# NCKempke/PIPS-IPMpp

Hardware: AMD Instinct MI355X
Metric: KKT factor+solve per IPM iter/sec, N-block arrowhead LP (higher is better)
Workload: dtype f64; 1 GPU; 64 blocks x 10000 vars (5000 eq rows, rho=0.001), Schur dim 2000, 64 blocks/GPU [BASELINE configs[1]]; deterministic=False, family=random, root=dense LDL^T, sparse_head=multifrontal (k_front), solves_per_unit=4, collective=none, nnzL_per_gpu=649118456

## Files before the change

### include/pips_hip.h

```cpp
#ifndef PIPS_HIP_H
#define PIPS_HIP_H
#include <stddef.h>
#include <stdint.h>

#ifdef __cplusplus
extern "C" {
#endif

const char* pips_hip_last_error(void);
long long pips_hip_host_wait_count(void);
int pips_hip_host_wait_sites(char* buf, int cap);
long long pips_hip_device_allocs_live(void);
long long pips_hip_device_bytes_live(void);
int pips_hip_device_count(void);

int pips_hip_ldl_create(void** handle, int n, const int* krow, const int* jcol, int device, int flags);
int pips_hip_ldl_set_inertia_hint(void* handle, int n_primal);
int pips_hip_ldl_set_pivot_rule(void* handle, double thr_rel, double repl_rel);
int pips_hip_ldl_set_refinement(void* handle, int max_steps, double tol);
int pips_hip_ldl_set_refinement_backward_error(void* handle, int max_steps, double tol);
int pips_hip_ldl_set_deterministic(void* handle, int on);
int pips_hip_ldl_analyze(void* handle);
int pips_hip_ldl_factor(void* handle, const double* vals_host);
int pips_hip_ldl_set_values(void* handle, const double* K_val_host);
// ... 147 lines not shown
} pips_csr_view;
typedef struct {
   int n, my, mz;
   pips_csr_view A, B, C, D, BL, DL;
   const double *c, *xlow, *xupp, *ixlow, *ixupp;
   const double* b;
   const double *clow, *cupp, *iclow, *icupp;
} pips_ipm_block;
int pips_ipm_create_general(void** handle, int n_blocks, const pips_ipm_block* blocks, int myl, int mzl, const double* bL,
                            const double* dlow, const double* dupp, const double* idlow, const double* idupp, double dual_reg,
                            int device, void* comm, int rank, int n_ranks);
int pips_ipm_create(void** handle, int N, int n0, int myl, const int* n_i, const int* my_i, const int* W_rowptr,
                    const int* W_colidx, const double* W_val, const int* T_rowptr, const int* T_colidx, const double* T_val,
                    const int* F_rowptr, const int* F_colidx, const double* F_val, const int* F0_rowptr, const int* F0_colidx,
                    const double* F0_val, const double* c, const double* b, double dual_reg, int device);
int pips_ipm_create_rank(void** handle, int N, int n0, int myl, const int* n_i, const int* my_i, const int* W_rowptr,
                         const int* W_colidx, const double* W_val, const int* T_rowptr, const int* T_colidx, const double* T_val,
                         const int* F_rowptr, const int* F_colidx, const double* F_val, const int* F0_rowptr, const int* F0_colidx,
                         const double* F0_val, const double* c, const double* b, double dual_reg, int device, void* comm, int rank,
                         int n_ranks);
int pips_ipm_solve(void* handle, int max_iter, double mutol, double artol, int verbose, double* result7);
int pips_ipm_set_gondzio(void* handle, int max_correctors);
int pips_ipm_set_option(void* handle, const char* name, double value);
int pips_ipm_set_free_variables(void* handle, const double* bounded_mask_host);
int pips_ipm_get_solution(void* handle, double* x_host, double* y_host);
int pips_ipm_get_dims(void* handle, long long* dims4);
int pips_ipm_get_iterate(void* handle, double* x, double* s, double* y, double* z, double* t, double* u, double* v, double* w,
                         double* lambda, double* pi, double* gamma, double* phi);
int pips_ipm_get_trace(void* handle, double* rows7, int max_rows, int* n_rows);
int pips_ipm_get_stats(void* handle, long long* stats4);
int pips_ipm_get_stats2(void* handle, long long* stats2);
int pips_ipm_get_schur_mode(void* handle, int* mode);
int pips_ipm_mult(void* handle, int transposed, const double* in_host, double* out_host);
enum {
   PIPS_SCALER_NONE = 0,
   PIPS_SCALER_EQUILIBRIUM = 1,
   PIPS_SCALER_GEOMETRIC_MEAN = 2,
   PIPS_SCALER_GEOMETRIC_MEAN_EQUILIBRIUM = 3,
   PIPS_SCALER_CURTIS_REID = 4
};
int pips_ipm_create_general_scaled(void** handle, int n_blocks, const pips_ipm_block* blocks, int myl, int mzl, const double* bL,
                                   const double* dlow, const double* dupp, const double* idlow, const double* idupp, double dual_reg,
                                   int device, void* comm, int rank, int n_ranks, int scaler);
int pips_ipm_get_scaling(void* handle, double* col, double* row_eq, double* row_ineq, double* info8);
int pips_ipm_outer_solve(void* handle, const double* G_host, const double* L_host, const double* rhs_host, double tol, double* sol_host,
                         double* info6);
int pips_ipm_create_qp(void** handle, int n_blocks, const pips_ipm_block* blocks, const pips_csr_view* Q, int myl, int mzl,
                       const double* bL, const double* dlow, const double* dupp, const double* idlow, const double* idupp,
                       double dual_reg, int device, void* comm, int rank, int n_ranks);
int pips_ipm_hessian_mult(void* handle, const double* in_host, double* out_host);
void pips_ipm_destroy(void* handle);

int pips_gen_row_nnz(int n_i, double rho);
int pips_gen_block(uint64_t seed, int block, int n_i, int my_i, int n0, int myl, double rho, int* W_rowptr,
                   int* W_colidx, double* W_val, int* T_rowptr, int* T_colidx, double* T_val, int* F_rowptr,
                   int* F_colidx, double* F_val, double* c, double* xstar);
int pips_gen_root(uint64_t seed, int n0, int myl, int* F0_rowptr, int* F0_colidx, double* F0_val, double* c0,
                  double* xstar0);
int pips_gen_diagonal(uint64_t seed, int block, int n, double lo, double hi, double* d);
int pips_kkt_leaf_assemble(int nx, int my, int mz, const int* Q_rowptr, const int* Q_colidx, const double* Q_val,
                           const int* B_rowptr, const int* B_colidx, const double* B_val, const int* D_rowptr,
                           const int* D_colidx, const double* D_val, int* K_rowptr, int* K_colidx, double* K_val,
                           int* diag_pos);
int pips_border_assemble(int nx, int my, int mz, int n0, int n_empty, int myl, int mzl, const int* R_rowptr,
                         const int* R_colidx, const double* R_val, const int* A_rowptr, const int* A_colidx,
                         const double* A_val, const int* C_rowptr, const int* C_colidx, const double* C_val,
                         const int* F_rowptr, const int* F_colidx, const double* F_val, const int* G_rowptr,
                         const int* G_colidx, const double* G_val, int* Bt_rowptr, int* Bt_colidx, double* Bt_val);
int pips_map_children_to_ranks(int n_children, int n_ranks, int* map);
int pips_symbolic_probe(int n, int n_primal, const int* krow, const int* jcol, int S, const int* Bt_rowptr,
                        const int* Bt_colidx, int force_n_head, int64_t* what, int n_what, int* perm, int* colcount);

int pips_symbolic_probe_hubs(int n, int n_primal, const int* krow, const int* jcol, int n_hubs, const int* hubs, int min_size,
                             int64_t* what, int n_what, int* perm, int* colcount);

int pips_layout_probe(int nblk, const int* n, const int* n_primal, const int* const* krow, const int* const* kcol,
                      int S, const int* const* bt_rowptr, const int* const* bt_colidx,
                      int deterministic, long long free_device_bytes, int64_t* what, int n_what);

int pips_tail_plan_probe(int nblk, const int* n, const int* n_primal, const int* const* krow, const int* const* kcol,
                         int S, const int* const* bt_rowptr, const int* const* bt_colidx, int force_n_head,
                         int* col_tasks, long long col_cap, int* grp_tasks, long long grp_cap, int64_t* counts);

int pips_det_plan_probe(int nblk, const int* n, const int* n_primal, const int* const* krow, const int* const* kcol,
                        int S, const int* const* bt_rowptr, const int* const* bt_colidx, int rank, int n_ranks, int n_panels,
                        long long* out, long long cap, int64_t* counts);

enum { PIPS_IPML_DIMS = 20, PIPS_IPML_SLOTS = 48 };
int pips_ipm_layout_probe(int n_blocks, const pips_ipm_block* blocks, const pips_csr_view* Q, int myl, int mzl, const double* bL,
                          const double* dlow, const double* dupp, const double* idlow, const double* idupp, int rank, int n_ranks,
                          int eliminate_z0, const double* col, const double* row, long long* dims, double* scalars, long long* sizes,
                          void* const* out);

int pips_schur_pack_probe(int nblk, int S, const int* const* bt_rowptr, int* nb, int* nb_max, int* const* local_of_row);

int pips_schur_target_probe(int nblk, int S, const int* const* bt_rowptr, const int* sc_rowptr, const int* sc_colidx, int lower, int* nb,
                            long long* n_touched, long long* pos, long long cap, int* const* tab);

int pips_gdx_read_block(void** block, const char* path, int num_blocks, int act_block, int offset);
int pips_gdx_block_counts(void* block, long long* counts14);
int pips_gdx_block_vector(void* block, int which, double* out, int capacity, int* length);
int pips_gdx_block_matrix(void* block, int which, int* present, int* rows, int* cols, int* rowptr, int* colidx, double* val);
void pips_gdx_block_destroy(void* block);

#ifdef __cplusplus
}
#endif
#endif
```

### pips-ipmpp_amd/csrc/engine.hip

```cpp
#include <hip/hip_runtime.h>

#include <algorithm>
#include <cstdlib>
#include <cstring>
#include <map>
#include <memory>
#include <mutex>
#include <thread>
#include <vector>

#include "common.h"
#include "devmem.h"
#include "layout.h"
#include "detplan.h"
#include "schurtarget.h"
#include "kernels.hip.h"
#include "rootkernel.hip.h"
#include "tailkernel.hip.h"
#include "pips_hip.h"

namespace pips {

static thread_local std::string g_last_error;
void set_last_error(const std::string& msg) { g_last_error = msg; }
// ... 655 lines not shown
         if (l.cnt > 0) launch_tile_gemm<2>(c, c.d_sc_tasks, l, c.stream, SC, ldSC);
         HIP_TRY(hipEventRecord((*c.ev_sc)[g], c.stream));
      }
   } else if (tile_gemm_bal_ready(c) && !c.d_sctab)
      launch_tile_gemm_bal<2>(c, p.d_tasks, p.schur, c.stream, SC, ldSC);
   else
      launch_tile_gemm<2>(c, p.d_tasks, p.schur, c.stream, SC, ldSC);
   return PIPS_OK;
}

static int tail_factor(const TailCtx& c, double* SC, int ldSC) {
   const bool trsm_tri = !c.bunch_kaufman && !c.is_root && env_int("PIPS_HIP_TRSM_DENSE", 0) == 0;
   if (!c.single && c.panels && c.side && trsm_tri && env_int("PIPS_HIP_TAIL_PANEL", 1) != 0) PIPS_TRY(tail_panels(c));
   else if (!c.single) PIPS_TRY(tail_columns(c, trsm_tri));
   else if (c.single->n_tasks > 0) PIPS_TRY(tail_single_launch(c));
   PIPS_TRY(tail_schur(c, SC, ldSC));
   HIP_TRY(hipGetLastError());
   return PIPS_OK;
}

static int tail_fwd(const TailCtx& c, double* xw, int nrhs = 1, long long xw_stride = 0) {
   const TailPlan& p = *c.plan;
   if (c.sweep && c.sweep->enabled && nrhs <= SWEEP_NRHS_MAX) {
      hipLaunchKernelGGL(k_tail_rows_fwd, dim3(c.sweep->n_tasks, nrhs), dim3(256), 0, c.stream, c.sweep->args(xw_stride, c.stream), c.d_blks, c.d_arena, c.d_dtail,
                         c.d_winv, xw);
      HIP_TRY(hipGetLastError());
      return PIPS_OK;
   }
   for (int j = 0; j < p.ntc_max; ++j)
      if (p.fwd[j].cnt > 0)
         hipLaunchKernelGGL(k_tail_fwd, dim3(p.fwd[j].cnt, nrhs), dim3(256), 0, c.stream, p.d_tasks + p.fwd[j].off, c.d_blks,
                            c.d_arena, c.d_dtail, c.d_winv, xw, j, xw_stride);
   HIP_TRY(hipGetLastError());
   return PIPS_OK;
}

static int tail_bwd(const TailCtx& c, double* xw, int nrhs = 1, long long xw_stride = 0, int border = 0) {
   const TailPlan& p = *c.plan;
   if (p.ntc_max == 0) return PIPS_OK;
   if (border && !(c.sweep && c.sweep->enabled)) PIPS_FAIL(PIPS_ERR_STATE, "border-backward sweep needs the single-launch tail sweeps");
   if (c.sweep && c.sweep->enabled && nrhs <= SWEEP_NRHS_MAX) {
      hipLaunchKernelGGL(k_tail_rows_bwd, dim3(c.sweep->n_tasks, nrhs), dim3(256), 0, c.stream, c.sweep->args(xw_stride, c.stream), c.d_blks, c.d_arena, c.d_dtail,
                         c.d_winv, xw, border);
      HIP_TRY(hipGetLastError());
      return PIPS_OK;
   }
   for (int i = p.ntc_max - 1; i >= 0; --i)
      if (p.bwd[i].cnt > 0)
         hipLaunchKernelGGL(k_tail_bwd, dim3(p.bwd[i].cnt, nrhs), dim3(256), 0, c.stream, p.d_tasks + p.bwd[i].off, c.d_blks,
                            c.d_arena, c.d_dtail, c.d_winv, xw, i, xw_stride);
   HIP_TRY(hipGetLastError());
   return PIPS_OK;
}


struct AnalyzeKnobs : LayoutKnobs {
   long long tail_poll_limit = 0;
   int tail_diag_blocked = 1;
};
struct Engine;
static void read_layout_knobs(const Engine* e, AnalyzeOptions& opt, AnalyzeKnobs& knobs);

struct EngineAnalysis {
   DevBuf<double> d_norms;
   PinnedBuf<double> h_norms;
   DevBuf<int> d_frowptr, d_fcol, d_fsrc;
   DevBuf<long long> d_flong;
   DevBuf<int> d_sctab;
   long long sc_len = 0;
   DevBuf<int> d_schur_cols, d_schur_slot;
   SchurPack pack;
   int packed_rhs = 0;
   DevBuf<int> d_pk_la;
   DevBuf<long long> d_pk_tabrow;
   PackRows h_pk_rows;
   std::vector<int> h_pk_tab;
   DevBuf<int> d_kb_rec;
   DevBuf<long long> d_kb_off;
   DevBuf<int> d_kb_list;
   DevBuf<int> d_kb_tail;
   DevBuf<double> d_mfU;
   DevBuf<double> d_mfLV;
   DevBuf<int> d_roots, d_root_off;
   DevBuf<BbBatch> d_bb_batches;
   DevBuf<BbMeta> d_bb_meta;
   DevBuf<int> d_bb_off, d_bb_pos;
   DevBuf<double> d_bb_out;
   DevBuf<int> d_bb_round_blk;
   DevBuf<int> d_round_blk;
   DevBuf<int> d_mfint;
   DevBuf<long long> d_mfdbg;
   DevBuf<int> d_spine, d_spine_off;
   TailPlan plan;
   PanelPlan panels;
   SweepRt sweep;
   TailSingle tsingle;
   DevBuf<double> d_uarena;
   DevBuf<double> d_arena, d_kval, d_bval, d_winv, d_dtail, d_xw, d_rhs, d_res, d_stage, d_pref;
   DevBuf<long long> d_kdst, d_bdst, d_kdiag, d_kptr, d_psign_off, d_perm_off, d_rowbase, d_bt_xoff;
   DevBuf<SnDesc> d_sns;
   DevBuf<BlkDesc> d_blks;
   DevBuf<int> d_lf_rows, d_lf_ptr, d_lf_src, d_lf_pos;
   DevBuf<double> d_lf_val;
   DevBuf<LeafDesc> d_leafdesc;
   DevBuf<int> d_lb_list;
   DevBuf<int> d_rowidx, d_upd, d_sncol, d_bmap, d_perm, d_inertia, d_nprimal;
   DevBuf<int> d_br_rowptr, d_br_sc, d_br_src;
   DevBuf<int> d_krowptr, d_kcolidx, d_bt_rowptr, d_bt_colidx, d_bt_rowsc;
   DevBuf<signed char> d_psign;
   struct GatherList {
      long long n_targets = 0, n_slots = 0;
      DevBuf<long long> d_tgt, d_off, d_slots;
      int upload(const HostGather& h) {
         *this = GatherList();
         n_targets = (long long)h.tgt.size(); n_slots = (long long)h.slots.size();
         if (h.tgt.empty()) return PIPS_OK;
         int rc;
         if ((rc = d_tgt.upload(h.tgt)) || (rc = d_off.upload(h.off)) || (rc = d_slots.upload(h.slots))) return rc;
         return PIPS_OK;
      }
   };
   DetGroupPlan det;
   ScKept sc_kept;
   DevBuf<double> d_slot_val, d_vslot_val;
   DevBuf<double> d_mvslot;
   std::vector<GatherList> g_levels, gv_levels;
   GatherList g_tail, g_sc, gv_tail;
   GatherList g_sc_grp;
   GatherList g_btm_grp;
   GatherList g_pk_grp;
   DevBuf<double> d_gvec, d_tvec;
   DevBuf<TileTask> d_det_tasks;
   DevBuf<double> d_gbuf;
   DevBuf<int> d_blk_group;
   GatherList g_btm, g_bm;
   DevBuf<BgEntry> d_bg_ent;
   DevBuf<long long> d_bg_ptr, d_bg_slot;
   DevBuf<int> d_bg_idx;
   DevBuf<double> d_bg_val;
   GatherList g_bslot_grp;
   DevBuf<double> d_bt_tmp;
   DevBuf<int> d_gemm_ctr;
   ScPanelPlan scp;
   std::vector<hipEvent_t> ev_sc;
   DevBuf<TileTask> d_sc_tasks;
   DevBuf<double> d_mx_xw, d_mx_rhs, d_mx_res;
   int mx_cap = 0;
   DevBuf<double> d_mmeasure;
   PinnedBuf<double> h_mmeasure;
   DevBuf<int> d_midx;
   DevBuf<double> d_hostx;
   DevBuf<double> d_hostpack;
   PinnedBuf<int> h_inertia_pin;
   hipEvent_t ev_inertia = nullptr;
   bool inertia_in_flight = false, inertia_on_host = false;
};

struct Engine : EngineAnalysis, BatchLayout {
   int device = 0;
   hipStream_t stream = nullptr;
   int nblk = 0, S = 0;
   bool analyzed = false, factored = false;
   long long analysis_gen = 0;
   int refine_steps = 1;
   double refine_tol = 0.0;
   int refine_mode = 0;
// ... 162 lines not shown
         PIPS_TRY(d_bb_meta.upload(h_bb_meta));
         PIPS_TRY(d_bb_pos.upload(h_bb_pos));
         PIPS_TRY(d_bb_off.upload(h_bb_off));
      }
      if (kb_any) {
         PIPS_TRY(d_kb_rec.upload(h_kb_rec));
         PIPS_TRY(d_kb_off.upload(h_kb_off));
         PIPS_TRY(d_kb_list.upload(h_kb_list));
         PIPS_TRY(d_kb_tail.upload(h_kb_tail));
      }
      if (mf) {
         PIPS_TRY(d_mfint.upload(h_mfint));
         PIPS_TRY(d_mfU.alloc((size_t)std::max<long long>(mfU_total, 1)));
         PIPS_TRY(d_mfLV.alloc((size_t)std::max<long long>(mfLV_total, 1)));
      }
      PIPS_TRY(d_frowptr.upload(h_frowptr));
      PIPS_TRY(d_fcol.upload(h_fcol));
      PIPS_TRY(d_fsrc.upload(h_fsrc));
      PIPS_TRY(d_flong.upload(h_flong));
      if (deterministic && bt_rows_total > 0) {
         const BorderGathers bg = border_product_gathers(*this);
         PIPS_TRY(g_btm.upload(bg.btm));
         PIPS_TRY(g_bm.upload(bg.bm));
         PIPS_TRY(d_bt_tmp.alloc((size_t)std::max<long long>(std::max(bt_rows_total, nnzB_total), 1)));
      }
      PIPS_TRY(d_schur_cols.upload(schur_cols));
      PIPS_TRY(d_schur_slot.upload(h_schur_slot));
      PIPS_TRY(d_arena.alloc(std::max<long long>(arena_total + bb_doubles + tail_scratch, 1)));
      if (tail_single) HIP_TRY(hipMemsetAsync(d_arena, 0, (size_t)arena_total * sizeof(double), stream));
      if (bb_doubles > 0) HIP_TRY(hipMemsetAsync(d_arena + arena_total, 0, (size_t)bb_doubles * sizeof(double), stream));
      PIPS_TRY(d_uarena.alloc(std::max<long long>(uarena_total, 1)));
      PIPS_TRY(d_kval.alloc(std::max<long long>(nnzK_total, 1)));
      HIP_TRY(hipMemset(d_kval, 0, std::max<long long>(nnzK_total, 1) * sizeof(double)));
      PIPS_TRY(d_winv.alloc(std::max<long long>(winv_total, 1)));
      PIPS_TRY(d_dtail.alloc(std::max<long long>(dtail_total, 1)));
      PIPS_TRY(d_xw.alloc(std::max<long long>(xw_total, 1)));
      PIPS_TRY(d_pref.alloc(std::max<long long>(xw_total, 1)));
      PIPS_TRY(d_rhs.alloc(std::max<long long>(n_total, 1)));
      PIPS_TRY(d_res.alloc(std::max<long long>(n_total, 1)));
      PIPS_TRY(d_stage.alloc(std::max<long long>(n_total, 1)));
      PIPS_TRY(d_norms.alloc((size_t)3 * nblk));
      PIPS_TRY(h_norms.alloc((size_t)3 * nblk));
      PIPS_TRY(d_inertia.alloc((size_t)3 * nblk));
      HIP_TRY(hipMemset(d_inertia, 0, (size_t)3 * nblk * sizeof(int)));
      PIPS_TRY(d_bval.upload(h_bval));
      PIPS_TRY(d_kdst.upload(h_kdst));
      PIPS_TRY(d_bdst.upload(h_bdst));
      PIPS_TRY(d_kdiag.upload(h_kdiag));
      PIPS_TRY(d_kptr.upload(kptr));
      PIPS_TRY(d_psign_off.upload(h_psign_off));
      PIPS_TRY(d_perm_off.upload(h_perm_off));
      PIPS_TRY(d_rowbase.upload(h_rowbase));
      PIPS_TRY(d_bt_xoff.upload(h_bt_xoff));
      PIPS_TRY(d_sns.upload(h_sns));
      PIPS_TRY(d_blks.upload(h_blks));
      PIPS_TRY(d_rowidx.upload(h_rowidx));
      if (n_lb > 0) PIPS_TRY(d_lb_list.upload(h_lb_list));
      if (!h_leafdesc.empty()) PIPS_TRY(d_leafdesc.upload(h_leafdesc));
      if (lf_entries > 0) {
         PIPS_TRY(d_lf_rows.upload(h_lf_rows));
         PIPS_TRY(d_lf_ptr.upload(h_lf_ptr));
         PIPS_TRY(d_lf_src.upload(h_lf_src));
         PIPS_TRY(d_lf_pos.upload(h_lf_pos));
         PIPS_TRY(d_lf_val.alloc((size_t)lf_entries));
      }
      PIPS_TRY(d_upd.upload(h_upd));
      PIPS_TRY(d_spine.upload(h_spine));
      PIPS_TRY(d_spine_off.upload(h_spine_off));
      PIPS_TRY(d_sncol.upload(h_sncol));
      PIPS_TRY(d_bmap.upload(h_bmap));
      PIPS_TRY(d_perm.upload(h_perm));
      PIPS_TRY(d_psign.upload(h_psign));
      PIPS_TRY(d_krowptr.upload(h_krowptr));
      PIPS_TRY(d_kcolidx.upload(h_kcolidx));
      PIPS_TRY(d_bt_rowptr.upload(h_bt_rowptr));
      PIPS_TRY(d_bt_colidx.upload(h_bt_colidx));
      PIPS_TRY(d_bt_rowsc.upload(h_bt_rowsc));
      if (!h_br_rowptr.empty()) {
         PIPS_TRY(d_br_rowptr.upload(h_br_rowptr));
         PIPS_TRY(d_br_sc.upload(h_br_sc));
         PIPS_TRY(d_br_src.upload(h_br_src));
      }
      PIPS_TRY(d_nprimal.upload(h_nprimal));
      return PIPS_OK;
   }

   ScatterCtx sx_atomic() const { return ScatterCtx{0, nullptr, nullptr, nullptr, nullptr}; }
   void launch_head_level(const LevelRange& L, double* SC, int ldSC, const ScatterCtx& sx) {
      if (L.simple_cnt > 0)
         hipLaunchKernelGGL(k_head_factor_simple, dim3((L.simple_cnt + 255) / 256), dim3(256), 0, stream, d_sns, L.simple_begin,
                            L.simple_cnt, d_blks, d_rowidx, d_upd, d_psign, d_psign_off, d_bmap, d_arena, SC, ldSC, d_inertia, d_pref, d_sctab, sx,
                            mf ? 1 : 0, d_mfLV, d_lf_pos, d_lf_val, d_arena);
      if (mf) return;
      if (L.small_cnt > 0)
         hipLaunchKernelGGL((k_head_factor<64, 8, 640>), dim3(L.small_cnt), dim3(64), (size_t)std::max(L.small_lds, 1) * sizeof(double), stream, d_sns,
                            L.small_begin, d_blks, d_rowidx, d_upd, d_psign, d_psign_off, d_bmap, d_arena, SC, ldSC, d_inertia, d_pref, d_sctab, sx,
                            L.small_lds);
      if (L.large_cnt > 0)
         hipLaunchKernelGGL((k_head_factor<256, 32, 6144>), dim3(L.large_cnt), dim3(256), (size_t)std::max(L.large_lds, 1) * sizeof(double), stream, d_sns,
                            L.large_begin, d_blks, d_rowidx, d_upd, d_psign, d_psign_off, d_bmap, d_arena, SC, ldSC,
                            d_inertia, d_pref, d_sctab, sx, L.large_lds);
   }
   template <int BLOCK, int WMAX, bool UG = false>
   int launch_front(const MfLaunch& m, double* SC, int ldSC) {
      const size_t lds = (size_t)m.lds_doubles * sizeof(double);
      if (lds > 64 * 1024) HIP_TRY(hipFuncSetAttribute((const void*)k_front<BLOCK, WMAX, UG>, hipFuncAttributeMaxDynamicSharedMemorySize, (int)lds));
      hipLaunchKernelGGL((k_front<BLOCK, WMAX, UG>), dim3(m.cnt), dim3(BLOCK), lds, stream, d_sns, m.begin, d_blks, d_rowidx, d_mfint, d_psign,
                         d_psign_off, d_bmap, d_arena, d_mfU, SC, ldSC, d_inertia, d_pref, d_sctab, d_mfdbg, d_mfLV, d_kval, d_bval, deterministic ? 1 : 0, d_arena);
      return PIPS_OK;
   }
   int launch_border_schur(double* SC, int ldSC) {
      constexpr int BLK = 512;
      const long long ncp = ((long long)bb_nbmax * (bb_nbmax + 1) / 2 + 1) & ~1LL;
      constexpr int parts = 1;
      const long long c_cap = ncp;
      BbPlanSize z; z.stage = bb_stage; z.poscap = bb_poscap; z.nbmax = bb_nbmax;
      const size_t lds = bb_lds_bytes(z);
      if (!bb_fits(z))
         PIPS_FAIL(PIPS_ERR_STATE, "k_border_schur: %zu bytes of LDS for nb = %d (batch of %d doubles, %d rows)", lds, bb_nbmax, bb_stage, bb_poscap);
      const int split = std::max(1, std::min(32, (bb_two_per_cu ? 512 : 256) / std::max(nblk, 1)));
      auto go = [&](auto kern, int cnt, const int* list, double* gb, long long gs, const int* grp, int sp, int ordered, double* out = nullptr,
                    long long out_stride = 0) -> int {
         if (lds > 64 * 1024) HIP_TRY(hipFuncSetAttribute((const void*)kern, hipFuncAttributeMaxDynamicSharedMemorySize, (int)lds));
         hipLaunchKernelGGL(kern, dim3(cnt, sp, parts), dim3(BLK), lds, stream, list, d_bb_off, d_bb_batches, d_bb_meta, d_bb_pos, d_blks, d_bmap, d_arena, SC, ldSC,
                            d_sctab, gb, gs, grp, bb_stage, bb_poscap, ordered, out, out_stride, (int)c_cap);
         return PIPS_OK;
      };
      const bool small = bb_stage <= 2 * 3 * BLK;
      int rc = PIPS_OK;
      if (deterministic && d_gbuf && d_bb_round_blk) {
         const long long tri = (long long)ncp;
         if (!d_bb_out) PIPS_TRY(d_bb_out.alloc((size_t)std::max(nblk, 1) * tri));
         rc = small ? go(k_border_schur<BLK, 3>, nblk, (const int*)nullptr, (double*)nullptr, 0LL, (const int*)nullptr, 1, 1, d_bb_out, tri)
                    : go(k_border_schur<BLK, 6>, nblk, (const int*)nullptr, (double*)nullptr, 0LL, (const int*)nullptr, 1, 1, d_bb_out, tri);
         for (size_t k = 0; k + 1 < det.bb_round_off.size() && !rc; ++k) {
            const int cnt = det.bb_round_off[k + 1] - det.bb_round_off[k];
            if (cnt > 0)
               hipLaunchKernelGGL(k_border_schur_add, dim3(cnt, 8), dim3(256), 0, stream, d_bb_round_blk + det.bb_round_off[k], d_blks, d_bmap, d_bb_out, tri, ldSC, d_sctab,
                                  d_gbuf, det_gstride(), d_blk_group);
         }
      } else
         rc = small ? go(k_border_schur<BLK, 3>, nblk, (const int*)nullptr, (double*)nullptr, 0LL, (const int*)nullptr, split, deterministic ? 1 : 0)
                    : go(k_border_schur<BLK, 6>, nblk, (const int*)nullptr, (double*)nullptr, 0LL, (const int*)nullptr, split, deterministic ? 1 : 0);
      return rc;
   }
   int dump_front_clocks() {
      std::vector<long long> h((size_t)nsn_total * 8);
      HIP_TRY(hipStreamSynchronize(stream));
      HIP_TRY(hipMemcpy(h.data(), d_mfdbg, h.size() * sizeof(long long), hipMemcpyDeviceToHost));
      static const char* names[7] = {"panel+zero", "stage ints", "leaf values + children", "leaf columns", "pivots", "update", "write-out"};
      for (const MfLaunch& m : mf_launches) {
         double ph[8] = {0}; long long nfs = 0, ws = 0;
         for (int i = m.begin; i < m.begin + m.cnt; ++i) {
            for (int q = 0; q < 7; ++q) ph[q] += (double)(h[(size_t)i * 8 + q + 1] - h[(size_t)i * 8 + q]);
            nfs += h_sns[i].w + h_sns[i].r; ws += h_sns[i].w;
         }
         fprintf(stderr, "[mf clocks] level %2d variant %d fronts %6d lds %6d  avg nf %5.1f w %4.1f | ", m.level, m.cls, m.cnt, m.lds_doubles * 8, (double)nfs / m.cnt, (double)ws / m.cnt);
         for (int q = 0; q < 7; ++q) fprintf(stderr, "%s %.1f%s", names[q], ph[q] / m.cnt * 0.01, q == 6 ? " us\n" : ", ");
      }
      return PIPS_OK;
   }
   void launch_border_rows(size_t l, hipStream_t st) {
      const int cnt = kb_level_off[l + 1] - kb_level_off[l];
      if (cnt == 0) return;
      const int* lst = d_kb_list + kb_level_off[l];
      if (kb_level_pairs[l] <= 3 || (cnt >= 16384 && kb_level_pairs[l] <= 8))
         hipLaunchKernelGGL((k_border_rows<64, 16>), dim3(cnt), dim3(64), kb_level_lds[l], st, lst, d_sns, d_blks, d_rowidx, d_kb_rec, d_kb_off, d_arena, d_arena, d_bval);
      else if (cnt <= 4096 && kb_level_pairs[l] > 8)
         hipLaunchKernelGGL((k_border_rows<512, 16>), dim3(cnt), dim3(512), kb_level_lds[l], st, lst, d_sns, d_blks, d_rowidx, d_kb_rec, d_kb_off, d_arena, d_arena, d_bval);
      else
         hipLaunchKernelGGL((k_border_rows<256, 16>), dim3(cnt), dim3(256), kb_level_lds[l], st, lst, d_sns, d_blks, d_rowidx, d_kb_rec, d_kb_off, d_arena, d_arena, d_bval);
   }
   int launch_fronts(int level, double* SC, int ldSC) {
      int rc = PIPS_OK;
      for (const MfLaunch& m : mf_launches) {
// ... 34 lines not shown
         HIP_TRY(hipGetLastError());
         HIP_TRY(hipStreamSynchronize(stream));
         HIP_TRY(hipMemcpy(rec.data(), d_rec, (size_t)slots_total * sizeof(long long), hipMemcpyDeviceToHost));
         d_rec.reset();
         PIPS_TRY(d_slot_val.alloc((size_t)slots_total));
      }
      {
         FactorSlotPlan fp;
         if ((rc = classify_factor_slots(rec, SCATTER_SC_FLAG, *this, sym, fp))) return rc;
         std::vector<long long>().swap(rec);
         for (int l = 0; l < nlev; ++l) PIPS_TRY(g_levels[l].upload(fp.levels[l]));
         PIPS_TRY(g_tail.upload(fp.tail));
         PIPS_TRY(g_sc.upload(fp.sc));
         sc_kept = std::move(fp.kept);
      }
      if (vslots_total > 0) {
         DevBuf<long long> d_rec;
         PIPS_TRY(d_rec.alloc((size_t)vslots_total));
         HIP_TRY(hipMemsetAsync(d_rec, 0xff, (size_t)vslots_total * sizeof(long long), stream));
         const ScatterCtx sxv{1, d_rec, nullptr, d_xw, nullptr};
         for (const LevelRange& L : levels) {
            if (L.simple_cnt > 0 && lf_rows == 0)
               hipLaunchKernelGGL(k_head_solve_simple, dim3((L.simple_cnt + 255) / 256, 1), dim3(256), 0, stream, d_sns, L.simple_begin,
                                  L.simple_cnt, d_blks, d_rowidx, d_arena, d_xw, 0LL, 0, sxv);
            const int begin = L.small_cnt > 0 ? L.small_begin : L.large_begin;
            const int cnt = L.small_cnt + L.large_cnt;
            if (cnt > 0) hipLaunchKernelGGL(k_head_fwd, dim3(cnt, 1), dim3(64), 0, stream, d_sns, begin, d_blks, d_rowidx, d_arena, d_xw, 0LL, sxv);
         }
         HIP_TRY(hipGetLastError());
         HIP_TRY(hipStreamSynchronize(stream));
         std::vector<long long> vrec((size_t)vslots_total);
         HIP_TRY(hipMemcpy(vrec.data(), d_rec, (size_t)vslots_total * sizeof(long long), hipMemcpyDeviceToHost));
         d_rec.reset();
         PIPS_TRY(d_vslot_val.alloc((size_t)vslots_total));
         SolveSlotPlan vp;
         classify_solve_slots(vrec, *this, sym, vp);
         for (int l = 0; l < nlev; ++l) PIPS_TRY(gv_levels[l].upload(vp.levels[l]));
         PIPS_TRY(gv_tail.upload(vp.tail));
      }
      (void)n_threads;
      return PIPS_OK;
   }

   const SchurPack& border_pack() {
      if (pack.off.empty()) build_schur_pack(in, S, pack);
      return pack;
   }
   int set_sc_tables(const std::vector<int>& tab, const std::vector<long long>& off, long long sc_nnz) {
      if (!analyzed) PIPS_FAIL(PIPS_ERR_STATE, "set_sc_tables: analyze first");
      HIP_TRY(hipSetDevice(device));
      int rc = d_sctab.upload(tab);
      if (rc) return rc;
      for (int b = 0; b < nblk; ++b) h_blks[b].sctab_off = off[b];
      HIP_TRY(hipMemcpy(d_blks, h_blks.data(), (size_t)nblk * sizeof(BlkDesc), hipMemcpyHostToDevice));
      sc_len = sc_nnz;
      packed_rhs = 0;
      if (schur_mode_eff == 2) {
         const SchurPack& pk = border_pack();
         if (pk.nb_max >= (1 << 24)) PIPS_FAIL(PIPS_ERR_STATE, "set_sc_tables: %d border columns in one block exceed the packed solves' 2^24", pk.nb_max);
         if ((rc = schur_pack_rows(in, S, off, (long long)tab.size(), h_pk_rows))) return rc;
         if ((long long)h_pk_rows.la.size() != bt_rows_total)
            PIPS_FAIL(PIPS_ERR_STATE, "set_sc_tables: %zu border rows, the analysis holds %lld", h_pk_rows.la.size(), bt_rows_total);
         PIPS_TRY(d_pk_la.upload(h_pk_rows.la));
         PIPS_TRY(d_pk_tabrow.upload(h_pk_rows.tabrow));
         if (deterministic) h_pk_tab = tab;
         else h_pk_rows = PackRows();
         packed_rhs = pk.nb_max;
      }
      if (head_slots) {
         g_levels.clear(); gv_levels.clear();
         g_tail = GatherList(); g_sc = GatherList(); gv_tail = GatherList();
         d_slot_val.reset(); d_vslot_val.reset(); d_mvslot.reset();
         if ((rc = build_deterministic(1))) return rc;
      }
      return PIPS_OK;
   }

   int factor_prologue() {
      PhaseTimer::Scope phase(&timer, stream, 0);
      hipLaunchKernelGGL(k_block_absmax_init, dim3((nblk + 255) / 256), dim3(256), 0, stream, d_blks, nblk);
      hipLaunchKernelGGL(k_block_absmax, dim3(std::max(1, std::min(64, (int)(nnzK_total / nblk / 4096))), nblk), dim3(256), 0, stream, d_kval,
                         d_kptr, d_blks);
      hipLaunchKernelGGL(k_block_absmax_finish, dim3((nblk + 255) / 256), dim3(256), 0, stream, d_blks, nblk, thr_rel, repl_rel);
      hipLaunchKernelGGL(k_arena_clear, dim3(256, nblk), dim3(256), 0, stream, d_blks, d_arena, mf ? 1 : 0);
      HIP_TRY(hipMemsetAsync(d_inertia, 0, (size_t)3 * nblk * sizeof(int), stream));
      if (!d_gemm_ctr) PIPS_TRY(d_gemm_ctr.alloc((size_t)GEMM_CTR_SLOTS * 8));
      HIP_TRY(hipMemsetAsync(d_gemm_ctr, 0, (size_t)GEMM_CTR_SLOTS * 8 * sizeof(int), stream));
      gemm_ctr_cursor = 0;
      if (nnzK_total > 0)
         hipLaunchKernelGGL(k_scatter, dim3(grid_for(nnzK_total, 256)), dim3(256), 0, stream, d_kdst, d_kval, d_arena, nnzK_total);
      if (nnzB_total > 0 && schur_mode_eff == 1)
         hipLaunchKernelGGL(k_scatter, dim3(grid_for(nnzB_total, 256)), dim3(256), 0, stream, d_bdst, d_bval, d_arena, nnzB_total);
      hipLaunchKernelGGL(k_tail_pad_diag, dim3(nblk), dim3(128), 0, stream, d_blks, d_arena, nblk);
      hipLaunchKernelGGL(k_pref_rows, dim3(32, nblk), dim3(256), 0, stream, d_blks, d_kval, d_kdiag, d_res, d_nprimal, d_krowptr, d_kcolidx);
      hipLaunchKernelGGL(k_pref_init, dim3(32, nblk), dim3(256), 0, stream, d_blks, d_perm, d_perm_off, (const double*)d_res, d_pref);
      return PIPS_OK;
   }
   void launch_root_assemble(double* SC, int ldSC) {
      const int asm_half = std::max(1, std::min(32, 1024 / std::max(nblk, 1)));
      if (deterministic && d_gbuf && SC && d_round_blk) {
         for (size_t k = 0; k + 1 < det.round_off.size(); ++k) {
            const int cnt = det.round_off[k + 1] - det.round_off[k];
            if (cnt > 0)
               hipLaunchKernelGGL(k_root_assemble, dim3(cnt, 2 * asm_half), dim3(256), 0, stream, d_round_blk + det.round_off[k], d_root_off, d_roots, d_sns, d_blks, d_rowidx,
                                  d_bmap, d_arena, d_mfU, SC, ldSC, d_sctab, d_gbuf, det_gstride(), d_blk_group, asm_half, asm_half);
         }
      } else
         hipLaunchKernelGGL(k_root_assemble, dim3(nblk, 2 * asm_half), dim3(256), 0, stream, (const int*)nullptr, d_root_off, d_roots, d_sns, d_blks, d_rowidx, d_bmap,
                            d_arena, d_mfU, SC, ldSC, d_sctab, (double*)nullptr, 0LL, (const int*)nullptr, asm_half, asm_half);
   }
   int factor_head(double* SC, int ldSC) {
      const ScatterCtx sx = head_slots ? ScatterCtx{2, nullptr, d_slot_val, d_arena, SC} : sx_atomic();
      for (size_t li = 0; li < levels.size(); ++li) {
         PhaseTimer::Scope phase(&timer, stream, 1);
         if (head_slots) gather(g_levels[li], d_slot_val, d_arena);
         launch_head_level(levels[li], SC, ldSC, sx);
         if (mf) PIPS_TRY(launch_fronts((int)li, SC, ldSC));
      }
      if (head_slots) {
         PhaseTimer::Scope phase(&timer, stream, 1);
         gather(g_tail, d_slot_val, d_arena);
         if (SC && deterministic && d_gbuf) {
            HIP_TRY(hipMemsetAsync(d_gbuf, 0, (size_t)det.n_groups * det_gstride() * sizeof(double), stream));
            gather(g_sc_grp, d_slot_val, d_gbuf);
         } else if (SC) gather(g_sc, d_slot_val, SC);
      }
      if (mf && n_roots > 0) { PhaseTimer::Scope phase(&timer, stream, 1); launch_root_assemble(SC, ldSC); }
      if (mf && d_kb_list) {
         PhaseTimer::Scope phase(&timer, stream, 1);
         for (size_t l = 0; l + 1 < kb_level_off.size(); ++l) launch_border_rows(l, stream);
         if (n_kb_tail > 0) hipLaunchKernelGGL(k_border_tail<16>, dim3(n_kb_tail), dim3(64), 0, stream, d_kb_tail, d_sns, d_blks, d_rowidx, d_arena);
      }
      if (mf && n_bb > 0 && SC) { PhaseTimer::Scope phase(&timer, stream, 1); PIPS_TRY(launch_border_schur(SC, ldSC)); }
      if (spine_total > 0) {
         PhaseTimer::Scope phase(&timer, stream, 1);
         hipLaunchKernelGGL((k_head_factor_spine<256, 32, 6144>), dim3(nblk), dim3(256), 0, stream, d_spine, d_spine_off, d_sns, d_blks,
                            d_rowidx, d_upd, d_psign, d_psign_off, d_bmap, d_arena, SC, ldSC, d_inertia, d_pref, d_sctab);
      }
      if (mf && getenv("PIPS_HIP_MF_CLOCKS")) {
         if (!d_mfdbg) PIPS_TRY(d_mfdbg.alloc((size_t)std::max(nsn_total, 1) * 8));
         else PIPS_TRY(dump_front_clocks());
      }
      hipLaunchKernelGGL(k_pref_tail, dim3(8, nblk), dim3(256), 0, stream, d_blks, d_arena, d_pref, 0);
      HIP_TRY(hipGetLastError());
      return PIPS_OK;
   }
   int factor_tail(double* SC, int ldSC) {
      TailCtx c = ctx();
      c.timer = &timer;
      c.det_reduce_later = schur_mode_eff == 2;
      PIPS_TRY(tail_factor(c, SC, ldSC));
      factored = true;
      perturbed_cache = -1;
      if (SC && schur_mode_eff == 2 && !schur_cols.empty()) {
         const int rec_schur = timer.begin_i(stream, 5);
         const int rc = schur_by_solves(SC, ldSC);
         timer.end_i(rec_schur, stream);
         if (rc) return rc;
      }
      if (SC && c.det_rounds && c.det_reduce_later) reduce_det_groups(c, SC, ldSC);
      return PIPS_OK;
   }
   int post_inertia() {
      h_amax.clear();
      if (!h_inertia_pin) {
         PIPS_TRY(h_inertia_pin.alloc((size_t)(3 * nblk + 1)));
         h_inertia_pin[3 * nblk] = 0;
         HIP_TRY(hipEventCreateWithFlags(&ev_inertia, hipEventDisableTiming));
      }
      HIP_TRY(hipMemcpyAsync(h_inertia_pin, d_inertia, (size_t)3 * nblk * sizeof(int), hipMemcpyDeviceToHost, stream));
      if (tail_single)
         HIP_TRY(hipMemcpyAsync(h_inertia_pin + 3 * nblk, tsingle.d_ctl + 9, sizeof(int), hipMemcpyDeviceToHost, stream));
      HIP_TRY(hipEventRecord(ev_inertia, stream));
      inertia_in_flight = true;
      inertia_on_host = false;
      return PIPS_OK;
   }
   int factor(double* SC, int ldSC) {
      if (!analyzed) PIPS_FAIL(PIPS_ERR_STATE, "factor called before analyze");
      HIP_TRY(hipSetDevice(device));
      if (deterministic && SC && S > 0 && !d_gbuf && d_blk_group)
         PIPS_TRY(d_gbuf.alloc((size_t)det.n_groups * det_gstride()));
      timer.reset();
      const int rec_total = timer.begin_i(stream, 6);
      PIPS_TRY(factor_prologue());
      PIPS_TRY(factor_head(SC, ldSC));
      PIPS_TRY(factor_tail(SC, ldSC));
      timer.end_i(rec_total, stream);
      return post_inertia();
   }

   int schur_by_solves(double* SC, int ldSC) {
      int rc = ensure_multi_buffers();
      if (rc) return rc;
      const bool det = deterministic && d_gbuf;
      const bool det_panel = det && det_panel_fits();
      if (det_panel && !d_mvslot) PIPS_TRY(d_mvslot.alloc((size_t)std::max<long long>(vslots_total, 1) * MQ));
      if (packed_rhs > 0) return schur_by_packed_solves(SC, det, det_panel);
      if (det && ldSC != S) PIPS_FAIL(PIPS_ERR_ARG, "deterministic mode, Schur mode 2: ldSC %d must equal S %d (the group buffers are S x S)", ldSC, S);
      const int bs = 32, ncols = (int)schur_cols.size();
      for (int c0 = 0; c0 < ncols; c0 += bs) {
         const int nr = std::min(bs, ncols - c0);
         HIP_TRY(hipMemsetAsync(d_mx_rhs, 0, (size_t)nr * n_total * sizeof(double), stream));
         hipLaunchKernelGGL(k_border_rows_to_dense, dim3(grid_for(bt_rows_total, 256)), dim3(256), 0, stream, d_bt_rowptr, d_bt_colidx,
                            d_bval, d_bt_rowsc, d_bt_xoff, d_schur_slot, c0, nr, d_mx_rhs, n_total, bt_rows_total);
         if ((rc = solve_chunk(d_mx_rhs, nr, det, det_panel))) return rc;
         if (det) {
            if (g_btm_grp.n_targets > 0)
               hipLaunchKernelGGL(k_border_tmult_chunk_det, dim3(grid_for(g_btm_grp.n_targets * 32, 256)), dim3(256), 0, stream, g_btm_grp.n_targets,
// ... 432 lines not shown
      {
         PhaseTimer::Scope phase(&timer, stream, 9);
         PIPS_TRY(tail_fwd(ctx(), d_xw));
         if (nb_pad_max > 0)
            hipLaunchKernelGGL(k_tail_border_fwd, dim3(nb_pad_max / TILE, nblk), dim3(256), 0, stream, d_blks, d_arena, d_dtail, d_xw);
         hipLaunchKernelGGL(k_border_collect, dim3(8, nblk), dim3(256), 0, stream, d_blks, d_bmap, d_xw, red);
      }
      ++aug_passes;
      HIP_TRY(hipGetLastError());
      return PIPS_OK;
   }
   int forward_augmented_det(const double* b_dev) {
      if (!factored) PIPS_FAIL(PIPS_ERR_STATE, "solve called before factor");
      if (!det.aug.ready || !head_slots) PIPS_FAIL(PIPS_ERR_STATE, "forward_augmented_det: not prepared");
      HIP_TRY(hipSetDevice(device));
      {
         PhaseTimer::Scope phase(&timer, stream, 7);
         hipLaunchKernelGGL(k_border_fill, dim3(8, nblk), dim3(256), 0, stream, d_blks, d_bmap, (const double*)nullptr, d_xw, 0.0);
         hipLaunchKernelGGL(k_permute_in, dim3(64, nblk, 1), dim3(256), 0, stream, d_blks, d_perm, d_perm_off, b_dev, 0LL, d_xw, 0LL);
      }
      {
         PhaseTimer::Scope phase(&timer, stream, 8);
         head_forward(d_xw, 1, 0, ScatterCtx{2, nullptr, d_vslot_val, d_xw, nullptr}, 0);
         hipLaunchKernelGGL(k_border_rowdot_det, dim3(grid_for(det.aug.n_ent, 256, 1 << 20)), dim3(256), 0, stream, det.aug.n_ent, d_bg_ent, d_arena, d_xw, d_bg_val);
         hipLaunchKernelGGL(k_border_gather_det, dim3((unsigned)((det.aug.n_targets + 3) / 4)), dim3(256), 0, stream, det.aug.n_targets, d_bg_ptr, d_bg_idx, d_bg_slot, d_bg_val, d_xw);
      }
      {
         PhaseTimer::Scope phase(&timer, stream, 9);
         PIPS_TRY(tail_fwd(ctx(), d_xw));
         if (nb_pad_max > 0)
            hipLaunchKernelGGL(k_tail_border_fwd, dim3(nb_pad_max / TILE, nblk), dim3(256), 0, stream, d_blks, d_arena, d_dtail, d_xw);
      }
      ++aug_passes;
      HIP_TRY(hipGetLastError());
      return PIPS_OK;
   }
   int backward_augmented(const double* x0_dev, double* out_dev) {
      if (!factored) PIPS_FAIL(PIPS_ERR_STATE, "solve called before factor");
      HIP_TRY(hipSetDevice(device));
      {
         PhaseTimer::Scope phase(&timer, stream, 10);
         hipLaunchKernelGGL(k_border_fill, dim3(8, nblk), dim3(256), 0, stream, d_blks, d_bmap, x0_dev, d_xw, 1.0);
         PIPS_TRY(tail_bwd(ctx(), d_xw, 1, 0, 1));
         head_backward(d_xw, 1, 0, 1, 1);
      }
      { PhaseTimer::Scope phase(&timer, stream, 7); hipLaunchKernelGGL(k_permute_out, dim3(64, nblk, 1), dim3(256), 0, stream, d_blks, d_perm, d_perm_off, out_dev, 0LL, d_xw, 0LL); }
      HIP_TRY(hipGetLastError());
      return PIPS_OK;
   }
   int solve_border_backward(const double* x0_dev, double* out_dev) {
      if (!factored) PIPS_FAIL(PIPS_ERR_STATE, "solve called before factor");
      HIP_TRY(hipSetDevice(device));
      HIP_TRY(hipMemsetAsync(d_xw, 0, (size_t)xw_total * sizeof(double), stream));
      hipLaunchKernelGGL(k_border_fill, dim3(8, nblk), dim3(256), 0, stream, d_blks, d_bmap, x0_dev, d_xw);
      TailCtx c = ctx();
      int rc = tail_bwd(c, d_xw, 1, 0, 1);
      if (rc) return rc;
      head_backward(d_xw, 1, 0, 1, 0, true);
      hipLaunchKernelGGL(k_permute_out, dim3(64, nblk, 1), dim3(256), 0, stream, d_blks, d_perm, d_perm_off, out_dev, 0LL, d_xw, 0LL);
      HIP_TRY(hipGetLastError());
      return PIPS_OK;
   }
};

static void read_layout_knobs(const Engine* e, AnalyzeOptions& opt, AnalyzeKnobs& knobs) {
   opt.tile = TILE;
   opt.max_sn_width = 16;
   if (const char* sw = getenv("PIPS_HIP_SN_WIDTH")) opt.max_sn_width = std::max(1, std::min(HEAD_WMAX, atoi(sw)));
   else if (e && e->sn_width > 0) opt.max_sn_width = std::min(HEAD_WMAX, e->sn_width);
   if (const char* rz = getenv("PIPS_HIP_RELAX_ZEROS")) opt.relax_zeros = atof(rz);
   if (const char* ndd = getenv("PIPS_HIP_ND_DEPTH")) opt.nd_depth = atoi(ndd);
   if (const char* ndm = getenv("PIPS_HIP_ND_MIN")) opt.nd_min_size = atoi(ndm);
   if (const char* ml = getenv("PIPS_HIP_MF_LDS")) opt.mf_lds_doubles = atoll(ml);
   if (const char* sp = getenv("PIPS_HIP_MF_SPLIT")) opt.mf_split_nb_max = atoi(sp) == 0 ? 0 : std::min(176, std::max(atoi(sp), 2));
   knobs.deterministic = e && e->deterministic;
   knobs.schur_mode = e ? e->schur_mode : 0;
   if (e && knobs.schur_mode == 0) knobs.schur_mode = std::max(0, std::min(2, env_int("PIPS_HIP_SCHUR_MODE", 0)));
   knobs.mf_lds_doubles = opt.mf_lds_doubles;
   knobs.mf_wanted = env_int("PIPS_HIP_MF", 1) != 0;
   if (!knobs.mf_wanted) opt.mf_split_nb_max = 0;
   opt.mf_konly = opt.mf_split_nb_max > 0 && !knobs.deterministic && opt.max_sn_width <= 16 && env_int("PIPS_HIP_MF_KONLY", 0) != 0;
   knobs.spine = env_flag("PIPS_HIP_SPINE");
   knobs.tail_single = env_flag("PIPS_HIP_TAIL_SINGLE");
   knobs.border_backward = env_flag("PIPS_HIP_BORDER_BACKWARD");
   knobs.aug_sweeps = env_flag("PIPS_HIP_AUG_SWEEPS");
   knobs.sweep_launches = getenv("PIPS_HIP_SWEEP_LAUNCHES") != nullptr;
   const int poll = env_int("PIPS_HIP_ROOT_POLL_LIMIT", 400000);
   knobs.tail_poll_limit = poll > 0 ? (long long)poll * 50 : 0;
   knobs.tail_diag_blocked = env_int("PIPS_HIP_ROOT_DIAG_BARRIERS", 0) ? 0 : 1;
}


extern "C" int pips_hip_allreduce_sum(void* comm, double* buf_dev, size_t n, void* stream);
extern "C" int pips_hip_all_gather(void* comm, double* buf_dev, size_t chunk, int n_parts, void* stream);
extern "C" int pips_hip_broadcast(void* comm, double* buf_dev, size_t n, int root, void* stream);
extern "C" int pips_hip_comm_has_broadcast(void* comm);

__global__ void k_inertia_to_double(const int* __restrict__ in, double* __restrict__ out, int back, int* __restrict__ in_out) {
   if (threadIdx.x < 3) { if (!back) out[threadIdx.x] = (double)in[threadIdx.x]; else in_out[threadIdx.x] = (int)(out[threadIdx.x] + 0.5); }
}

struct DenseLdl {
   int device = 0, n = 0, npad = 0, n_primal = -1;
   int pivoting = 0;
   hipStream_t stream = nullptr;
   double thr_rel = 1e-13, repl_rel = 1e-8;
   bool factored = false;
   std::vector<BlkDesc> h_blks;
   TailPlan plan;
   DevBuf<BlkDesc> d_blks;
   DevBuf<double> d_R, d_winv, d_dtail, d_xw, d_in, d_pref;
   DevBuf<double> d_U;
   DevBuf<signed char> d_psign;
   DevBuf<long long> d_psign_off, d_kptr;
   DevBuf<int> d_inertia;
   int h_inertia[3] = {0, 0, 0};
   hipStream_t side = nullptr;
   hipEvent_t ev_panel = nullptr, ev_rest = nullptr;
   int ensure_input_buffer() {
      if (!d_in) PIPS_TRY(d_in.alloc((size_t)std::max(n, 1) * std::max(n, 1)));
      return PIPS_OK;
   }

   ~DenseLdl() {
      if (side) (void)hipStreamDestroy(side);
      if (ev_panel) (void)hipEventDestroy(ev_panel);
      if (ev_rest) (void)hipEventDestroy(ev_rest);
   }
   SweepRt sweep;
   bool single_launch = !getenv("PIPS_HIP_ROOT_LAUNCHES");
   bool last_single = false;
   DevBuf<double> d_C;
   DevBuf<TileTask> d_rtasks;
   int n_rtasks = 0, n_rbulk = 0;
   DevBuf<int> d_rflags;
   double plan_makespan_us = 0.0;
   long long root_poll_limit = 400000;
   bool root_error_pending = false;
   int ensure_single_launch() {
      if (d_rtasks) return PIPS_OK;
      const int ntc = npad / TILE;
      RootPlanParams pp;
      if (const char* q = getenv("PIPS_HIP_ROOT_CHAIN_CU")) pp.chain_slots = atoi(q) != 0 ? 2 : 0;
      if (pp.chain_slots == 0) pp.workers = 512;
      std::vector<int> t, tc;
      int rc = build_root_plan(ntc, pp, t, tc, &plan_makespan_us);
      if (rc) return rc;
      n_rbulk = (int)(t.size() / 4);
      t.insert(t.end(), tc.begin(), tc.end());
      n_rtasks = (int)(t.size() / 4);
      PIPS_TRY(d_rtasks.alloc(std::max<size_t>(t.size() / 4, 1)));
      HIP_TRY(hipMemcpy(d_rtasks, t.data(), t.size() * sizeof(int), hipMemcpyHostToDevice));
      PIPS_TRY(d_rflags.alloc(((size_t)8 + (size_t)ntc * ntc + 2 * (size_t)ntc)));
      PIPS_TRY(d_C.alloc((size_t)npad * npad));
      if (const char* pl = getenv("PIPS_HIP_ROOT_POLL_LIMIT")) root_poll_limit = atoll(pl);
      return PIPS_OK;
   }
   int factor_single_launch() {
      const int ntc = npad / TILE;
      HIP_TRY(hipMemsetAsync(d_rflags, 0, ((size_t)8 + (size_t)ntc * ntc + 2 * (size_t)ntc) * sizeof(int), stream));
      RootArgs a{};
      a.tasks = d_rtasks; a.n_tasks = n_rtasks; a.n_bulk = n_rbulk; a.ntc = ntc; a.ld = npad;
      a.C = d_C; a.R = d_R; a.U = d_U; a.winv = d_winv; a.dtail = d_dtail; a.pref = d_pref; a.psign = d_psign; a.inertia = d_inertia;
      a.ctl = d_rflags; a.prog = d_rflags + 8; a.rowdone = a.prog + (size_t)ntc * ntc; a.dready = a.rowdone + ntc;
      a.blk = d_blks; a.poll_limit = root_poll_limit;
      a.diag_blocked = getenv("PIPS_HIP_ROOT_DIAG_BARRIERS") ? 0 : 1;
// ... 593 lines not shown
      hipLaunchKernelGGL(k_border_entry_products, dim3(grid_for(e->bt_rows_total, 256)), dim3(256), 0, e->stream, e->d_bt_rowptr, e->d_bval,
                         e->d_bt_rowsc, x0_dev, e->d_bt_tmp, e->bt_rows_total, alpha);
      e->gather(e->g_bm, e->d_bt_tmp, t_dev);
   } else if (e->bt_rows_total > 0 && e->d_br_rowptr)
      hipLaunchKernelGGL(k_border_mult_rows, dim3(grid_for(e->n_total, 256, 1 << 20)), dim3(256), 0, e->stream, e->d_br_rowptr, e->d_br_sc, e->d_br_src,
                         e->d_bval, x0_dev, t_dev, e->n_total, alpha);
   else if (e->bt_rows_total > 0)
      hipLaunchKernelGGL(k_border_mult, dim3(grid_for(e->bt_rows_total * BT_LANES, 256, 65536)), dim3(256), 0, e->stream, e->d_bt_rowptr,
                         e->d_bt_colidx, e->d_bval, e->d_bt_rowsc, e->d_bt_xoff, x0_dev, t_dev, e->bt_rows_total, alpha);
   HIP_TRY(hipGetLastError());
   return PIPS_OK;
}

int pips_hip_batch_inertia(void* handle, int b, int* pos, int* neg, int* zero) {
   Engine* e = (Engine*)handle;
   if (!e || !e->factored || b < 0 || b >= e->nblk) PIPS_FAIL(PIPS_ERR_STATE, "pips_hip_batch_inertia: factor first");
   int rc = e->fetch_inertia();
   if (rc) return rc;
   if (pos) *pos = e->h_inertia[3 * b];
   if (neg) *neg = e->h_inertia[3 * b + 1];
   if (zero) *zero = e->h_inertia[3 * b + 2];
   return PIPS_OK;
}

int pips_hip_batch_tail_to_host(void* handle, int b, int which, double* out, int64_t n_out, int* dims) {
   Engine* e = (Engine*)handle;
   if (!e || !e->factored || b < 0 || b >= e->nblk || which < 0 || which > 2) PIPS_FAIL(PIPS_ERR_STATE, "pips_hip_batch_tail_to_host: factor first");
   const BlkDesc& bd = e->h_blks[b];
   if (dims) { dims[0] = bd.m; dims[1] = bd.m_pad; dims[2] = bd.nb; dims[3] = bd.ldT; }
   if (!out) return PIPS_OK;
   const double* src = which == 0 ? e->d_arena + bd.T : which == 1 ? e->d_uarena + bd.U : e->d_dtail + bd.dt_off;
   const int64_t n = which == 0 ? (int64_t)bd.ldT * bd.m_pad : which == 1 ? (int64_t)bd.m_pad * bd.m_pad : bd.m_pad;
   if (n_out < n) PIPS_FAIL(PIPS_ERR_ARG, "pips_hip_batch_tail_to_host: %lld doubles needed, %lld given", (long long)n, (long long)n_out);
   HIP_TRY(hipSetDevice(e->device));
   HIP_TRY(hipStreamSynchronize(e->stream));
   if (n > 0) HIP_TRY(hipMemcpy(out, src, (size_t)n * sizeof(double), hipMemcpyDeviceToHost));
   return PIPS_OK;
}

static void sym_info(const std::vector<BlockSym>& sym, int64_t* what, int n_what) {
   int64_t v[13] = {0};
   for (const BlockSym& s : sym) {
      v[10] += (int64_t)s.upd.size() * 4;
      v[11] += s.nb;
      v[12] += (int64_t)s.a_dst.size();
      v[0] += s.nnzL; v[1] += s.n; v[2] += s.n_head; v[3] += s.m; v[4] += (int64_t)s.sn.size();
      v[5] = std::max<int64_t>(v[5], s.n_levels);
      v[6] += (int64_t)s.flops_factor; v[7] += (int64_t)s.flops_border; v[8] += s.arena * 8;
      v[9] = std::max<int64_t>(v[9], s.m_pad / TILE);
   }
   for (int i = 0; i < n_what && i < 13; ++i) what[i] = v[i];
}

int pips_hip_batch_info(void* handle, int64_t* what, int n_what) {
   Engine* e = (Engine*)handle;
   if (!e || e->sym.empty()) PIPS_FAIL(PIPS_ERR_STATE, "pips_hip_batch_info: analyze first");
   sym_info(e->sym, what, n_what);
   if (n_what > 13) what[13] = e->border_backward_ok ? 1 : 0;
   if (n_what > 14) what[14] = e->mf ? 1 : 0;
   if (n_what > 15) { what[15] = 0; for (const BlockSym& s : e->sym) what[15] = std::max<int64_t>(what[15], s.mf_max_front); }
   if (n_what > 16) what[16] = e->mfU_total * 8;
   if (n_what > 17) { what[17] = 0; for (const MfLaunch& m : e->mf_launches) if (m.cls >= 6) what[17] += m.cnt; }
   if (n_what > 19) {
      what[18] = what[19] = 0;
      for (const BlockSym& s : e->sym) {
         what[18] += s.nnzL - (int64_t)s.m * (s.m + 1) / 2;
         what[19] += (int64_t)s.rowidx.size();
      }
   }
   if (n_what > 21) {
      what[20] = 0;
      int64_t tail_border = 0;
      for (const BlockSym& s : e->sym) {
         for (const HeadSupernode& hs : s.sn) what[20] += (int64_t)hs.w * (hs.r - hs.rb);
         tail_border += (int64_t)s.nb * s.m;
      }
      what[21] = e->aug_sweeps_ok ? 1 : 0;
      if (n_what > 22) what[22] = e->aug_passes;
      if (n_what > 23) what[23] = tail_border;
   }
   if (n_what > 24) { what[24] = 0; for (const BlockSym& s : e->sym) what[24] += s.mf_split ? 1 : 0; }
   if (n_what > 25) { what[25] = 0; for (const BlockSym& s : e->sym) what[25] += (e->mf && s.mf_konly) ? 1 : 0; }
   if (n_what > 26) what[26] = e->packed_rhs;
   return PIPS_OK;
}

int pips_hip_batch_sync(void* handle) {
   Engine* e = (Engine*)handle;
   if (!e) PIPS_FAIL(PIPS_ERR_ARG, "null handle");
   HIP_TRY(hipSetDevice(e->device));
   HIP_TRY(hipStreamSynchronize(e->stream));
   return e->sweep.take_error("pips_hip_batch_sync");
}

int pips_hip_batch_set_timing(void* handle, int on) {
   Engine* e = (Engine*)handle;
   if (!e) PIPS_FAIL(PIPS_ERR_ARG, "null handle");
   e->timer.on = on != 0;
   return PIPS_OK;
}

int pips_hip_batch_get_timing(void* handle, double* ms, int64_t* cnt, int n) {
   Engine* e = (Engine*)handle;
   if (!e) PIPS_FAIL(PIPS_ERR_ARG, "null handle");
   HIP_TRY(hipSetDevice(e->device));
   HIP_TRY(hipStreamSynchronize(e->stream));
   e->timer.collect();
   for (int i = 0; i < n && i < PhaseTimer::NPHASE; ++i) {
      if (ms) ms[i] = e->timer.ms[i];
      if (cnt) cnt[i] = e->timer.cnt[i];
   }
   return PIPS_OK;
}

void pips_hip_batch_destroy(void* handle) { delete (Engine*)handle; }

struct LdlGroup;
struct SchurScratch {
   std::mutex mu;
   std::map<int, DevBuf<double>> per_device;
};
static SchurScratch& g_schur_scratch = *new SchurScratch;

__global__ void k_schur_take_block(double* __restrict__ SC, int ld, const int* __restrict__ bm, int nb, double* __restrict__ C) {
   const int j = blockIdx.y;
   for (int i = blockIdx.x * blockDim.x + threadIdx.x; i < nb; i += gridDim.x * blockDim.x) {
      double* p = SC + bm[i] + (long long)bm[j] * ld;
      C[i + (long long)j * nb] = *p;
      *p = 0.0;
   }
}

enum { SC_KIND_NONE = 0, SC_KIND_DENSE = 1, SC_KIND_SPARSE = 2 };
struct SparseSchurBind {
   bool bound = false;
   SchurPatternId id;
   std::vector<long long> pos;
   DevBuf<double> d_val;
   std::vector<double> h_val;
};

struct LdlHandle {
   Engine eng;
   bool have_perm = false;
   int sc_kind = SC_KIND_NONE;
   SparseSchurBind sparse_sc;
   DevBuf<double> d_sc;
   std::vector<double> h_sc;
   std::shared_ptr<LdlGroup> group;
   int group_index = -1;
   bool newest_in_group = false;
   ~LdlHandle();
};
struct LdlGroup {
   Engine eng;
   std::vector<LdlHandle*> members;
   DevBuf<double> d_sc, d_x;
   std::vector<double> h_sc;
   int sc_kind = SC_KIND_NONE;
   SparseSchurBind sparse_sc;
};
LdlHandle::~LdlHandle() {
   if (group && group_index >= 0 && group_index < (int)group->members.size() && group->members[group_index] == this) group->members[group_index] = nullptr;
}
static int ldl_group_is_current(const LdlGroup& g, const char* who) {
   if (!g.eng.factored) PIPS_FAIL(PIPS_ERR_STATE, "%s: pips_hip_ldl_factor_schur_batch first", who);
// ... 1017 lines not shown
   AnalyzeKnobs knobs;
   read_layout_knobs(nullptr, opt, knobs);
   if (deterministic) { knobs.deterministic = true; opt.mf_konly = false; }
   knobs.free_device_bytes = free_device_bytes;
   std::vector<BlockSym> sym;
   BatchLayout lay;
   const int n_threads = (int)std::max(1u, std::min(16u, std::thread::hardware_concurrency()));
   int rc = analyze_symbolic(in, S, n_threads, opt, knobs, sym);
   if (!rc) rc = build_batch_layout(in, sym, S, knobs, lay);
   if (!rc) rc = check_batch_layout(in, sym, S, knobs, lay);
   if (rc) return rc;
   int64_t v[21] = {lay.arena_total, lay.xw_total, lay.uarena_total, lay.nsn_total, (int64_t)lay.levels.size(), (int64_t)lay.levels_top.size(),
                    (int64_t)lay.mf_launches.size(), 0, lay.n_bb, lay.bb_stage, lay.tail_single, lay.border_backward_ok, lay.aug_sweeps_ok,
                    lay.slots_total, lay.vslots_total, lay.n_total, lay.mf, lay.schur_mode_eff, lay.bb_doubles, lay.mfU_total, lay.spine_total};
   for (const MfLaunch& m : lay.mf_launches) if (m.cls >= 6) v[7] += m.cnt;
   for (int i = 0; what && i < n_what && i < 21; ++i) what[i] = v[i];
   return PIPS_OK;
}

int pips_tail_plan_probe(int nblk, const int* n, const int* n_primal, const int* const* krow, const int* const* kcol, int S,
                         const int* const* bt_rowptr, const int* const* bt_colidx, int force_n_head, int* col_tasks, long long col_cap,
                         int* grp_tasks, long long grp_cap, int64_t* counts) {
   std::vector<BlockInput> in;
   PIPS_TRY(probe_inputs("pips_tail_plan_probe", nblk, n, n_primal, krow, kcol, S, bt_rowptr, bt_colidx, in));
   if (!counts || col_cap < 0 || grp_cap < 0 || (col_cap > 0 && !col_tasks) || (grp_cap > 0 && !grp_tasks))
      PIPS_FAIL(PIPS_ERR_ARG, "pips_tail_plan_probe: bad arguments");
   AnalyzeOptions opt;
   AnalyzeKnobs knobs;
   read_layout_knobs(nullptr, opt, knobs);
   opt.force_n_head = force_n_head;
   knobs.free_device_bytes = 0;
   std::vector<BlockSym> sym;
   BatchLayout lay;
   const int n_threads = (int)std::max(1u, std::min(16u, std::thread::hardware_concurrency()));
   PIPS_TRY(analyze_symbolic(in, S, n_threads, opt, knobs, sym));
   PIPS_TRY(build_batch_layout(in, sym, S, knobs, lay));
   TailPlan plan;
   plan.lists(lay.h_blks, 0, false, true, &lay.tile_first, true, 4);
   PanelPlan pp;
   pp.lists(plan, 4);
   long long nc = 0, ng = 0, launches_col = 0, launches_grp = 0;
   auto col = [&](const TaskList& l, int kind) {
      launches_col += l.cnt > 0;
      for (long long q = l.off; q < l.off + l.cnt; ++q, ++nc) {
         const TileTask& t = plan.h_tasks[q];
         if (nc < col_cap) { int* r = col_tasks + 6 * nc; r[0] = kind; r[1] = t.blk; r[2] = t.ti; r[3] = t.tj; r[4] = t.pad & 0xffff; r[5] = t.pad >> 16; }
      }
   };
   auto grp = [&](long long off, int cnt, int list, int group, int index) {
      for (int q = 0; q < cnt; ++q, ++ng) {
         const TileTask& t = pp.h_tasks[off + q];
         if (ng < grp_cap) {
            int* r = grp_tasks + 9 * ng;
            r[0] = list; r[1] = group; r[2] = index; r[3] = q; r[4] = t.blk; r[5] = t.ti; r[6] = t.tj; r[7] = t.pad & 0xffff; r[8] = t.pad >> 16;
         }
      }
   };
   auto grp_list = [&](const TaskList& l, int list, int group, int index) { launches_grp += l.cnt > 0; grp(l.off, l.cnt, list, group, index); };
   for (int j = 0; j < plan.ntc_max; ++j) {
      col(plan.upd_diag[j], 0);
      col(plan.upd[j], 0);
      launches_col += plan.diag[j].cnt > 0;
      col(plan.trsm[j], 1);
   }
   for (int i = 0; i < pp.n_groups; ++i) {
      grp_list(pp.deep[i], 0, i, 0);
      grp_list(pp.pre[i], 1, i, 0);
      grp_list(pp.block_deep[i], 2, i, 0);
      for (int j = i * pp.P; j < std::min((i + 1) * pp.P, plan.ntc_max); ++j) {
         grp_list(pp.upd_in[j], 3, i, j);
         launches_grp += plan.diag[j].cnt > 0;
         grp_list(pp.trsm_in[j], 4, i, j);
      }
      launches_grp += pp.strips[i].cnt > 0;
      for (int q = 0; q < pp.strips[i].cnt; ++q) {
         const TileStrip& st = pp.h_strips[pp.strips[i].off + q];
         grp(st.off, st.cnt, 5, i, q);
      }
   }
   counts[0] = nc; counts[1] = ng; counts[2] = plan.ntc_max; counts[3] = pp.n_groups; counts[4] = launches_col; counts[5] = launches_grp;
   return PIPS_OK;
}

int pips_det_plan_probe(int nblk, const int* n, const int* n_primal, const int* const* krow, const int* const* kcol, int S,
                        const int* const* bt_rowptr, const int* const* bt_colidx, int rank, int n_ranks, int n_panels, long long* out,
                        long long cap, int64_t* counts) {
   std::vector<BlockInput> in;
   PIPS_TRY(probe_inputs("pips_det_plan_probe", nblk, n, n_primal, krow, kcol, S, bt_rowptr, bt_colidx, in));
   if (!counts || cap < 0 || (cap > 0 && !out) || n_ranks < 1 || rank < 0 || rank >= n_ranks) PIPS_FAIL(PIPS_ERR_ARG, "pips_det_plan_probe: bad arguments");
   AnalyzeOptions opt;
   AnalyzeKnobs knobs;
   read_layout_knobs(nullptr, opt, knobs);
   knobs.deterministic = true; opt.mf_konly = false;
   knobs.free_device_bytes = 0;
   std::vector<BlockSym> sym;
   BatchLayout lay;
   const int n_threads = (int)std::max(1u, std::min(16u, std::thread::hardware_concurrency()));
   PIPS_TRY(analyze_symbolic(in, S, n_threads, opt, knobs, sym));
   PIPS_TRY(build_batch_layout(in, sym, S, knobs, lay));
   const BorderGathers bg = lay.bt_rows_total > 0 ? border_product_gathers(lay) : BorderGathers();
   const DetGroupPlan p = build_det_group_plan(lay, sym, S, rank, n_ranks, (long long)S * S, ScKept(), PackedTables());
   const ScPanelPlan sp = sc_panel_plan(lay, sym, S, n_panels);
   long long at = 0;
   int section = 0;
   auto put = [&](long long v) { if (at < cap) out[at] = v; ++at; };
   auto end = [&](long long& from) { counts[16 + section++] = at - from; from = at; };
   auto gather = [&](const HostGather& g) {
      put((long long)g.tgt.size());
      for (long long v : g.tgt) put(v);
      for (long long v : g.off) put(v);
      for (long long v : g.slots) put(v);
   };
   long long from = 0, aug_rows = 0;
   for (const SnDesc& sn : lay.h_sns) aug_rows += sn.r - sn.rb;
   for (int b = 0; b < nblk; ++b) put(p.grp[b]);
   end(from);
   for (int b = 0; b < nblk; ++b) {
      const BlkDesc& d = lay.h_blks[b];
      put(d.ntc); put(d.nb); put(d.nb_pad); put(lay.mf ? lay.h_root_off[b + 1] - lay.h_root_off[b] : 0);
      put(lay.n_bb > 0 ? lay.h_bb_off[b + 1] - lay.h_bb_off[b] : 0); put((long long)sym[b].bmap.size());
   }
   end(from);
   for (size_t k = 0; k < p.rounds.size(); ++k)
      for (long long q = p.rounds[k].off; q < p.rounds[k].off + p.rounds[k].cnt; ++q) { put((long long)k); put(p.tasks[q].blk); put(p.tasks[q].ti); put(p.tasks[q].tj); }
   end(from);
   for (size_t k = 0; k + 1 < p.round_off.size(); ++k)
      for (int q = p.round_off[k]; q < p.round_off[k + 1]; ++q) { put((long long)k); put(p.round_blk[q]); }
   end(from);
   for (size_t k = 0; k + 1 < p.bb_round_off.size(); ++k)
      for (int q = p.bb_round_off[k]; q < p.bb_round_off[k + 1]; ++q) { put((long long)k); put(p.bb_round_blk[q]); }
   end(from);
   gather(p.btm_grp); end(from);
   gather(bg.btm); end(from);
   gather(bg.bm); end(from);
   gather(p.aug.bslot_grp); end(from);
   for (const BgEntry& e : p.aug.ent) { put(e.off); put(e.y); put(e.stride); put(e.w); }
   end(from);
   for (long long v : p.aug.ptr) put(v);
   end(from);
   for (int v : p.aug.idx) put(v);
   end(from);
   for (long long v : p.aug.slot) put(v);
   end(from);
   for (int v : sp.row_begin) put(v);
   end(from);
   for (size_t g = 0; g < sp.groups.size(); ++g)
      for (long long q = sp.groups[g].off; q < sp.groups[g].off + sp.groups[g].cnt; ++q) { put((long long)g); put(sp.tasks[q].blk); put(sp.tasks[q].ti); put(sp.tasks[q].tj); }
   end(from);
   for (int b = 0; b < nblk; ++b)
      for (int v : sym[b].bmap) put(v);
   end(from);
   const int64_t head[16] = {p.n_groups, p.first_slot, p.slots, p.global, p.aug.ready, p.aug_sweeps_ok, lay.aug_sweeps_ok, lay.mf, lay.n_bb, lay.n_roots,
                             lay.schur_mode_eff, (int64_t)sp.groups.size(), p.aug.n_targets, p.aug.n_ent, aug_rows, at};
   std::copy(head, head + 16, counts);
   return PIPS_OK;
}

}
```

### pips-ipmpp_amd/csrc/kernels.hip.h

```cpp
#pragma once
#include <hip/hip_runtime.h>
#include <stdint.h>

#include "records.h"

namespace pips {

constexpr int KB = 16;
constexpr int LDS_PAD = 16;
constexpr int LDSW = TILE + LDS_PAD;

typedef double double4_t __attribute__((ext_vector_type(4)));

struct BelowRow { const double* p; long long stride; };
__device__ __forceinline__ BelowRow below_row(const double* __restrict__ arena, const SnDesc& sn, int a) {
   if (a < sn.ld - sn.w) return BelowRow{arena + sn.panel + sn.w + a, (long long)sn.ld};
   return BelowRow{arena + sn.bb + (a - sn.rb), (long long)((sn.r - sn.rb + 3) & ~3)};
}

__device__ __forceinline__ void atomic_add_f64(double* p, double v) {
   __hip_atomic_fetch_add(p, v, __ATOMIC_RELAXED, __HIP_MEMORY_SCOPE_AGENT);
}

struct ScatterCtx {
// ... 288 lines not shown
            if (aa >= bb) f(bs + aa, bs + bb);
         }
      }
   };

   int b0 = 0;
   const int* U = upd + sn.upd;
   for (int sg = 0; sg < sn.n_useg; ++sg) {
      const int sb0 = U[0], sb1 = U[1], tld = U[3];
      const long long tpanel = (long long)(((unsigned long long)(unsigned)U[5] << 32) | (unsigned long long)(unsigned)U[4]);
      const int* pp = U + USEG_HDR;
      double* TP = arena + bd.arena_off + tpanel;
      for_pairs(sb0, sb1, [&](int a, int b) {
         scatter_add(sx, TP + pp[a - sb0] + (long long)pp[b - sb0] * tld, false, pair_slot(sn.slot, a, b, r), -entry(a, b));
      });
      U += USEG_HDR + (r - sb0);
      b0 = sb1;
   }
   const int n = bd.n, n_head = bd.n_head;
   if (b0 < sn.rb) {
      double* T = arena + bd.T_in;
      for_pairs(b0, sn.rb, [&](int a, int b) {
         const int ra = rows[a], cb = rows[b];
         const int tr = ra < n ? ra - n_head : bd.m_pad + (ra - n);
         scatter_add(sx, T + tr + (long long)(cb - n_head) * bd.ldT, false, pair_slot(sn.slot, a, b, r), -entry(a, b));
      });
      b0 = sn.rb;
   }
   if (b0 < r && SC) {
      const int* bm = bmap + bd.bmap_off;
      for_pairs(b0, r, [&](int a, int b) {
         scatter_add(sx, sc_entry(SC, ldSC, bm, sctab, bd.sctab_off, bd.nb, rows[a] - n, rows[b] - n), true, pair_slot(sn.slot, a, b, r), -entry(a, b));
      });
   }
}

template <int BLOCK, int WMAX, int LCAP>
__global__ __launch_bounds__(BLOCK) void k_head_factor(const SnDesc* __restrict__ sns, int sn_begin,
                                                      const BlkDesc* __restrict__ blks,
                                                      const int* __restrict__ rowidx, const int* __restrict__ upd,
                                                      const signed char* __restrict__ psign,
                                                      const long long* __restrict__ psign_off,
                                                      const int* __restrict__ bmap, double* __restrict__ arena,
                                                      double* __restrict__ SC, int ldSC, int* __restrict__ inertia,
                                                      const double* __restrict__ pref, const int* __restrict__ sctab,
                                                      ScatterCtx sx = ScatterCtx{0, nullptr, nullptr, nullptr, nullptr}, int lcap = LCAP) {
   extern __shared__ double head_Ls[];
   const SnDesc sn = sns[sn_begin + blockIdx.x];
   const BlkDesc bd = blks[sn.blk];
   head_factor_body<BLOCK, WMAX, LCAP>(sn, bd, rowidx, upd, psign, psign_off, bmap, arena, SC, ldSC, inertia, pref, sctab, sx, head_Ls, lcap);
}

template <int BLOCK, int WMAX, int LCAP>
__global__ __launch_bounds__(BLOCK) void k_head_factor_spine(const int* __restrict__ spine, const int* __restrict__ spine_off,
                                                            const SnDesc* __restrict__ sns, const BlkDesc* __restrict__ blks,
                                                            const int* __restrict__ rowidx, const int* __restrict__ upd,
                                                            const signed char* __restrict__ psign,
                                                            const long long* __restrict__ psign_off,
                                                            const int* __restrict__ bmap, double* __restrict__ arena,
                                                            double* __restrict__ SC, int ldSC, int* __restrict__ inertia,
                                                            const double* __restrict__ pref, const int* __restrict__ sctab) {
   __shared__ double Ls[LCAP];
   const int p0 = spine_off[blockIdx.x], p1 = spine_off[blockIdx.x + 1];
   if (p0 == p1) return;
   const BlkDesc bd = blks[blockIdx.x];
   for (int p = p0; p < p1; ++p) {
      const SnDesc sn = sns[spine[p]];
      head_factor_body<BLOCK, WMAX, LCAP>(sn, bd, rowidx, upd, psign, psign_off, bmap, arena, SC, ldSC, inertia, pref, sctab,
                                          ScatterCtx{0, nullptr, nullptr, nullptr, nullptr}, Ls, LCAP);
      __threadfence();
      __syncthreads();
   }
}

__global__ __launch_bounds__(256) void k_head_factor_simple(const SnDesc* __restrict__ sns, int sn_begin, int cnt,
                                                           const BlkDesc* __restrict__ blks, const int* __restrict__ rowidx,
                                                           const int* __restrict__ upd, const signed char* __restrict__ psign,
                                                           const long long* __restrict__ psign_off, const int* __restrict__ bmap,
                                                           double* __restrict__ arena, double* __restrict__ SC, int ldSC,
                                                           int* __restrict__ inertia, const double* __restrict__ pref,
                                                           const int* __restrict__ sctab,
                                                           ScatterCtx sx = ScatterCtx{0, nullptr, nullptr, nullptr, nullptr}, int mf = 0,
                                                           double* __restrict__ lvals = nullptr, const int* __restrict__ lfpos = nullptr,
                                                           double* __restrict__ lfval = nullptr, double* __restrict__ bbarena = nullptr) {
   __shared__ int cnt_s[3];
   __shared__ int blk_s;
   const int t = blockIdx.x * blockDim.x + threadIdx.x;
   if (threadIdx.x == 0) blk_s = sns[sn_begin + min(blockIdx.x * blockDim.x, (unsigned)cnt - 1)].blk;
   if (threadIdx.x < 3) cnt_s[threadIdx.x] = 0;
   __syncthreads();
   if (t < cnt) {
      const SnDesc sn = sns[sn_begin + t];
      const BlkDesc bd = blks[sn.blk];
      const int r = sn.r;
      double* P = arena + sn.panel;
      const int* rows = rowidx + sn.rows;
      bool pert;
      const double d = fix_pivot(P[0], psign[psign_off[sn.blk] + sn.c0], pref[bd.xw_off + sn.c0], bd.thr_rel, bd.repl_rel, bd.repl_abs, pert);
      P[0] = d;
      const int which = pert ? 2 : (d > 0 ? 0 : 1);
      if (sn.blk == blk_s) atomicAdd(&cnt_s[which], 1); else atomicAdd(&inertia[3 * sn.blk + which], 1);
      double l[SIMPLE_RMAX];
      int ro[SIMPLE_RMAX];
#pragma unroll
      for (int a = 0; a < SIMPLE_RMAX; ++a)
         if (a < r) { ro[a] = rows[a]; l[a] = P[1 + a] / d; P[1 + a] = l[a]; }
      if (lfpos) {
         const int* lp = lfpos + sn.rows;
#pragma unroll
         for (int a = 0; a < SIMPLE_RMAX; ++a)
            if (a < r && ro[a] < bd.n) lfval[lp[a]] = l[a];
      }
      double* T = arena + bd.T_in;
      const int* bm = bmap + bd.bmap_off;
      const int n = bd.n, n_head = bd.n_head;
      const bool to_parent = mf && sn.n_useg > 0;
      if (to_parent) {
         double* lv = lvals + sn.U;
         lv[0] = d;
#pragma unroll
         for (int a = 0; a < SIMPLE_RMAX; ++a)
            if (a < r) lv[1 + a] = l[a];
         if (sn.bb >= 0) {
            double* Q = bbarena + sn.bb;
#pragma unroll
            for (int a = 0; a < SIMPLE_RMAX; ++a)
               if (a < r && a >= sn.rb) Q[a - sn.rb] = l[a];
            Q[(r - sn.rb + 3) & ~3] = d;
         }
      }
      int b_head = 0;
      if (to_parent) b_head = r;
      else {
         const int* U = upd + sn.upd;
         const int nseg = sn.n_useg < r ? sn.n_useg : r;
         for (int sg = 0; sg < nseg; ++sg) {
            const int sb0 = U[0], sb1 = U[1], tld = U[3];
            if (sb0 != b_head || sb1 <= sb0 || sb1 > r) break;
            const long long tpanel = (long long)(((unsigned long long)(unsigned)U[5] << 32) | (unsigned long long)(unsigned)U[4]);
            const int* pp = U + USEG_HDR;
            double* TP = arena + bd.arena_off + tpanel;
            for (int b = sb0; b < sb1; ++b) {
               const double lbd = P[1 + b] * d;
               const long long colo = (long long)pp[b - sb0] * tld;
               for (int a = b; a < r; ++a)
                  scatter_add(sx, TP + pp[a - sb0] + colo, false, pair_slot(sn.slot, a, b, r), -P[1 + a] * lbd);
            }
            U += USEG_HDR + (r - sb0);
            b_head = sb1;
         }
      }
#pragma unroll
      for (int b = 0; b < SIMPLE_RMAX; ++b) {
         if (b < r && b >= b_head) {
            const int cb = ro[b];
            const double lbd = l[b] * d;
#pragma unroll
            for (int a = b; a < SIMPLE_RMAX; ++a) {
               if (a < r) {
                  const int ra = ro[a];
                  const double u = l[a] * lbd;
                  if (cb < n) {
                     const int tr = ra < n ? ra - n_head : bd.m_pad + (ra - n);
                     scatter_add(sx, T + tr + (long long)(cb - n_head) * bd.ldT, false, pair_slot(sn.slot, a, b, r), -u);
                  } else if (SC) {
                     scatter_add(sx, sc_entry(SC, ldSC, bm, sctab, bd.sctab_off, bd.nb, ra - n, cb - n), true, pair_slot(sn.slot, a, b, r), -u);
                  }
               }
            }
         }
      }
   }
   __syncthreads();
   if (threadIdx.x < 3 && cnt_s[threadIdx.x]) atomicAdd(&inertia[3 * blk_s + threadIdx.x], cnt_s[threadIdx.x]);
}

__device__ __forceinline__ int packed_col(int p, int n) {
   const float t = 2.0f * n + 1.0f;
   int b = (int)((t - sqrtf(t * t - 8.0f * (float)p)) * 0.5f);
   b = b < 0 ? 0 : (b > n - 1 ? n - 1 : b);
   while (b > 0 && b * n - b * (b - 1) / 2 > p) --b;
   while (b + 1 < n && (b + 1) * n - (b + 1) * b / 2 <= p) ++b;
   return b;
}

__device__ __forceinline__ double readlane_f64(double v, int lane) {
   const int lo = __builtin_amdgcn_readlane(__double2loint(v), lane), hi = __builtin_amdgcn_readlane(__double2hiint(v), lane);
   return __hiloint2double(hi, lo);
}

__device__ __forceinline__ void lds_add(double* p, double v) {
   (void)__hip_atomic_fetch_add(p, v, __ATOMIC_RELAXED, __HIP_MEMORY_SCOPE_WORKGROUP);
}

template <int BLOCK, int WMAX, bool UG>
__global__ __launch_bounds__(BLOCK) void k_front(const SnDesc* __restrict__ sns, int sn_begin, const BlkDesc* __restrict__ blks,
                                                const int* __restrict__ rowidx, const int* __restrict__ mfint,
                                                const signed char* __restrict__ psign, const long long* __restrict__ psign_off,
                                                const int* __restrict__ bmap, double* __restrict__ arena,
                                                double* __restrict__ uarena, double* __restrict__ SC, int ldSC,
                                                int* __restrict__ inertia, const double* __restrict__ pref,
                                                const int* __restrict__ sctab, long long* __restrict__ dbg,
                                                const double* __restrict__ lvals, const double* __restrict__ kval,
                                                const double* __restrict__ bval, int ordered, double* __restrict__ bbarena) {
   extern __shared__ __attribute__((aligned(16))) double mf_F[];
   __shared__ double dk[WMAX];
#define MF_STAMP(q) do { if (dbg && threadIdx.x == 0) dbg[(long long)(sn_begin + blockIdx.x) * 8 + (q)] = (long long)wall_clock64(); } while (0)
   MF_STAMP(0);
   double* F = mf_F;
   const SnDesc sn = sns[sn_begin + blockIdx.x];
   const BlkDesc bd = blks[sn.blk];
   const int w = sn.w, r = bd.mf_split == 2 ? sn.rb : sn.r, nf = w + r, tid = threadIdx.x, lane = tid & 63, i = tid;
   const int* H = mfint + sn.mf;
   const int n_child = H[0], n_leaf = H[1], n_ent = H[2] >> 1, n_leafpart = H[3], n_items = H[4], n_vals = H[5], sum_rc = H[6];
   const int uc = bd.mf_split ? sn.rb : r;
   const int np = uc * r - uc * (uc - 1) / 2;
   auto co = [nf](int j) { return j * nf - j * (j - 1) / 2; };
   const int cw = co(w);
   const int rp = (r + 3) & ~3;
   const int pw = cw > w * rp ? cw : w * rp;
   double* FU = UG ? uarena + sn.U : F + pw;
   auto cu = [r](int b) { return b * r - b * (b - 1) / 2; };
   auto front_add = [&](int fi, int fj, double v) {
      if (fj < w) lds_add(F + co(fj) + (fi - fj), v);
      else if (UG) FU[cu(fj - w) + (fi - fj)] += v;
      else lds_add(FU + cu(fj - w) + (fi - fj), v);
   };
   double* P = arena + sn.panel;
   double* vals = F + pw + (UG ? 0 : np) + 8;
   int* relbuf = (int*)(vals + n_vals);
   int* leafpart = relbuf + sum_rc;

   const double prf = lane < w ? pref[bd.xw_off + sn.c0 + lane] : 1.0;
   const int sgn = lane < w ? (int)psign[psign_off[sn.blk] + sn.c0 + lane] : 0;

   {
      typedef double double2_t __attribute__((ext_vector_type(2)));
      const int nz = (pw + (UG ? 0 : np) + 8 + 1) >> 1;
      double2_t* F2 = (double2_t*)F;
      const double2_t z = {0.0, 0.0};
      for (int idx = tid; idx < nz; idx += BLOCK) F2[idx] = z;
      if (UG) for (int idx = tid; idx < np; idx += BLOCK) FU[idx] = 0.0;
   }
   __syncthreads();
   MF_STAMP(1);
   {
      const int* src = H + MF_HDR + 3 * n_child;
      for (int idx = tid; idx < sum_rc + n_leafpart; idx += BLOCK) relbuf[idx] = src[idx];
   }
   __syncthreads();
   MF_STAMP(2);
   if (n_leaf) {
      const double* lv = lvals + bd.lv_off + H[7];
      for (int idx = tid; idx < n_vals; idx += BLOCK) vals[idx] = lv[idx];
   }
   {
      const int* E = H + MF_HDR + 3 * n_child + sum_rc + n_leafpart + 1;
// ... 124 lines not shown
#pragma unroll
         for (int k = 0; k < WMAX; ++k)
            if (k < w) Q[k * rpb] = y[k];
      }
   }
   }
   __syncthreads();
   if (sn.bb >= 0 && tid < w) { const int rpb = (sn.r - sn.rb + 3) & ~3; bbarena[sn.bb + w * rpb + tid] = dk[tid]; }
   if (i >= w && i < nf) {
#pragma unroll
      for (int k = 0; k < WMAX; ++k)
         if (k < w) F[k * rp + (i - w)] = y[k];
   }
   for (int idx = tid; idx < w * (rp - r); idx += BLOCK) { const int k = idx / (rp - r); F[k * rp + r + (idx - k * (rp - r))] = 0.0; }
   __syncthreads();

   MF_STAMP(5);
   if (r > 0) {
      typedef double double2_t __attribute__((ext_vector_type(2)));
      const int nt = rp >> 2, ntb = (uc + 3) >> 2, ntiles = ntb * nt - ntb * (ntb - 1) / 2;
      for (int t = tid; t < ntiles; t += BLOCK) {
         const int tb = packed_col(t, nt), ta = tb + (t - (tb * nt - tb * (tb - 1) / 2));
         const int a0 = 4 * ta, b0 = 4 * tb;
         double acc[4][4];
#pragma unroll
         for (int x = 0; x < 4; ++x)
#pragma unroll
            for (int z = 0; z < 4; ++z) acc[x][z] = 0.0;
#pragma unroll 4
         for (int k = 0; k < w; ++k) {
            const double2_t* ca = (const double2_t*)(F + k * rp + a0);
            const double2_t* cb = (const double2_t*)(F + k * rp + b0);
            const double2_t a01 = ca[0], a23 = ca[1], b01 = cb[0], b23 = cb[1];
            const double d = dk[k];
            const double la[4] = {a01.x, a01.y, a23.x, a23.y};
            const double lb[4] = {b01.x * d, b01.y * d, b23.x * d, b23.y * d};
#pragma unroll
            for (int x = 0; x < 4; ++x)
#pragma unroll
               for (int z = 0; z < 4; ++z) acc[x][z] += la[x] * lb[z];
         }
#pragma unroll
         for (int z = 0; z < 4; ++z) {
            const int b = b0 + z;
            if (b < uc) {
               double* ub = FU + cu(b) - b;
#pragma unroll
               for (int x = 0; x < 4; ++x) {
                  const int a = a0 + x;
                  if (a < r && a >= b) { if (UG) ub[a] -= acc[x][z]; else lds_add(ub + a, -acc[x][z]); }
               }
            }
         }
      }
   }
   __syncthreads();

   MF_STAMP(6);
   if (np == 0) { MF_STAMP(7); return; }
   if (!UG) {
      double* Ug = uarena + sn.U;
      for (int idx = tid; idx < np; idx += BLOCK) Ug[idx] = FU[idx];
   }
   MF_STAMP(7);
}


__global__ __launch_bounds__(256) void k_root_assemble(const int* __restrict__ blk_list, const int* __restrict__ root_off,
                                                      const int* __restrict__ roots, const SnDesc* __restrict__ sns,
                                                      const BlkDesc* __restrict__ blks, const int* __restrict__ rowidx,
                                                      const int* __restrict__ bmap, double* __restrict__ arena,
                                                      const double* __restrict__ uarena, double* __restrict__ SC, int ldSC,
                                                      const int* __restrict__ sctab, double* __restrict__ gbuf, long long gstride,
                                                      const int* __restrict__ blk_group, int nt, int ns) {
   __shared__ int s_b0[256], s_b1[256], s_r[256], s_rb[256];
   __shared__ long long s_rows[256], s_U[256];
   const int blk = blk_list ? blk_list[blockIdx.x] : blockIdx.x;
   const BlkDesc bd = blks[blk];
   double* T = arena + bd.T_in;
   const int* bm = bmap + bd.bmap_off;
   const int n = bd.n, n_head = bd.n_head, c = blockIdx.y;
   double* S_ = gbuf ? gbuf + gstride * blk_group[blk] : SC;
   const bool tail_chunk = c < nt;
   if (!tail_chunk && (!S_ || bd.mf_split)) return;
   int lo, hi;
   if (tail_chunk) {
      const int cw = (bd.m_pad + nt - 1) / nt;
      lo = n_head + c * cw; hi = min(lo + cw, n);
   } else {
      const int cw = (bd.nb + ns - 1) / ns;
      lo = n + (c - nt) * cw; hi = min(lo + cw, n + bd.nb);
   }
   if (lo >= hi) return;
   const int q_begin = root_off[blk], q_end = root_off[blk + 1];
   for (int q0 = q_begin; q0 < q_end; q0 += 256) {
      const int nq = min(256, q_end - q0);
      __syncthreads();
      if ((int)threadIdx.x < nq) {
         const SnDesc sn = sns[roots[q0 + threadIdx.x]];
         const int* rows = rowidx + sn.rows;
         int a = 0, b = sn.r;
         while (a < b) { const int m = (a + b) >> 1; if (rows[m] < lo) a = m + 1; else b = m; }
         const int b0 = a;
         b = sn.r;
         while (a < b) { const int m = (a + b) >> 1; if (rows[m] < hi) a = m + 1; else b = m; }
         s_b0[threadIdx.x] = b0; s_b1[threadIdx.x] = a; s_r[threadIdx.x] = sn.r; s_rb[threadIdx.x] = sn.rb;
         s_rows[threadIdx.x] = sn.rows; s_U[threadIdx.x] = sn.U;
      }
      __syncthreads();
      for (int k = 0; k < nq; ++k) {
         const int b0 = s_b0[k], b1 = s_b1[k];
         if (b0 >= b1) continue;
         const int rb = s_rb[k], r = bd.mf_split == 2 ? rb : s_r[k];
         const int* rows = rowidx + s_rows[k];
         const double* U = uarena + s_U[k];
         const int per0 = r - b0, total = (b1 - b0) * per0;
         for (int idx = threadIdx.x; idx < total; idx += 256) {
            const int bi = idx / per0, a = b0 + (idx - bi * per0), b = b0 + bi;
            if (a < b) continue;
            const double u = U[b * r - b * (b - 1) / 2 + a - b];
            const int ra = rows[a], cb = rows[b];
            if (b < rb) {
               const int tr = ra < n ? ra - n_head : bd.m_pad + (ra - n);
               T[tr + (long long)(cb - n_head) * bd.ldT] += u;
            } else {
               double* tgt = sc_entry(S_, ldSC, bm, sctab, bd.sctab_off, bd.nb, ra - n, cb - n);
               if (gbuf) *tgt += u; else atomic_add_f64(tgt, u);
            }
         }
         __syncthreads();
      }
   }
}

constexpr int BR_IDMAX = 192;
constexpr int BR_PCHUNK = 64;
struct BrPair { long long panel, bb, rows; int wC, nbc, ldC, ns, b0, pad; };
template <int BLOCK, int WMAX>
__global__ __launch_bounds__(BLOCK) void k_border_rows(const int* __restrict__ list, const SnDesc* __restrict__ sns, const BlkDesc* __restrict__ blks,
                                                       const int* __restrict__ rowidx, const int* __restrict__ rec, const long long* __restrict__ rec_off,
                                                       double* __restrict__ arena, const double* __restrict__ fin, const double* __restrict__ bval) {
   extern __shared__ __attribute__((aligned(16))) double br_X[];
   constexpr int NW = BLOCK / 64;
   __shared__ short map[BR_IDMAX], kq[NW * WMAX];
   __shared__ double ljj[WMAX * WMAX], dj[WMAX], dl[NW * WMAX * WMAX];
   __shared__ BrPair pd[BR_PCHUNK];
   const int tid = threadIdx.x, lane = tid & 63, wave = tid >> 6;
   const int jid = list[blockIdx.x];
   const SnDesc J = sns[jid];
   const int* H = rec + rec_off[jid];
   const int bn = blks[J.blk].n;
   const long long b_off = blks[J.blk].b_off;
   const int w = J.w, nbj = J.r - J.rb, rp = (nbj + 3) & ~3;
   const int n_pairs = H[0], n_ent = H[1];
   double* X = br_X;
   for (int p = tid; p < n_pairs && p < BR_PCHUNK; p += BLOCK) {
      const int seg = H[3 + 2 * p], b0 = seg & 0xffff;
      const SnDesc C = sns[H[2 + 2 * p]];
      pd[p] = BrPair{C.panel + C.w + b0, C.bb, C.rows, C.w, C.r - C.rb, C.ld, (seg >> 16) - b0, b0, C.rb};
   }
   for (int idx = tid; idx < w * rp; idx += BLOCK) X[idx] = 0.0;
   for (int g = tid; g < BR_IDMAX; g += BLOCK) map[g] = -1;
   {
      const double* PJ = fin + J.panel;
      for (int idx = tid; idx < w * w; idx += BLOCK) {
         const int k = idx / w, j = idx - k * w;
         ljj[k * WMAX + j] = k > j ? PJ[k + (long long)j * J.ld] : 0.0;
      }
      if (tid < w) dj[tid] = PJ[tid + (long long)tid * J.ld];
   }
   __syncthreads();
   for (int a = tid; a < nbj; a += BLOCK) map[rowidx[J.rows + J.rb + a] - bn] = (short)a;
   {
      const int* E = H + 2 + 2 * n_pairs;
      const double* bv = bval + b_off;
      for (int e = tid; e < n_ent; e += BLOCK) {
         const int ak = E[2 * e];
         X[(ak >> 16) * rp + (ak & 0xffff)] = bv[E[2 * e + 1]];
      }
   }
   __syncthreads();
   double* dlw = dl + wave * (WMAX * WMAX);
   short* kqw = kq + wave * WMAX;
   for (int p0 = 0; p0 < n_pairs; p0 += BR_PCHUNK) {
      if (p0 > 0) {
         __syncthreads();
         for (int p = p0 + tid; p < n_pairs && p < p0 + BR_PCHUNK; p += BLOCK) {
            const int seg = H[3 + 2 * p], b0 = seg & 0xffff;
            const SnDesc C = sns[H[2 + 2 * p]];
            pd[p - p0] = BrPair{C.panel + C.w + b0, C.bb, C.rows, C.w, C.r - C.rb, C.ld, (seg >> 16) - b0, b0, C.rb};
         }
         __syncthreads();
      }
      const int pn = n_pairs - p0 < BR_PCHUNK ? n_pairs - p0 : BR_PCHUNK;
      for (int p = wave; p < pn; p += NW) {
         const BrPair P = pd[p];
         const int wC = P.wC, nbc = P.nbc, rpC = (nbc + 3) & ~3, ns = P.ns, w4 = (wC + 3) & ~3;
         const double* PC = fin + P.panel;
         const double* LbC = fin + P.bb;
         for (int idx = lane; idx < ns * w4; idx += 64) {
            const int c = idx / ns, qi = idx - c * ns;
            dlw[qi * WMAX + c] = c < wC ? PC[qi + (long long)c * P.ldC] : 0.0;
         }
         if (lane < ns) kqw[lane] = (short)(rowidx[P.rows + P.b0 + lane] - J.c0);
         __builtin_amdgcn_fence(__ATOMIC_ACQ_REL, "wavefront");
         __builtin_amdgcn_wave_barrier();
         for (int t = lane; t < nbc; t += 64) {
            const int aj = map[rowidx[P.rows + P.pad + t] - bn];
            double lbd[WMAX];
#pragma unroll
            for (int c = 0; c < WMAX; ++c) {
               const int cc = c < wC ? c : wC - 1;
               const double v = LbC[cc * rpC + t] * LbC[wC * rpC + cc];
               lbd[c] = c < wC ? v : 0.0;
            }
// ... 2378 lines not shown
```

### pips-ipmpp_amd/csrc/layout.cpp

```cpp
#include "layout.h"

#include <algorithm>
#include <climits>
#include <cmath>
#include <thread>
#include <type_traits>
#include <utility>

namespace pips {

static inline long long mf_unp(const BlockSym& bs, const HeadSupernode& s) {
   const long long uc = bs.mf_split ? s.rb : s.r, r = mf_rows(bs, s);
   return uc * r - uc * (uc - 1) / 2;
}

FrontLds front_lds(const BlockSym& bs, int l) {
   const HeadSupernode& s = bs.sn[l];
   const long long w = s.w, r = mf_rows(bs, s), nf = w + r;
   FrontLds f;
   f.panel = std::max<long long>(w * nf - w * (w - 1) / 2, w * ((r + 3) / 4 * 4));
   f.upd = mf_unp(bs, s);
   f.extra = 0;
   if (l < (int)bs.mf_meta.size() && bs.mf_meta[l] >= 0) {
      const int* H = bs.mf_int.data() + bs.mf_meta[l];
// ... 415 lines not shown
      if (h_list.empty()) h_list.push_back(0);
      if (h_tail.empty()) h_tail.push_back(0);
   }
   return PIPS_OK;
}

void layout_spine_lists(const std::vector<BlockSym>& sym, const std::vector<std::vector<int>>& sorted_id, int lstar, BatchLayout& o) {
   const int nblk = (int)sym.size();
   o.h_spine_off.assign(nblk + 1, 0);
   for (int b = 0; b < nblk; ++b) {
      for (int l = 0; l < (int)sym[b].sn.size(); ++l)
         if (sym[b].sn[l].level >= lstar) o.h_spine.push_back(sorted_id[b][l]);
      o.h_spine_off[b + 1] = (int)o.h_spine.size();
   }
   o.spine_total = (int)o.h_spine.size();
}

void layout_tail_single(const std::vector<BlockSym>& sym, const LayoutKnobs& knobs, BatchLayout& o) {
   const int nblk = (int)sym.size();
   long long scratch = 0;
   for (int b = 0; b < nblk; ++b) scratch += sym[b].arena - sym[b].T_off;
   const double need = 8.0 * (double)(o.arena_total + o.bb_doubles + scratch + o.uarena_total) + 4e9;
   const int want_single = knobs.tail_single >= 0 ? knobs.tail_single : (nblk <= 16 ? 1 : 0);
   o.tail_single = o.mf && !knobs.deterministic && scratch > 0 && want_single != 0 && need < (double)(size_t)knobs.free_device_bytes;
   o.tail_scratch = o.tail_single ? scratch : 0;
   long long at = o.arena_total + o.bb_doubles;
   for (int b = 0; b < nblk; ++b) {
      o.h_blks[b].T_in = o.tail_single ? at : o.h_blks[b].T;
      at += sym[b].arena - sym[b].T_off;
   }
}

int layout_index_arrays(const std::vector<BlockInput>& in, const std::vector<BlockSym>& sym, const std::vector<std::vector<int>>& sorted_id,
                        const Bases& B, BatchLayout& o) {
   const int nblk = (int)in.size();
   const bool mf = o.mf;
   const std::vector<long long>&kptr = o.kptr, &x_off = o.x_off;
   o.h_upd.reserve(B.upd_base[nblk]);
   o.h_psign_off.assign(nblk, 0); o.h_perm_off.assign(nblk, 0);
   o.h_kdst.assign(o.nnzK_total, 0); o.h_bdst.assign(o.nnzB_total, 0); o.h_kdiag.assign(o.n_total, 0); o.h_rowbase.assign(o.n_total, 0);
   o.h_krowptr.assign(o.n_total + 1, 0); o.h_kcolidx.assign(o.nnzK_total, 0);
   o.h_rowidx.reserve(B.rows_base[nblk]);
   o.h_sncol.reserve(B.sncol);
   for (int b = 0; b < nblk; ++b) {
      const BlockSym& s = sym[b];
      o.h_rowidx.insert(o.h_rowidx.end(), s.rowidx.begin(), s.rowidx.end());
      o.h_upd.insert(o.h_upd.end(), s.upd.begin(), s.upd.end());
      for (int c = 0; c < s.n_head; ++c) o.h_sncol.push_back(sorted_id[b][s.sn_of_col[c]]);
      o.h_bmap.insert(o.h_bmap.end(), s.bmap.begin(), s.bmap.end());
      o.h_psign_off[b] = (long long)o.h_psign.size();
      o.h_psign.insert(o.h_psign.end(), s.psign.begin(), s.psign.end());
      o.h_perm_off[b] = (long long)o.h_perm.size();
      o.h_perm.insert(o.h_perm.end(), s.perm.begin(), s.perm.end());
      auto dst = [&](long long rel) { return rel >= s.T_off ? o.h_blks[b].T_in + (rel - s.T_off) : o.h_blks[b].arena_off + rel; };
      for (size_t p = 0; p < s.a_dst.size(); ++p) o.h_kdst[kptr[b] + p] = (mf && s.a_front[p]) ? -1 : dst(s.a_dst[p]);
      for (size_t p = 0; p < s.b_dst.size(); ++p) o.h_bdst[B.bptr[b] + p] = (mf && s.b_front[p]) ? -1 : dst(s.b_dst[p]);
      for (int i = 0; i < s.n; ++i) {
         long long dp = -1;
         for (int p = in[b].krow[i]; p < in[b].krow[i + 1]; ++p)
            if (in[b].kcol[p] == i) dp = kptr[b] + p;
         if (dp < 0) PIPS_FAIL(PIPS_ERR_ARG, "block %d row %d has no explicit diagonal entry (create_kkt always stores one)", b, i);
         o.h_kdiag[x_off[b] + i] = dp;
         o.h_rowbase[x_off[b] + i] = x_off[b];
         o.h_krowptr[x_off[b] + i] = (int)(kptr[b] + in[b].krow[i]);
      }
      std::copy(in[b].kcol.begin(), in[b].kcol.end(), o.h_kcolidx.begin() + kptr[b]);
   }
   o.h_krowptr[o.n_total] = (int)o.nnzK_total;
   if (mf) {
      o.h_mfint.assign((size_t)B.mfint_base[nblk], 0);
      for (int b = 0; b < nblk; ++b) {
         const BlockSym& s = sym[b];
         std::copy(s.mf_int.begin(), s.mf_int.end(), o.h_mfint.begin() + B.mfint_base[b]);
         for (int64_t pos : s.mf_fix) o.h_mfint[(size_t)(B.mfint_base[b] + pos)] = sorted_id[b][s.mf_int[(size_t)pos]];
      }
   }
   o.h_nprimal.resize(nblk);
   for (int b = 0; b < nblk; ++b) o.h_nprimal[b] = in[b].n_primal;
   o.tile_first.resize(nblk);
   for (int b = 0; b < nblk; ++b) o.tile_first[b] = &sym[b].tile_first;
   return PIPS_OK;
}

void layout_full_rows(const std::vector<BlockInput>& in, const std::vector<BlockSym>& sym, BatchLayout& o) {
   const int nblk = (int)in.size();
   const std::vector<long long>&kptr = o.kptr, &x_off = o.x_off;
   std::vector<int>& frp = o.h_frowptr;
   frp.assign(o.n_total + 1, 0);
   for (int b = 0; b < nblk; ++b)
      for (int i = 0; i < sym[b].n; ++i)
         for (int p = in[b].krow[i]; p < in[b].krow[i + 1]; ++p) {
            const int j = in[b].kcol[p];
            ++frp[x_off[b] + i + 1];
            if (j != i) ++frp[x_off[b] + j + 1];
         }
   for (long long r = 0; r < o.n_total; ++r) frp[r + 1] += frp[r];
   std::vector<int>&fcol = o.h_fcol, &fsrc = o.h_fsrc;
   fcol.assign(frp[o.n_total], 0); fsrc.assign(frp[o.n_total], 0);
   std::vector<int> fill(frp.begin(), frp.end() - 1);
   for (int b = 0; b < nblk; ++b)
      for (int i = 0; i < sym[b].n; ++i)
         for (int p = in[b].krow[i]; p < in[b].krow[i + 1]; ++p) {
            const int j = in[b].kcol[p], src = (int)(kptr[b] + p);
            int q = fill[x_off[b] + i]++;
            fcol[q] = j; fsrc[q] = src;
            if (j != i) { q = fill[x_off[b] + j]++; fcol[q] = i; fsrc[q] = src; }
         }
   for (long long r = 0; r < o.n_total; ++r)
      if (frp[r + 1] - frp[r] > FULL_LONG_ROW) o.h_flong.push_back(r);
   o.n_flong = (int)o.h_flong.size();
}

void layout_border_csr(const std::vector<BlockInput>& in, int S, const Bases& B, BatchLayout& o) {
   const int nblk = (int)in.size();
   std::vector<int>&h_bt_rowptr = o.h_bt_rowptr, &h_bt_colidx = o.h_bt_colidx, &h_bt_rowsc = o.h_bt_rowsc;
   std::vector<long long>& h_bt_xoff = o.h_bt_xoff;
   h_bt_colidx.assign(o.nnzB_total, 0);
   o.h_bval.assign(o.nnzB_total, 0.0);
   h_bt_rowptr.push_back(0);
   for (int b = 0; b < nblk; ++b) {
      if (in[b].btrow.empty()) continue;
      for (int s2 = 0; s2 < S; ++s2) {
         h_bt_rowptr.push_back((int)(B.bptr[b] + in[b].btrow[s2 + 1]));
         h_bt_rowsc.push_back(s2);
         h_bt_xoff.push_back(o.x_off[b]);
      }
      std::copy(in[b].btcol.begin(), in[b].btcol.end(), h_bt_colidx.begin() + B.bptr[b]);
      std::copy(in[b].btval.begin(), in[b].btval.end(), o.h_bval.begin() + B.bptr[b]);
   }
   o.bt_rows_total = (long long)h_bt_rowsc.size();
   o.h_bt_rownnz.assign((size_t)o.bt_rows_total, 0);
   for (long long i = 0; i < o.bt_rows_total; ++i) o.h_bt_rownnz[(size_t)i] = h_bt_rowptr[i + 1] - h_bt_rowptr[i];
   for (int b = 0; b < nblk; ++b)
      if (!in[b].btrow.empty()) o.h_bt_rowblk.insert(o.h_bt_rowblk.end(), (size_t)S, b);
   {
      std::vector<char> used(std::max(S, 1), 0);
      for (int b = 0; b < nblk; ++b)
         if (!in[b].btrow.empty())
            for (int s2 = 0; s2 < S; ++s2)
               if (in[b].btrow[s2 + 1] > in[b].btrow[s2]) used[s2] = 1;
      o.h_schur_slot.assign(std::max(S, 1), -1);
      for (int s2 = 0; s2 < S; ++s2)
         if (used[s2]) { o.h_schur_slot[s2] = (int)o.schur_cols.size(); o.schur_cols.push_back(s2); }
   }
   if (o.bt_rows_total > 0 && o.nnzB_total > 0 && o.nnzB_total < (1LL << 31)) {
      std::vector<int>&rp = o.h_br_rowptr, &sc = o.h_br_sc, &src = o.h_br_src;
      rp.assign((size_t)o.n_total + 1, 0);
      for (long long r = 0; r < o.bt_rows_total; ++r)
         for (int p = h_bt_rowptr[r]; p < h_bt_rowptr[r + 1]; ++p) ++rp[h_bt_xoff[r] + h_bt_colidx[p] + 1];
      for (long long i = 0; i < o.n_total; ++i) rp[i + 1] += rp[i];
      sc.assign((size_t)o.nnzB_total, 0); src.assign((size_t)o.nnzB_total, 0);
      std::vector<int> fill(rp.begin(), rp.end() - 1);
      for (long long r = 0; r < o.bt_rows_total; ++r)
         for (int p = h_bt_rowptr[r]; p < h_bt_rowptr[r + 1]; ++p) {
            const int q = fill[h_bt_xoff[r] + h_bt_colidx[p]]++;
            sc[q] = h_bt_rowsc[r]; src[q] = p;
         }
   }
}

void layout_leaf_gather(BatchLayout& o) {
   const std::vector<SnDesc>& h_sns = o.h_sns;
   const std::vector<BlkDesc>& h_blks = o.h_blks;
   const std::vector<int>& h_rowidx = o.h_rowidx;
   const long long xw_total = o.xw_total;
   if (!o.levels.empty())
// ... 12 lines not shown
         int r_in = 0;
         while (r_in < sn.r && h_rowidx[sn.rows + r_in] < bd.n) ++r_in;
         h_leaf[i] = LeafDesc{sn.panel, (int)sn.rows, (int)bd.xw_off, sn.c0, r_in};
      }
      std::vector<int> cnt((size_t)xw_total + 1, 0);
      long long nent = 0;
      for (int i = L0->simple_begin; i < L0->simple_begin + L0->simple_cnt; ++i) {
         const SnDesc& sn = h_sns[i];
         const BlkDesc& bd = h_blks[sn.blk];
         for (int a = 0; a < sn.r; ++a) {
            const int ra = h_rowidx[sn.rows + a];
            if (ra >= bd.n) break;
            ++cnt[bd.xw_off + ra];
            ++nent;
         }
      }
      if (nent > 0 && nent < (1LL << 31)) {
         std::vector<int>&h_rows = o.h_lf_rows, &h_ptr = o.h_lf_ptr, &h_src = o.h_lf_src, &h_pos = o.h_lf_pos;
         h_ptr.assign(1, 0); h_src.assign((size_t)nent, 0); h_pos.assign(h_rowidx.size(), -1);
         std::vector<int> slot((size_t)xw_total, -1);
         for (long long t = 0; t < xw_total; ++t)
            if (cnt[t] > 0) { slot[t] = (int)h_rows.size(); h_rows.push_back((int)t); h_ptr.push_back(h_ptr.back() + cnt[t]); }
         std::vector<int> fill(h_ptr.begin(), h_ptr.end() - 1);
         for (int i = L0->simple_begin; i < L0->simple_begin + L0->simple_cnt; ++i) {
            const SnDesc& sn = h_sns[i];
            const BlkDesc& bd = h_blks[sn.blk];
            for (int a = 0; a < sn.r; ++a) {
               const int ra = h_rowidx[sn.rows + a];
               if (ra >= bd.n) break;
               const int q = fill[slot[bd.xw_off + ra]]++;
               h_src[q] = (int)(bd.xw_off + sn.c0);
               h_pos[sn.rows + a] = q;
            }
         }
         o.lf_rows = (long long)h_rows.size(); o.lf_entries = nent;
      }
   }
}

void layout_sweep_decisions(const std::vector<BlockSym>& sym, const LayoutKnobs& knobs, BatchLayout& o) {
   double fwd_entries = 0.0, border_entries = 0.0;
   int ntc_max = 0;
   for (const BlkDesc& bd : o.h_blks) ntc_max = std::max(ntc_max, bd.ntc);
   for (const BlockSym& sb : sym) {
      fwd_entries += 0.5 * (double)sb.m_pad * sb.m_pad;
      border_entries += (double)sb.nb_pad * sb.m_pad;
      for (const HeadSupernode& sn : sb.sn) {
         const int nbord = sn.r - sn.rb;
         fwd_entries += (double)sn.w * (sn.r - nbord) + 0.5 * sn.w * sn.w;
         border_entries += (double)sn.w * nbord;
      }
   }
   o.fwd_entries = fwd_entries; o.border_entries = border_entries;
   const bool sweep_enabled = ntc_max > 0 && !knobs.sweep_launches;
   const bool deterministic = knobs.deterministic;
   o.border_backward_ok = o.schur_mode_eff == 1 && o.nnzB_total > 0 && (sweep_enabled || ntc_max == 0) && !deterministic && border_entries <= 3.0 * fwd_entries;
   if (knobs.border_backward >= 0)
      o.border_backward_ok = knobs.border_backward != 0 && o.schur_mode_eff == 1 && o.nnzB_total > 0 && sweep_enabled && !deterministic;
   const bool aug_paths = o.schur_mode_eff == 1 && o.nnzB_total > 0 && (sweep_enabled || ntc_max == 0) && o.spine_total == 0;
   o.aug_sweeps_ok = aug_paths && border_entries <= 3.0 * fwd_entries;
   if (knobs.aug_sweeps >= 0) o.aug_sweeps_ok = knobs.aug_sweeps != 0 && aug_paths;
}

}

int build_batch_layout(const std::vector<BlockInput>& in, const std::vector<BlockSym>& sym, int S, const LayoutKnobs& knobs,
                       BatchLayout& out) {
   out = BatchLayout();
   out.mf = knobs.mf;
   out.schur_mode_eff = knobs.schur_mode_eff;
   Bases B;
   int rc, nlev = 0;
   if ((rc = layout_offsets(in, sym, out.mf, out, B))) return rc;
   const std::vector<Key> keys = layout_sort_keys(sym, out.mf, knobs.mf_lds_doubles, out.nsn_total, nlev);
   out.n_levels_all = nlev;
   const int lstar = layout_spine_cut(sym, nlev, knobs);
   std::vector<std::vector<int>> sorted_id, roots_of;
   layout_supernodes(sym, keys, nlev, lstar, B, out, sorted_id, roots_of);
   if (out.mf) layout_roots_and_batches(sym, sorted_id, roots_of, out);
   if ((rc = layout_konly(sym, sorted_id, out))) return rc;
   layout_spine_lists(sym, sorted_id, lstar, out);
   layout_tail_single(sym, knobs, out);
   if ((rc = layout_index_arrays(in, sym, sorted_id, B, out))) return rc;
   layout_full_rows(in, sym, out);
   layout_border_csr(in, S, B, out);
   layout_leaf_gather(out);
   layout_sweep_decisions(sym, knobs, out);
   return PIPS_OK;
}

#define LAYOUT_REQUIRE(cond, ...) \
   do { if (!(cond)) PIPS_FAIL(PIPS_ERR_STATE, "layout invariant " __VA_ARGS__); } while (0)

int check_batch_layout(const std::vector<BlockInput>& in, const std::vector<BlockSym>& sym, int S, const LayoutKnobs& knobs,
                       const BatchLayout& o) {
   const int nblk = (int)in.size();
   (void)S;
   auto scratch_of = [&](int b) { return sym[b].arena - sym[b].T_off; };
   for (int b = 0; b < nblk; ++b) {
      const BlkDesc& d = o.h_blks[b];
      const bool last = b + 1 == nblk;
      const BlockSym& s = sym[b];
      LAYOUT_REQUIRE(d.arena_off >= 0 && d.arena_off + s.arena <= (last ? o.arena_total : o.h_blks[b + 1].arena_off), "1: arena region of block %d", b);
      LAYOUT_REQUIRE(d.U + (long long)s.m_pad * s.m_pad <= (last ? o.uarena_total : o.h_blks[b + 1].U), "1: U-arena region of block %d", b);
      LAYOUT_REQUIRE(d.xw_off + s.n_head + s.m_pad + s.nb_pad <= (last ? o.xw_total : o.h_blks[b + 1].xw_off), "1: work-vector region of block %d", b);
      LAYOUT_REQUIRE(d.winv_off + (long long)d.ntc * TILE * TILE <= (last ? o.winv_total : o.h_blks[b + 1].winv_off), "1: winv region of block %d", b);
      LAYOUT_REQUIRE(d.dt_off + s.m_pad <= (last ? o.dtail_total : o.h_blks[b + 1].dt_off), "1: dtail region of block %d", b);
      if (!o.tail_single) LAYOUT_REQUIRE(d.T_in == d.T, "1: T_in of block %d differs from T without the single-launch tails", b);
      else {
         const long long end = last ? o.arena_total + o.bb_doubles + o.tail_scratch : o.h_blks[b + 1].T_in;
         LAYOUT_REQUIRE(d.T_in >= o.arena_total + o.bb_doubles && d.T_in + scratch_of(b) <= end, "1: scratch region of block %d", b);
      }
   }
   std::vector<long long> sn_base(nblk + 1, 0);
   for (int b = 0; b < nblk; ++b) sn_base[b + 1] = sn_base[b] + (long long)sym[b].sn.size();
   LAYOUT_REQUIRE((long long)o.h_sns.size() == sn_base[nblk] && o.nsn_total == (int)sn_base[nblk], "2: %zu supernode records", o.h_sns.size());
   std::vector<int> loc_of(o.h_sns.size()), level_of(o.h_sns.size()), sorted_of((size_t)sn_base[nblk], -1);
   for (size_t i = 0; i < o.h_sns.size(); ++i) {
      const SnDesc& sn = o.h_sns[i];
      LAYOUT_REQUIRE(sn.blk >= 0 && sn.blk < nblk && sn.c0 >= 0 && sn.c0 < sym[sn.blk].n_head, "2: supernode %zu names no head column", i);
      const int loc = sym[sn.blk].sn_of_col[sn.c0];
      LAYOUT_REQUIRE(sorted_of[(size_t)(sn_base[sn.blk] + loc)] < 0, "2: supernode %d of block %d appears twice in the sorted order", loc, sn.blk);
      sorted_of[(size_t)(sn_base[sn.blk] + loc)] = (int)i;
      loc_of[i] = loc; level_of[i] = sym[sn.blk].sn[loc].level;
      LAYOUT_REQUIRE(i == 0 || level_of[i - 1] <= level_of[i], "2: supernode %zu breaks the order by level", i);
      const int par = sym[sn.blk].sn_parent.empty() ? -1 : sym[sn.blk].sn_parent[loc];
      LAYOUT_REQUIRE(par < 0 || sym[sn.blk].sn[par].level > level_of[i], "2: head parent of supernode %zu is not on a higher level", i);
   }
   {
      int pos = 0;
      const int nl = (int)(o.levels.size() + o.levels_top.size());
      LAYOUT_REQUIRE(nl == o.n_levels_all, "2: %d level ranges for %d levels", nl, o.n_levels_all);
      for (int l = 0; l < nl; ++l) {
         const LevelRange& L = l < (int)o.levels.size() ? o.levels[l] : o.levels_top[l - (int)o.levels.size()];
         std::pair<int, int> rg[3] = {{L.simple_begin, L.simple_cnt}, {L.small_begin, L.small_cnt}, {L.large_begin, L.large_cnt}};
         std::sort(rg, rg + 3, [](auto& a, auto& b) { return (a.second > 0 ? a.first : INT_MAX) < (b.second > 0 ? b.first : INT_MAX); });
         for (auto& r : rg) {
            if (r.second <= 0) continue;
            LAYOUT_REQUIRE(r.first == pos, "2: ranges of level %d overlap or leave a gap at supernode %d", l, pos);
            pos += r.second;
         }
         LAYOUT_REQUIRE(pos <= o.nsn_total && (pos == 0 || level_of[pos - 1] <= l) && (pos == o.nsn_total || level_of[pos] > l), "2: ranges of level %d do not hold the level", l);
      }
      LAYOUT_REQUIRE(pos == o.nsn_total, "2: level ranges cover %d of %d supernodes", pos, o.nsn_total);
   }
   if (o.mf) {
      std::vector<char> covered(o.h_sns.size(), 0);
      for (const MfLaunch& m : o.mf_launches) {
         LAYOUT_REQUIRE(m.begin >= 0 && m.cnt > 0 && m.begin + m.cnt <= o.nsn_total && m.lds_doubles <= MF_LDS_MAX, "3: front launch at %d (%d fronts, %d doubles of LDS)", m.begin, m.cnt, m.lds_doubles);
         for (int i = m.begin; i < m.begin + m.cnt; ++i) {
            const BlockSym& bs = sym[o.h_sns[i].blk];
            const HeadSupernode& s = bs.sn[loc_of[i]];
            LAYOUT_REQUIRE(!covered[i] && !is_simple(s) && level_of[i] == m.level, "3: supernode %d in a second launch, simple, or on another level", i);
            covered[i] = 1;
            const FrontLds f = front_lds(bs, loc_of[i]);
            const long long nf = s.w + mf_rows(bs, s);
            LAYOUT_REQUIRE(m.lds_doubles >= f.doubles(knobs.mf_lds_doubles), "3: launch of front %d has %d doubles of LDS, the front needs %lld", i, m.lds_doubles, f.doubles(knobs.mf_lds_doubles));
            const bool admits = m.cls >= 6 ? (!f.resident(knobs.mf_lds_doubles) && (m.cls == 7 || nf <= 256))
                                           : (f.resident(knobs.mf_lds_doubles) && (m.cls % 3 != 0 || nf <= 64) && (m.cls / 3 != 0 || s.w <= 16));
            LAYOUT_REQUIRE(admits && nf <= MF_MAX_FRONT, "3: class %d does not admit front %d (w %d, %lld rows)", m.cls, i, s.w, nf);
         }
      }
      for (size_t i = 0; i < o.h_sns.size(); ++i)
         LAYOUT_REQUIRE((covered[i] != 0) == !is_simple(sym[o.h_sns[i].blk].sn[loc_of[i]]), "3: front %zu is in no launch", i);
   } else
      LAYOUT_REQUIRE(o.mf_launches.empty() && o.n_bb == 0, "3: front launches without the multifrontal head");
// ... 5 lines not shown
            const BbBatch& c = o.h_bb_batches[q];
            LAYOUT_REQUIRE(c.cnt >= 1 && c.cnt <= BB_GMAX && c.ndoubles <= o.bb_stage && c.npos <= o.bb_poscap, "4: batch %d holds %d supernodes, %d doubles, %d rows", q, c.cnt, c.ndoubles, c.npos);
            LAYOUT_REQUIRE(c.src == at && sym[b].mf_split, "4: batch %d of block %d is not contiguous with the one before", q, b);
            at += c.ndoubles;
            for (int p = 0; p < c.npos; ++p) {
               const int pos = o.h_bb_pos[(size_t)(c.pos + p)];
               LAYOUT_REQUIRE(pos >= 0 && pos < sym[b].nb, "4: batch %d stages border row %d of %d", q, pos, sym[b].nb);
            }
         }
      LAYOUT_REQUIRE(at == o.arena_total + o.bb_doubles, "4: batches hold %lld of %lld doubles", at - o.arena_total, o.bb_doubles);
      std::vector<std::pair<long long, long long>> reg;
      for (const SnDesc& sn : o.h_sns)
         if (sn.bb >= 0) reg.push_back({sn.bb, (long long)sn.w * ((sn.r - sn.rb + 3) & ~3) + ((sn.w + 1) & ~1)});
      std::sort(reg.begin(), reg.end());
      for (size_t i = 0; i < reg.size(); ++i)
         LAYOUT_REQUIRE(reg[i].first >= o.arena_total && reg[i].first + reg[i].second <= (i + 1 < reg.size() ? reg[i + 1].first : o.arena_total + o.bb_doubles), "4: border-row regions overlap or leave the arena");
      BbPlanSize z; z.stage = o.bb_stage; z.poscap = o.bb_poscap; z.nbmax = o.bb_nbmax;
      LAYOUT_REQUIRE(bb_fits(z), "4: %zu bytes of LDS for k_border_schur", bb_lds_bytes(z));
   }
   std::vector<long long> bptr(nblk + 1, 0);
   for (int b = 0; b < nblk; ++b) bptr[b + 1] = bptr[b] + (long long)in[b].btcol.size();
   for (int b = 0; b < nblk; ++b) {
      const BlkDesc& d = o.h_blks[b];
      auto inside = [&](long long t) {
         return t == -1 || (t >= d.arena_off && t < d.arena_off + sym[b].arena) || (o.tail_single && t >= d.T_in && t < d.T_in + scratch_of(b));
      };
      for (long long p = o.kptr[b]; p < o.kptr[b + 1]; ++p) LAYOUT_REQUIRE(inside(o.h_kdst[(size_t)p]), "5: entry %lld of K leaves block %d", p, b);
      for (long long p = bptr[b]; p < bptr[b + 1]; ++p) LAYOUT_REQUIRE(inside(o.h_bdst[(size_t)p]), "5: border entry %lld leaves block %d", p, b);
      for (int i = 0; i < sym[b].n; ++i) {
         const long long dp = o.h_kdiag[(size_t)(o.x_off[b] + i)];
         LAYOUT_REQUIRE(dp >= o.kptr[b] + in[b].krow[i] && dp < o.kptr[b] + in[b].krow[i + 1] && o.h_kcolidx[(size_t)dp] == i, "5: diagonal position of row %d of block %d", i, b);
      }
   }
   LAYOUT_REQUIRE((long long)o.h_fcol.size() == 2 * o.nnzK_total - o.n_total && o.h_fsrc.size() == o.h_fcol.size(), "5: two-triangle structure holds %zu entries", o.h_fcol.size());
   {
      std::vector<int> row_of((size_t)o.nnzK_total);
      for (long long r = 0; r < o.n_total; ++r)
         for (int p = o.h_krowptr[(size_t)r]; p < o.h_krowptr[(size_t)r + 1]; ++p) row_of[(size_t)p] = (int)(r - o.h_rowbase[(size_t)r]);
      for (long long r = 0; r < o.n_total; ++r)
         for (int q = o.h_frowptr[(size_t)r]; q < o.h_frowptr[(size_t)r + 1]; ++q) {
            const int src = o.h_fsrc[(size_t)q], i = row_of[(size_t)src], j = o.h_kcolidx[(size_t)src], me = (int)(r - o.h_rowbase[(size_t)r]), c = o.h_fcol[(size_t)q];
            LAYOUT_REQUIRE((me == i && c == j) || (me == j && c == i), "5: entry %d of the two-triangle row %lld maps to (%d, %d)", q, r, i, j);
         }
   }
   if (!o.h_br_rowptr.empty()) {
      std::vector<int> btrow_of((size_t)o.nnzB_total);
      for (long long r = 0; r < o.bt_rows_total; ++r)
         for (int p = o.h_bt_rowptr[(size_t)r]; p < o.h_bt_rowptr[(size_t)r + 1]; ++p) btrow_of[(size_t)p] = (int)r;
      std::vector<char> seen((size_t)o.nnzB_total, 0);
      LAYOUT_REQUIRE(o.h_br_rowptr[(size_t)o.n_total] == o.nnzB_total, "6: the border by leaf row holds %d of %lld entries", o.h_br_rowptr[(size_t)o.n_total], o.nnzB_total);
      for (long long i = 0; i < o.n_total; ++i)
         for (int q = o.h_br_rowptr[(size_t)i]; q < o.h_br_rowptr[(size_t)i + 1]; ++q) {
            const int p = o.h_br_src[(size_t)q];
            LAYOUT_REQUIRE(p >= 0 && p < o.nnzB_total && !seen[(size_t)p], "6: border entry %d taken twice", p);
            seen[(size_t)p] = 1;
            const int r = btrow_of[(size_t)p];
            LAYOUT_REQUIRE(o.h_bt_xoff[(size_t)r] + o.h_bt_colidx[(size_t)p] == i && o.h_bt_rowsc[(size_t)r] == o.h_br_sc[(size_t)q], "6: border entry %d sits in another leaf row or Schur column", p);
         }
   }
   if (o.lf_entries > 0) {
      std::vector<char> seen((size_t)o.lf_entries, 0);
      const LevelRange& L0 = o.levels[0];
      long long n_seen = 0;
      for (int i = L0.simple_begin; i < L0.simple_begin + L0.simple_cnt; ++i) {
         const SnDesc& sn = o.h_sns[i];
         bool in_block = true;
         for (int a = 0; a < sn.r; ++a) {
            in_block = in_block && o.h_rowidx[(size_t)(sn.rows + a)] < o.h_blks[sn.blk].n;
            const int q = o.h_lf_pos[(size_t)(sn.rows + a)];
            LAYOUT_REQUIRE(in_block ? (q >= 0 && q < o.lf_entries && !seen[(size_t)q]) : q == -1, "6: gather position of row %d of leaf %d", a, i);
            if (in_block) { seen[(size_t)q] = 1; ++n_seen; }
         }
      }
      LAYOUT_REQUIRE(n_seen == o.lf_entries, "6: %lld of %lld gather positions are taken", n_seen, o.lf_entries);
   }
   return PIPS_OK;
}

void BatchLayout::drop_uploaded() {
   auto drop = [](auto&... v) { (std::decay_t<decltype(v)>().swap(v), ...); };
   drop(h_rowidx, h_sncol, h_bmap, h_perm, h_upd, h_mfint, h_nprimal, h_psign, h_psign_off, h_perm_off, h_kdst, h_bdst, h_kdiag, h_rowbase,
        h_krowptr, h_kcolidx, h_frowptr, h_fcol, h_fsrc, h_flong, h_bt_rowptr, h_bt_colidx, h_bt_xoff, h_bval, h_br_rowptr, h_br_sc, h_br_src,
        h_schur_slot, h_leafdesc, h_lf_rows, h_lf_ptr, h_lf_src, h_lf_pos, h_lb_list, tile_first, h_roots, h_bb_batches, h_bb_meta, h_bb_pos,
        h_kb_rec, h_kb_list, h_kb_tail, h_kb_off, h_spine, h_spine_off);
}

}

extern "C" int pips_schur_pack_probe(int nblk, int S, const int* const* bt_rowptr, int* nb, int* nb_max, int* const* local_of_row) {
   if (nblk <= 0 || S < 0 || !bt_rowptr || !nb || !nb_max || !local_of_row) PIPS_FAIL(pips::PIPS_ERR_ARG, "pips_schur_pack_probe: bad arguments");
   *nb_max = 0;
   for (int b = 0; b < nblk; ++b) {
      if (!local_of_row[b]) PIPS_FAIL(pips::PIPS_ERR_ARG, "pips_schur_pack_probe: local_of_row[%d] is NULL", b);
      nb[b] = pips::schur_pack_block(S, bt_rowptr[b], local_of_row[b]);
      *nb_max = std::max(*nb_max, nb[b]);
   }
   return pips::PIPS_OK;
}
```

### pips-ipmpp_amd/csrc/layout.h

```cpp
#pragma once
#include <cstdint>
#include <string>
#include <vector>

#include "common.h"
#include "records.h"

namespace pips {

struct BlockInput {
   int n = 0, n_primal = -1;
   std::vector<int> krow, kcol;
   std::vector<int> btrow, btcol;
   std::vector<double> btval;
};

struct LevelRange {
   int simple_begin, simple_cnt, small_begin, small_cnt, large_begin, large_cnt;
   int small_lds = 0, large_lds = 0;
};

struct MfLaunch { int level, cls, begin, cnt, lds_doubles; };
constexpr long long MF_LDS_MAX = 20352;

inline bool is_simple(const HeadSupernode& s) { return s.w == 1 && s.r <= SIMPLE_RMAX && s.level == 0; }
inline int mf_rows(const BlockSym& bs, const HeadSupernode& s) { return bs.mf_konly ? s.rb : s.r; }

struct FrontLds {
   long long panel, upd, extra;
   bool resident(long long lds_budget) const { return panel + upd + 8 <= lds_budget; }
   long long doubles(long long lds_budget) const { return panel + (resident(lds_budget) ? upd : 0) + 8 + extra; }
};
FrontLds front_lds(const BlockSym& bs, int l);
int mf_class(const BlockSym& bs, int l, long long lds_budget);

struct BbPlanSize { int stage = 3072, poscap = 0, nbmax = 0; bool two_per_cu = false; };
BbPlanSize bb_plan_size(const std::vector<BlockSym>& sym);
size_t bb_lds_bytes(const BbPlanSize& z);
inline bool bb_fits(const BbPlanSize& z) { return bb_lds_bytes(z) <= 160 * 1024 && z.poscap <= 4 * 512 && z.stage <= 2 * 6 * 512; }

struct LayoutKnobs {
   bool deterministic = false;
   int schur_mode = 0;
   bool mf_wanted = true;
   long long mf_lds_doubles = 19200;
   int spine = -1;
   int tail_single = -1;
   int border_backward = -1, aug_sweeps = -1;
   bool sweep_launches = false;
   long long free_device_bytes = 0;
   bool mf = false;
   int schur_mode_eff = 1;
};

struct SchurPack {
   std::vector<int> nb;
   std::vector<long long> off;
   std::vector<int> cols;
   int nb_max = 0;
   const int* block_cols(int b) const { return cols.data() + off[b]; }
};
int schur_pack_block(int S, const int* bt_rowptr, int* local_of_row);
void build_schur_pack(const std::vector<BlockInput>& in, int S, SchurPack& out);
struct PackRows {
   std::vector<int> la;
   std::vector<long long> tabrow;
};
int schur_pack_rows(const std::vector<BlockInput>& in, int S, const std::vector<long long>& off, long long tab_size, PackRows& out);

struct BatchLayout {
   bool mf = false;
   int schur_mode_eff = 1;
   std::vector<BlkDesc> h_blks;
   std::vector<long long> kptr;
   std::vector<long long> x_off;
   long long n_total = 0, nnzK_total = 0, nnzB_total = 0, arena_total = 0, xw_total = 0, bt_rows_total = 0, uarena_total = 0;
   long long winv_total = 0, dtail_total = 0;
   long long mfU_total = 0, mfLV_total = 0;
   int nsn_total = 0;
   std::vector<SnDesc> h_sns;
   std::vector<LevelRange> levels;
   std::vector<LevelRange> levels_top;
   std::vector<MfLaunch> mf_launches;
   int spine_total = 0, n_levels_all = 0;
   int head_wcap = HEAD_WMAX;
   long long slots_total = 0, vslots_total = 0;
   std::vector<int> h_roots, h_root_off;
   int n_roots = 0;
   std::vector<BbBatch> h_bb_batches;
   std::vector<BbMeta> h_bb_meta;
   std::vector<int> h_bb_pos, h_bb_off;
   int n_bb = 0;
   long long bb_doubles = 0;
   int bb_stage = 3072, bb_nbmax = 0, bb_poscap = 0;
   bool bb_two_per_cu = false;
   bool kb_any = false;
   std::vector<int> h_kb_rec, h_kb_list, h_kb_tail;
   std::vector<long long> h_kb_off;
   std::vector<int> kb_level_off;
   std::vector<int> kb_level_pairs, kb_level_lds;
   int n_kb_tail = 0;
   std::vector<int> h_spine, h_spine_off;
   bool tail_single = false;
   long long tail_scratch = 0;
   std::vector<int> schur_cols;
   std::vector<int> h_bt_rowsc, h_bt_rownnz, h_bt_rowblk;
   int n_flong = 0;
   long long lf_rows = 0, lf_entries = 0;
   int n_lb = 0, nb_pad_max = 0;
   bool border_backward_ok = false, aug_sweeps_ok = false;
   double fwd_entries = 0.0, border_entries = 0.0;
   std::vector<int> h_rowidx, h_sncol, h_bmap, h_perm, h_upd, h_mfint, h_nprimal;
   std::vector<signed char> h_psign;
   std::vector<long long> h_psign_off, h_perm_off, h_kdst, h_bdst, h_kdiag, h_rowbase;
   std::vector<int> h_krowptr, h_kcolidx;
   std::vector<int> h_frowptr, h_fcol, h_fsrc;
   std::vector<long long> h_flong;
   std::vector<int> h_bt_rowptr, h_bt_colidx;
   std::vector<long long> h_bt_xoff;
   std::vector<double> h_bval;
   std::vector<int> h_br_rowptr, h_br_sc, h_br_src;
   std::vector<int> h_schur_slot;
   std::vector<LeafDesc> h_leafdesc;
   std::vector<int> h_lf_rows, h_lf_ptr, h_lf_src, h_lf_pos;
   std::vector<int> h_lb_list;
   std::vector<const std::vector<int>*> tile_first;
   void drop_uploaded();
};

int analyze_blocks(const std::vector<BlockInput>& in, int S, const AnalyzeOptions& opt, int n_threads, bool with_border, std::vector<BlockSym>& sym);
bool blocked_solves_cheaper(const std::vector<BlockSym>& sym, int S, const AnalyzeOptions& opt);
bool fronts_fit(const std::vector<BlockSym>& sym, const AnalyzeOptions& opt);
bool border_split_must_go(const std::vector<BlockSym>& sym, bool mf);
int analyze_symbolic(const std::vector<BlockInput>& in, int S, int n_threads, AnalyzeOptions& opt, LayoutKnobs& knobs, std::vector<BlockSym>& sym);

int build_batch_layout(const std::vector<BlockInput>& in, const std::vector<BlockSym>& sym, int S, const LayoutKnobs& knobs,
                       BatchLayout& out);
int check_batch_layout(const std::vector<BlockInput>& in, const std::vector<BlockSym>& sym, int S, const LayoutKnobs& knobs,
                       const BatchLayout& lay);

}
```

### pips-ipmpp_amd/csrc/records.h

```cpp
#pragma once
#include <stdint.h>

#ifdef __HIPCC__
#define PIPS_HD __host__ __device__
#else
#define PIPS_HD
#endif

namespace pips {

constexpr int TILE = 128;

struct SnDesc {
   long long panel;
   long long rows;
   long long upd;
   int w, r, c0, blk;
   int n_useg, rb;
   int ld, pad_;
   long long slot;
   long long vslot;
   long long U;
   long long mf;
   long long bb;
};

struct BlkDesc {
   long long arena_off;
   long long T;
   long long sncol_off;
   long long xw_off;
   long long x_off;
   long long bmap_off;
   long long winv_off;
   long long dt_off;
   long long sctab_off;
   int n, n_head, m, m_pad, nb, nb_pad, ldT, ntc, ntr;
   int mf_split;
   long long U;
   double thr_rel, repl_rel;
   double repl_abs;
   long long lv_off;
   long long k_off, b_off;
   long long T_in;
};

struct TileTask { int blk, ti, tj, pad; };
struct TileStrip { int off, cnt; };

constexpr int HEAD_WMAX = 32;
constexpr int SIMPLE_RMAX = 16;

constexpr int BB_GMAX = 8;
constexpr int BB_TR = 4;
PIPS_HD inline int bb_tile_count(int rp) {
   const int nt4 = rp >> 2;
   if (BB_TR == 4) return nt4 * (nt4 + 1) / 2;
   const int nt8 = (rp + 7) >> 3;
   int cnt = 0;
   for (int tb = 0; tb < nt4; ++tb) cnt += nt8 - (tb >> 1);
   return cnt;
}
struct BbMeta { int lt_off, pos_off, w, nbj, tile0, pad0, pad1, pad2; };
struct BbBatch {
   long long src;
   long long pos;
   int first, cnt;
   int ndoubles, ntiles, npos, pad;
};

struct LeafDesc {
   long long panel;
   int rows;
   int xoff;
   int c0;
   int r_in;
};

struct BgEntry { long long off; unsigned y; unsigned short stride, w; };

constexpr int FULL_LONG_ROW = 512;

static_assert(sizeof(SnDesc) == 96 && sizeof(BlkDesc) == 176 && sizeof(TileTask) == 16, "record layout read by the kernels");
static_assert(sizeof(BbMeta) == 32 && sizeof(BbBatch) == 40 && sizeof(LeafDesc) == 24 && sizeof(BgEntry) == 16, "record layout read by the kernels");

}
```

### pips-ipmpp_amd/python/capi.py

```python
import ctypes as C
import sys
import os

import numpy as np

try:
    import torch
except Exception:
    torch = None

_HERE = os.path.dirname(os.path.abspath(__file__))
LIB_PATH = os.environ.get("PIPS_HIP_LIBRARY") or os.path.join(os.path.dirname(_HERE), "libpipship.so")


class PipsHipError(RuntimeError):
    pass


def _load():
    if not os.path.exists(LIB_PATH):
        raise PipsHipError(
            f"{LIB_PATH} is missing: build it with `python -c 'import __graft_entry__ as g; g.build()'` "
            "(hipcc --offload-arch=gfx950). The MI355X backend has no CPU fallback.")
    return C.CDLL(LIB_PATH, mode=C.RTLD_GLOBAL)


lib = _load()

_i32p = np.ctypeslib.ndpointer(dtype=np.int32, flags="C_CONTIGUOUS")
_f64p = np.ctypeslib.ndpointer(dtype=np.float64, flags="C_CONTIGUOUS")
_i64p = np.ctypeslib.ndpointer(dtype=np.int64, flags="C_CONTIGUOUS")
_vp = C.c_void_p

lib.pips_hip_last_error.restype = C.c_char_p
lib.pips_hip_device_count.restype = C.c_int
lib.pips_hip_host_wait_count.restype = C.c_longlong
lib.pips_hip_device_allocs_live.restype = C.c_longlong
lib.pips_hip_device_bytes_live.restype = C.c_longlong

SYMBOLS = [
    "pips_hip_last_error", "pips_hip_device_count",
    "pips_hip_ldl_create", "pips_hip_ldl_set_inertia_hint", "pips_hip_ldl_set_pivot_rule", "pips_hip_ldl_set_refinement", "pips_hip_ldl_set_refinement_backward_error", "pips_hip_ldl_set_deterministic",
    "pips_hip_ldl_analyze", "pips_hip_ldl_factor", "pips_hip_ldl_set_values", "pips_hip_ldl_solve", "pips_hip_ldl_inertia", "pips_hip_ldl_info",
    "pips_hip_ldl_get_perm", "pips_hip_ldl_set_border", "pips_hip_ldl_factor_schur", "pips_hip_ldl_destroy",
    "pips_hip_ldl_solve_dev", "pips_hip_ldl_solve_sparse", "pips_hip_ldl_factor_schur_batch", "pips_hip_ldl_solve_batch", "pips_hip_ldl_solve_batch_dev",
    "pips_hip_ldl_inertia_batch", "pips_hip_ldl_factor_schur_sparse", "pips_hip_ldl_factor_schur_sparse_batch",
    "pips_hip_dense_ldl_create", "pips_hip_dense_ldl_factor", "pips_hip_dense_ldl_factor_dev", "pips_hip_dense_ldl_solve",
    "pips_hip_dense_ldl_solve_dev", "pips_hip_dense_ldl_inertia", "pips_hip_dense_ldl_info", "pips_hip_dense_ldl_set_pivoting", "pips_hip_dense_ldl_set_distributed", "pips_hip_dense_ldl_destroy", "pips_root_plan_build", "pips_layout_probe", "pips_tail_plan_probe", "pips_ipm_layout_probe", "pips_hip_host_wait_count", "pips_hip_host_wait_sites", "pips_hip_device_allocs_live", "pips_hip_device_bytes_live",
    "pips_hip_batch_create", "pips_hip_batch_set_block", "pips_hip_batch_set_options", "pips_hip_batch_set_schur_mode", "pips_hip_batch_set_deterministic", "pips_hip_batch_get_schur_mode", "pips_hip_batch_add_regularization", "pips_hip_batch_set_refinement",
    "pips_hip_batch_last_refinement_steps", "pips_hip_batch_set_refinement_backward_error",
    "pips_hip_batch_last_refinement_measure", "pips_hip_batch_analyze",
    "pips_hip_batch_set_values", "pips_hip_batch_set_diagonals_dev", "pips_hip_batch_set_diagonals", "pips_hip_batch_factor",
    "pips_hip_batch_solve_dev", "pips_hip_batch_solve", "pips_hip_batch_border_tmult_dev", "pips_hip_batch_border_mult_dev",
    "pips_hip_batch_inertia", "pips_hip_batch_tail_to_host", "pips_hip_batch_info", "pips_hip_batch_sync", "pips_hip_batch_set_timing",
    "pips_hip_batch_get_timing", "pips_hip_batch_destroy",
    "pips_hip_kkt_create", "pips_hip_kkt_create_sparse", "pips_hip_kkt_get_schur_sparse", "pips_hip_kkt_sparse_root_info", "pips_hip_kkt_factorize", "pips_hip_kkt_set_root_regularization", "pips_hip_kkt_solve_compressed", "pips_hip_kkt_get_schur",
    "pips_hip_kkt_set_root_inequalities", "pips_hip_kkt_set_zdiag0_dev", "pips_hip_kkt_set_root_hessian",
    "pips_hip_kkt_root_inertia", "pips_hip_kkt_get_timing", "pips_hip_kkt_last_ltsolve_from_factor", "pips_hip_kkt_last_solve_path", "pips_hip_kkt_set_solve_check", "pips_hip_kkt_solve_check_counts", "pips_hip_kkt_set_solve_graph", "pips_hip_kkt_set_root_stream", "pips_hip_kkt_solve_graph_stats", "pips_hip_kkt_set_root_pivoting", "pips_hip_kkt_destroy",
    "pips_hip_malloc", "pips_hip_free", "pips_hip_memcpy_h2d", "pips_hip_memcpy_d2h", "pips_hip_memset",
    "pips_hip_comm_unique_id", "pips_hip_comm_create", "pips_hip_comm_create_external", "pips_hip_comm_set_external_rsag", "pips_hip_comm_set_external_broadcast", "pips_hip_broadcast", "pips_hip_comm_has_broadcast", "pips_hip_allreduce_sum_rsag", "pips_hip_all_gather", "pips_hip_comm_size", "pips_hip_allreduce_sum", "pips_hip_comm_destroy",
    "pips_hip_vec_axpy", "pips_hip_vec_axpby", "pips_hip_vec_scale", "pips_hip_vec_copy", "pips_hip_vec_set",
    "pips_hip_vec_add_const", "pips_hip_vec_mul", "pips_hip_vec_div", "pips_hip_vec_add_product", "pips_hip_vec_add_quotient",
    "pips_hip_vec_divide_some", "pips_hip_vec_select_nonzeros", "pips_hip_vec_safe_invert", "pips_hip_vec_gondzio_projection", "pips_hip_vec_dot",
    "pips_hip_vec_one_norm", "pips_hip_vec_inf_norm", "pips_hip_vec_min", "pips_hip_vec_sumsq_scaled", "pips_hip_vec_stepbound",
    "pips_hip_vec_find_blocking", "pips_hip_vec_weighted_stepbounds", "pips_hip_vec_dot_shifted", "pips_ipm_create", "pips_ipm_create_rank", "pips_ipm_create_general", "pips_ipm_create_general_scaled", "pips_ipm_create_qp", "pips_ipm_hessian_mult", "pips_ipm_get_scaling", "pips_ipm_get_dims", "pips_ipm_get_iterate", "pips_ipm_get_stats2", "pips_ipm_get_schur_mode", "pips_ipm_mult", "pips_ipm_outer_solve", "pips_ipm_solve", "pips_ipm_set_gondzio", "pips_ipm_set_option", "pips_ipm_set_free_variables", "pips_ipm_get_solution", "pips_ipm_get_trace", "pips_ipm_get_stats", "pips_ipm_destroy",
    "pips_gdx_read_block", "pips_gdx_block_counts", "pips_gdx_block_vector", "pips_gdx_block_matrix", "pips_gdx_block_destroy",
    "pips_gen_row_nnz", "pips_gen_block", "pips_gen_root", "pips_gen_diagonal", "pips_kkt_leaf_assemble",
    "pips_border_assemble", "pips_symbolic_probe", "pips_symbolic_probe_hubs", "pips_map_children_to_ranks", "pips_schur_pack_probe", "pips_det_plan_probe", "pips_schur_target_probe",
]

PIPS_SCALER_NONE = 0
PIPS_SCALER_EQUILIBRIUM = 1
PIPS_SCALER_GEOMETRIC_MEAN = 2
PIPS_SCALER_GEOMETRIC_MEAN_EQUILIBRIUM = 3
PIPS_SCALER_CURTIS_REID = 4
SCALERS = {None: PIPS_SCALER_NONE, "none": PIPS_SCALER_NONE, "equilibrium": PIPS_SCALER_EQUILIBRIUM, "geometric": PIPS_SCALER_GEOMETRIC_MEAN,
           "geometric_equilibrium": PIPS_SCALER_GEOMETRIC_MEAN_EQUILIBRIUM, "curtis_reid": PIPS_SCALER_CURTIS_REID}


def _check(rc, what):
    if rc != 0:
        msg = lib.pips_hip_last_error()
        raise PipsHipError(f"{what} failed (code {rc}): {msg.decode() if msg else '?'}")


def device_count():
    return int(lib.pips_hip_device_count())


def host_wait_count():
    return int(lib.pips_hip_host_wait_count())


def device_allocs_live():
    return int(lib.pips_hip_device_allocs_live())


def device_bytes_live():
    return int(lib.pips_hip_device_bytes_live())


def host_wait_sites():
    buf = C.create_string_buffer(16384)
    lib.pips_hip_host_wait_sites(buf, 16384)
    out = {}
    for ln in buf.value.decode().splitlines():
        k, v = ln.rsplit(" ", 1)
        out[k] = int(v)
    return out


def _ptr(a):
    if a is None:
        return None
    if isinstance(a, (int, np.integer)):
        return C.c_void_p(int(a))
    if torch is not None and isinstance(a, torch.Tensor):
        return C.c_void_p(a.data_ptr())
    return a.ctypes.data_as(C.c_void_p)


def _i32(a):
    return np.ascontiguousarray(a, dtype=np.int32)


def _f64(a):
    return np.ascontiguousarray(a, dtype=np.float64)


class Csr:

# ... 406 lines not shown
        self.n[b] = K.nrows
        _check(lib.pips_hip_batch_set_block(self._h, C.c_int(b), C.c_int(K.nrows), C.c_int(n_primal), _ptr(K.rowptr),
                                            _ptr(K.colidx), _ptr(Bt.rowptr) if Bt is not None else None,
                                            _ptr(Bt.colidx) if Bt is not None else None,
                                            _ptr(Bt.val) if Bt is not None else None), "pips_hip_batch_set_block")

    def set_options(self, force_n_head=-1, refine_steps=-1, thr_rel=-1.0, repl_rel=-1.0):
        _check(lib.pips_hip_batch_set_options(self._h, C.c_int(force_n_head), C.c_int(refine_steps), C.c_double(thr_rel),
                                              C.c_double(repl_rel)), "pips_hip_batch_set_options")

    def add_regularization(self, primal, dual):
        _check(lib.pips_hip_batch_add_regularization(self._h, C.c_double(primal), C.c_double(dual)), "add_regularization")

    def set_refinement(self, max_steps, tol):
        _check(lib.pips_hip_batch_set_refinement(self._h, C.c_int(max_steps), C.c_double(tol)), "pips_hip_batch_set_refinement")

    def set_refinement_backward_error(self, max_steps, tol):
        _check(lib.pips_hip_batch_set_refinement_backward_error(self._h, C.c_int(max_steps), C.c_double(tol)),
               "pips_hip_batch_set_refinement_backward_error")

    def last_refinement_measure(self):
        lib.pips_hip_batch_last_refinement_measure.restype = C.c_double
        return float(lib.pips_hip_batch_last_refinement_measure(self._h))

    def last_refinement_steps(self):
        return int(lib.pips_hip_batch_last_refinement_steps(self._h))

    def analyze(self, n_threads=8):
        _check(lib.pips_hip_batch_analyze(self._h, C.c_int(n_threads)), "pips_hip_batch_analyze")

    def set_values(self, b, vals):
        _check(lib.pips_hip_batch_set_values(self._h, C.c_int(b), _ptr(_f64(vals))), "pips_hip_batch_set_values")

    def set_schur_mode(self, mode):
        _check(lib.pips_hip_batch_set_schur_mode(self._h, C.c_int(mode)), "pips_hip_batch_set_schur_mode")

    def set_deterministic(self, on=True):
        _check(lib.pips_hip_batch_set_deterministic(self._h, C.c_int(1 if on else 0)), "pips_hip_batch_set_deterministic")

    def schur_mode(self):
        m = C.c_int()
        _check(lib.pips_hip_batch_get_schur_mode(self._h, C.byref(m)), "pips_hip_batch_get_schur_mode")
        return m.value

    def set_diagonals(self, diag):
        if torch is not None and isinstance(diag, torch.Tensor):
            _check(lib.pips_hip_batch_set_diagonals_dev(self._h, _ptr(diag)), "pips_hip_batch_set_diagonals_dev")
        else:
            _check(lib.pips_hip_batch_set_diagonals(self._h, _ptr(_f64(diag))), "pips_hip_batch_set_diagonals")

    def factor(self, SC_dev=None, ldSC=0):
        _check(lib.pips_hip_batch_factor(self._h, _ptr(SC_dev), C.c_int(ldSC)), "pips_hip_batch_factor")

    def solve(self, x):
        if torch is not None and isinstance(x, torch.Tensor):
            _check(lib.pips_hip_batch_solve_dev(self._h, _ptr(x)), "pips_hip_batch_solve_dev")
        else:
            assert x.dtype == np.float64 and x.flags.c_contiguous
            _check(lib.pips_hip_batch_solve(self._h, _ptr(x)), "pips_hip_batch_solve")
        return x

    def border_tmult(self, z_dev, b0_dev, alpha):
        _check(lib.pips_hip_batch_border_tmult_dev(self._h, _ptr(z_dev), _ptr(b0_dev), C.c_double(alpha)), "border_tmult")

    def border_mult(self, x0_dev, t_dev, alpha):
        _check(lib.pips_hip_batch_border_mult_dev(self._h, _ptr(x0_dev), _ptr(t_dev), C.c_double(alpha)), "border_mult")

    def inertia(self, b):
        p, n, z = C.c_int(), C.c_int(), C.c_int()
        _check(lib.pips_hip_batch_inertia(self._h, C.c_int(b), C.byref(p), C.byref(n), C.byref(z)), "batch inertia")
        return p.value, n.value, z.value

    def tail_to_host(self, b, which):
        w = {"panel": 0, "U": 1, "d": 2}[which]
        dims = (C.c_int * 4)()
        _check(lib.pips_hip_batch_tail_to_host(self._h, C.c_int(b), C.c_int(w), None, C.c_int64(0), dims), "pips_hip_batch_tail_to_host")
        m, m_pad, nb, ldT = (int(v) for v in dims)
        shape = {0: (m_pad, ldT), 1: (m_pad, m_pad), 2: (m_pad,)}[w]
        out = np.zeros(shape, np.float64)
        _check(lib.pips_hip_batch_tail_to_host(self._h, C.c_int(b), C.c_int(w), _ptr(out), C.c_int64(out.size), dims), "pips_hip_batch_tail_to_host")
        return (out.T if w < 2 else out), (m, m_pad, nb, ldT)

    def info(self):
        what = np.zeros(27, np.int64)
        _check(lib.pips_hip_batch_info(self._h, _ptr(what), C.c_int(27)), "pips_hip_batch_info")
        keys = ["nnzL", "n", "n_head", "m", "n_sn", "n_levels", "flops_factor", "flops_border", "arena_bytes", "ntc", "upd_table_bytes", "nb", "nnzK",
                "ltsolve_from_augmented_factor", "multifrontal_head", "max_front", "update_matrix_bytes", "fronts_in_device_memory", "nnzL_head", "head_row_indices",
                "nnzL_border", "augmented_sweeps", "augmented_passes", "tail_border_entries", "blocks_with_border_split", "blocks_with_k_only_fronts",
                "packed_schur_rhs"]
        return {k: int(v) for k, v in zip(keys, what)}

    def sync(self):
        _check(lib.pips_hip_batch_sync(self._h), "pips_hip_batch_sync")

    def set_timing(self, on=True):
        _check(lib.pips_hip_batch_set_timing(self._h, C.c_int(1 if on else 0)), "set_timing")

    def get_timing(self):
        ms = np.zeros(16)
        cnt = np.zeros(16, np.int64)
        _check(lib.pips_hip_batch_get_timing(self._h, _ptr(ms), _ptr(cnt), C.c_int(16)), "get_timing")
        names = ["scatter", "head", "tail_update", "tail_diag", "tail_trsm", "schur", "total", "solve_permute", "solve_head_fwd", "solve_tail",
                 "solve_head_bwd", "solve_refine"]
        return {k: (float(ms[i]), int(cnt[i])) for i, k in enumerate(names)}

    def close(self):
        if self._h:
            lib.pips_hip_batch_destroy(self._h)
            self._h = C.c_void_p()

    def __del__(self):
        try:
            self.close()
        except Exception:
            pass


class Comm:

    def __init__(self, id_bytes, n_ranks, rank, device):
        self._h = C.c_void_p()
        buf = (C.c_char * 128).from_buffer_copy(id_bytes)
        _check(lib.pips_hip_comm_create(C.byref(self._h), buf, C.c_int(n_ranks), C.c_int(rank), C.c_int(device)),
               "pips_hip_comm_create")

    @staticmethod
    def unique_id():
        buf = (C.c_char * 128)()
        _check(lib.pips_hip_comm_unique_id(buf), "pips_hip_comm_unique_id")
        return bytes(buf)

    def allreduce_sum(self, t, n=None, stream=None):
        n = t.numel() if n is None else n
        _check(lib.pips_hip_allreduce_sum(self._h, _ptr(t), C.c_size_t(n), _ptr(stream)), "pips_hip_allreduce_sum")

    def broadcast(self, t, root, n=None, stream=None):
        n = t.numel() if n is None else n
        _check(lib.pips_hip_broadcast(self._h, _ptr(t), C.c_size_t(n), C.c_int(root), _ptr(stream)), "pips_hip_broadcast")

    def has_broadcast(self):
        return bool(lib.pips_hip_comm_has_broadcast(self._h))

    def close(self):
        if self._h:
            lib.pips_hip_comm_destroy(self._h)
            self._h = C.c_void_p()


_ALLREDUCE_CB = C.CFUNCTYPE(C.c_int, C.c_void_p, C.c_void_p, C.c_size_t)


class _DeviceDoubles:

    def __init__(self, ptr, n):
        self.__cuda_array_interface__ = {"shape": (int(n),), "typestr": "<f8", "data": (int(ptr), False), "version": 2}


class ExternalComm(Comm):

    def __init__(self, allreduce, reduce_scatter=None, all_gather=None, n_ranks=1, rank=0):
        def _cb(_user, ptr, n):
            try:
                allreduce(int(ptr), int(n))
                return 0
            except Exception as e:
                sys.stderr.write(f"external all-reduce failed: {e}\n")
                return 1

        self._cb = _ALLREDUCE_CB(_cb)
        self._h = C.c_void_p()
        _check(lib.pips_hip_comm_create_external(C.byref(self._h), self._cb, None), "pips_hip_comm_create_external")
        if reduce_scatter is not None and all_gather is not None:
# ... 530 lines not shown
```

Before: 8.470 64-block work units/s (1 factorize + 4 solveCompressed).

## Add first-touch tail column assembly kernel behind an environment flag

```diff
diff --git a/include/pips_hip.h b/include/pips_hip.h
--- a/include/pips_hip.h
+++ b/include/pips_hip.h
@@ -253,6 +253,10 @@
                          int S, const int* const* bt_rowptr, const int* const* bt_colidx, int force_n_head,
                          int* col_tasks, long long col_cap, int* grp_tasks, long long grp_cap, int64_t* counts);
 
+int pips_first_touch_probe(int nblk, const int* n, const int* n_primal, const int* const* krow, const int* const* kcol,
+                           int S, const int* const* bt_rowptr, const int* const* bt_colidx, int force_n_head, int deterministic,
+                           long long lds_bytes, long long free_device_bytes, long long* out, long long cap, int64_t* counts);
+
 int pips_det_plan_probe(int nblk, const int* n, const int* n_primal, const int* const* krow, const int* const* kcol,
                         int S, const int* const* bt_rowptr, const int* const* bt_colidx, int rank, int n_ranks, int n_panels,
                         long long* out, long long cap, int64_t* counts);
diff --git a/pips-ipmpp_amd/csrc/engine.hip b/pips-ipmpp_amd/csrc/engine.hip
--- a/pips-ipmpp_amd/csrc/engine.hip
+++ b/pips-ipmpp_amd/csrc/engine.hip
@@ -761,6 +761,10 @@
    DevBuf<double> d_mfU;
    DevBuf<double> d_mfLV;
    DevBuf<int> d_roots, d_root_off;
+   DevBuf<long long> d_ft_colbase;
+   DevBuf<int> d_ft_init_off, d_ft_piece_off, d_ft_leaves;
+   DevBuf<FtInit> d_ft_init;
+   DevBuf<FtPiece> d_ft_piece;
    DevBuf<BbBatch> d_bb_batches;
    DevBuf<BbMeta> d_bb_meta;
    DevBuf<int> d_bb_off, d_bb_pos;
@@ -1089,6 +1093,16 @@
          PIPS_TRY(d_br_src.upload(h_br_src));
       }
       PIPS_TRY(d_nprimal.upload(h_nprimal));
+      if (tail_first_touch) {
+         if ((size_t)ft_ld_max * sizeof(double) > 64 * 1024)
+            HIP_TRY(hipFuncSetAttribute((const void*)k_tail_first_touch, hipFuncAttributeMaxDynamicSharedMemorySize, (int)(ft_ld_max * sizeof(double))));
+         PIPS_TRY(d_ft_colbase.upload(h_ft_colbase));
+         PIPS_TRY(d_ft_init_off.upload(h_ft_init_off));
+         PIPS_TRY(d_ft_init.upload(h_ft_init));
+         PIPS_TRY(d_ft_piece_off.upload(h_ft_piece_off));
+         PIPS_TRY(d_ft_piece.upload(h_ft_piece));
+         PIPS_TRY(d_ft_leaves.upload(h_ft_leaves));
+      }
       return PIPS_OK;
    }
 
@@ -1097,7 +1111,7 @@
       if (L.simple_cnt > 0)
          hipLaunchKernelGGL(k_head_factor_simple, dim3((L.simple_cnt + 255) / 256), dim3(256), 0, stream, d_sns, L.simple_begin,
                             L.simple_cnt, d_blks, d_rowidx, d_upd, d_psign, d_psign_off, d_bmap, d_arena, SC, ldSC, d_inertia, d_pref, d_sctab, sx,
-                            mf ? 1 : 0, d_mfLV, d_lf_pos, d_lf_val, d_arena);
+                            mf ? 1 : 0, d_mfLV, d_lf_pos, d_lf_val, d_arena, tail_first_touch ? 1 : 0);
       if (mf) return;
       if (L.small_cnt > 0)
          hipLaunchKernelGGL((k_head_factor<64, 8, 640>), dim3(L.small_cnt), dim3(64), (size_t)std::max(L.small_lds, 1) * sizeof(double), stream, d_sns,
@@ -1298,7 +1312,7 @@
       hipLaunchKernelGGL(k_block_absmax, dim3(std::max(1, std::min(64, (int)(nnzK_total / nblk / 4096))), nblk), dim3(256), 0, stream, d_kval,
                          d_kptr, d_blks);
       hipLaunchKernelGGL(k_block_absmax_finish, dim3((nblk + 255) / 256), dim3(256), 0, stream, d_blks, nblk, thr_rel, repl_rel);
-      hipLaunchKernelGGL(k_arena_clear, dim3(256, nblk), dim3(256), 0, stream, d_blks, d_arena, mf ? 1 : 0);
+      if (!tail_first_touch) hipLaunchKernelGGL(k_arena_clear, dim3(256, nblk), dim3(256), 0, stream, d_blks, d_arena, mf ? 1 : 0);
       HIP_TRY(hipMemsetAsync(d_inertia, 0, (size_t)3 * nblk * sizeof(int), stream));
       if (!d_gemm_ctr) PIPS_TRY(d_gemm_ctr.alloc((size_t)GEMM_CTR_SLOTS * 8));
       HIP_TRY(hipMemsetAsync(d_gemm_ctr, 0, (size_t)GEMM_CTR_SLOTS * 8 * sizeof(int), stream));
@@ -1307,13 +1321,19 @@
          hipLaunchKernelGGL(k_scatter, dim3(grid_for(nnzK_total, 256)), dim3(256), 0, stream, d_kdst, d_kval, d_arena, nnzK_total);
       if (nnzB_total > 0 && schur_mode_eff == 1)
          hipLaunchKernelGGL(k_scatter, dim3(grid_for(nnzB_total, 256)), dim3(256), 0, stream, d_bdst, d_bval, d_arena, nnzB_total);
-      hipLaunchKernelGGL(k_tail_pad_diag, dim3(nblk), dim3(128), 0, stream, d_blks, d_arena, nblk);
+      if (!tail_first_touch) hipLaunchKernelGGL(k_tail_pad_diag, dim3(nblk), dim3(128), 0, stream, d_blks, d_arena, nblk);
       hipLaunchKernelGGL(k_pref_rows, dim3(32, nblk), dim3(256), 0, stream, d_blks, d_kval, d_kdiag, d_res, d_nprimal, d_krowptr, d_kcolidx);
       hipLaunchKernelGGL(k_pref_init, dim3(32, nblk), dim3(256), 0, stream, d_blks, d_perm, d_perm_off, (const double*)d_res, d_pref);
       return PIPS_OK;
    }
    void launch_root_assemble(double* SC, int ldSC) {
       const int asm_half = std::max(1, std::min(32, 1024 / std::max(nblk, 1)));
+      if (tail_first_touch) {
+         if (SC && n_roots > 0)
+            hipLaunchKernelGGL(k_root_assemble, dim3(nblk, asm_half), dim3(256), 0, stream, (const int*)nullptr, d_root_off, d_roots, d_sns, d_blks, d_rowidx, d_bmap,
+                               d_arena, d_mfU, SC, ldSC, d_sctab, (double*)nullptr, 0LL, (const int*)nullptr, 0, asm_half);
+         return;
+      }
       if (deterministic && d_gbuf && SC && d_round_blk) {
          for (size_t k = 0; k + 1 < det.round_off.size(); ++k) {
             const int cnt = det.round_off[k + 1] - det.round_off[k];
@@ -1325,6 +1345,15 @@
          hipLaunchKernelGGL(k_root_assemble, dim3(nblk, 2 * asm_half), dim3(256), 0, stream, (const int*)nullptr, d_root_off, d_roots, d_sns, d_blks, d_rowidx, d_bmap,
                             d_arena, d_mfU, SC, ldSC, d_sctab, (double*)nullptr, 0LL, (const int*)nullptr, asm_half, asm_half);
    }
+   int launch_tail_first_touch(double* SC, int ldSC) {
+      const size_t lds = (size_t)ft_ld_max * sizeof(double);
+      hipLaunchKernelGGL(k_tail_first_touch, dim3(ft_cols_max, nblk), dim3(64), lds, stream, d_blks, d_ft_colbase, d_ft_init_off, d_ft_init, d_ft_piece_off,
+                         d_ft_piece, d_rowidx, d_kval, d_bval, d_mfU, d_arena);
+      if (n_ft_leaves > 0)
+         hipLaunchKernelGGL(k_leaf_products, dim3((n_ft_leaves + 255) / 256), dim3(256), 0, stream, d_ft_leaves, n_ft_leaves, d_sns, d_blks, d_rowidx, d_bmap,
+                            d_arena, SC, ldSC, d_sctab);
+      return PIPS_OK;
+   }
    int factor_head(double* SC, int ldSC) {
       const ScatterCtx sx = head_slots ? ScatterCtx{2, nullptr, d_slot_val, d_arena, SC} : sx_atomic();
       for (size_t li = 0; li < levels.size(); ++li) {
@@ -1341,6 +1370,7 @@
             gather(g_sc_grp, d_slot_val, d_gbuf);
          } else if (SC) gather(g_sc, d_slot_val, SC);
       }
+      if (tail_first_touch) { PhaseTimer::Scope phase(&timer, stream, 1); PIPS_TRY(launch_tail_first_touch(SC, ldSC)); }
       if (mf && n_roots > 0) { PhaseTimer::Scope phase(&timer, stream, 1); launch_root_assemble(SC, ldSC); }
       if (mf && d_kb_list) {
          PhaseTimer::Scope phase(&timer, stream, 1);
@@ -1939,6 +1969,8 @@
    opt.mf_konly = opt.mf_split_nb_max > 0 && !knobs.deterministic && opt.max_sn_width <= 16 && env_int("PIPS_HIP_MF_KONLY", 0) != 0;
    knobs.spine = env_flag("PIPS_HIP_SPINE");
    knobs.tail_single = env_flag("PIPS_HIP_TAIL_SINGLE");
+   knobs.tail_first_touch = env_flag("PIPS_HIP_TAIL_FIRST_TOUCH");
+   knobs.ft_lds_bytes = std::min(FT_LDS_MAX, std::max(0LL, (long long)env_int("PIPS_HIP_FIRST_TOUCH_LDS", (int)FT_LDS_BUDGET)));
    knobs.border_backward = env_flag("PIPS_HIP_BORDER_BACKWARD");
    knobs.aug_sweeps = env_flag("PIPS_HIP_AUG_SWEEPS");
    knobs.sweep_launches = getenv("PIPS_HIP_SWEEP_LAUNCHES") != nullptr;
@@ -2698,6 +2730,7 @@
    if (n_what > 24) { what[24] = 0; for (const BlockSym& s : e->sym) what[24] += s.mf_split ? 1 : 0; }
    if (n_what > 25) { what[25] = 0; for (const BlockSym& s : e->sym) what[25] += (e->mf && s.mf_konly) ? 1 : 0; }
    if (n_what > 26) what[26] = e->packed_rhs;
+   if (n_what > 27) what[27] = e->tail_first_touch ? 1 : 0;
    return PIPS_OK;
 }
 
@@ -3881,6 +3914,79 @@
    return PIPS_OK;
 }
 
+int pips_first_touch_probe(int nblk, const int* n, const int* n_primal, const int* const* krow, const int* const* kcol, int S,
+                           const int* const* bt_rowptr, const int* const* bt_colidx, int force_n_head, int deterministic, long long lds_bytes,
+                           long long free_device_bytes, long long* out, long long cap, int64_t* counts) {
+   std::vector<BlockInput> in;
+   PIPS_TRY(probe_inputs("pips_first_touch_probe", nblk, n, n_primal, krow, kcol, S, bt_rowptr, bt_colidx, in));
+   if (!counts || cap < 0 || (cap > 0 && !out)) PIPS_FAIL(PIPS_ERR_ARG, "pips_first_touch_probe: bad arguments");
+   AnalyzeOptions opt;
+   AnalyzeKnobs knobs;
+   read_layout_knobs(nullptr, opt, knobs);
+   if (deterministic) { knobs.deterministic = true; opt.mf_konly = false; }
+   opt.force_n_head = force_n_head;
+   knobs.free_device_bytes = free_device_bytes;
+   if (lds_bytes > 0) knobs.ft_lds_bytes = lds_bytes;
+   std::vector<BlockSym> sym;
+   BatchLayout old, lay;
+   const int n_threads = (int)std::max(1u, std::min(16u, std::thread::hardware_concurrency()));
+   PIPS_TRY(analyze_symbolic(in, S, n_threads, opt, knobs, sym));
+   PIPS_TRY(build_batch_layout(in, sym, S, knobs, lay));
+   PIPS_TRY(check_batch_layout(in, sym, S, knobs, lay));
+   knobs.tail_first_touch = 0;
+   PIPS_TRY(build_batch_layout(in, sym, S, knobs, old));
+   long long at = 0;
+   int section = 0;
+   auto put = [&](long long v) { if (at < cap) out[at] = v; ++at; };
+   long long from = 0;
+   auto end = [&]() { counts[8 + section++] = at - from; from = at; };
+   for (int b = 0; b < nblk; ++b) {
+      const BlkDesc& d = lay.h_blks[b];
+      put(d.n); put(d.n_head); put(d.m); put(d.m_pad); put(d.nb); put(d.ldT); put(d.mf_split); put(d.T_in); put(lay.kptr[b]);
+      put((long long)in[b].btcol.size()); put(lay.mf ? lay.h_root_off[b + 1] - lay.h_root_off[b] : 0); put(d.ntc);
+   }
+   end();
+   for (long long v : lay.h_ft_colbase) put(v);
+   end();
+   for (int v : lay.h_ft_init_off) put(v);
+   end();
+   for (const FtInit& e : lay.h_ft_init) { put(e.row); put(e.src); }
+   end();
+   for (int v : lay.h_ft_piece_off) put(v);
+   end();
+   for (const FtPiece& e : lay.h_ft_piece) { put(e.front); put(e.u); put(e.rows); put(e.cnt); }
+   end();
+   for (int v : lay.h_ft_leaves) put(v);
+   end();
+   for (long long v : old.h_kdst) put(v);
+   end();
+   for (long long v : lay.h_kdst) put(v);
+   end();
+   for (long long v : old.h_bdst) put(v);
+   end();
+   for (long long v : lay.h_bdst) put(v);
+   end();
+   for (int b = 0; b < nblk && lay.mf; ++b)
+      for (int q = lay.h_root_off[b]; q < lay.h_root_off[b + 1]; ++q) {
+         const SnDesc& sn = lay.h_sns[lay.h_roots[q]];
+         put(b); put(lay.h_roots[q]); put(sn.r); put(sn.rb); put(sn.U); put(sn.rows);
+      }
+   end();
+   for (int v : lay.h_rowidx) put(v);
+   end();
+   if (!lay.levels.empty()) {
+      const LevelRange& L0 = lay.levels[0];
+      for (int i = L0.simple_begin; i < L0.simple_begin + L0.simple_cnt; ++i) {
+         const SnDesc& sn = lay.h_sns[i];
+         put(i); put(sn.blk); put(sn.r); put(sn.n_useg); put(sn.rows);
+      }
+   }
+   end();
+   const int64_t head[8] = {lay.tail_first_touch, lay.mf, lay.tail_single, lay.schur_mode_eff, lay.mfU_total, lay.nnzK_total, lay.nnzB_total, at};
+   std::copy(head, head + 8, counts);
+   return PIPS_OK;
+}
+
 int pips_det_plan_probe(int nblk, const int* n, const int* n_primal, const int* const* krow, const int* const* kcol, int S,
                         const int* const* bt_rowptr, const int* const* bt_colidx, int rank, int n_ranks, int n_panels, long long* out,
                         long long cap, int64_t* counts) {
diff --git a/pips-ipmpp_amd/csrc/kernels.hip.h b/pips-ipmpp_amd/csrc/kernels.hip.h
--- a/pips-ipmpp_amd/csrc/kernels.hip.h
+++ b/pips-ipmpp_amd/csrc/kernels.hip.h
@@ -394,7 +394,8 @@
                                                            const int* __restrict__ sctab,
                                                            ScatterCtx sx = ScatterCtx{0, nullptr, nullptr, nullptr, nullptr}, int mf = 0,
                                                            double* __restrict__ lvals = nullptr, const int* __restrict__ lfpos = nullptr,
-                                                           double* __restrict__ lfval = nullptr, double* __restrict__ bbarena = nullptr) {
+                                                           double* __restrict__ lfval = nullptr, double* __restrict__ bbarena = nullptr,
+                                                           int defer = 0) {
    __shared__ int cnt_s[3];
    __shared__ int blk_s;
    const int t = blockIdx.x * blockDim.x + threadIdx.x;
@@ -462,6 +463,7 @@
             b_head = sb1;
          }
       }
+      if (defer) b_head = r;
 #pragma unroll
       for (int b = 0; b < SIMPLE_RMAX; ++b) {
          if (b < r && b >= b_head) {
@@ -485,6 +487,48 @@
    }
    __syncthreads();
    if (threadIdx.x < 3 && cnt_s[threadIdx.x]) atomicAdd(&inertia[3 * blk_s + threadIdx.x], cnt_s[threadIdx.x]);
+}
+
+__global__ __launch_bounds__(256) void k_leaf_products(const int* __restrict__ leaves, int cnt, const SnDesc* __restrict__ sns,
+                                                      const BlkDesc* __restrict__ blks, const int* __restrict__ rowidx,
+                                                      const int* __restrict__ bmap, double* __restrict__ arena, double* __restrict__ SC,
+                                                      int ldSC, const int* __restrict__ sctab) {
+   const int t = blockIdx.x * blockDim.x + threadIdx.x;
+   if (t >= cnt) return;
+   const SnDesc sn = sns[leaves[t]];
+   const BlkDesc bd = blks[sn.blk];
+   const int r = sn.r;
+   const double* P = arena + sn.panel;
+   const int* rows = rowidx + sn.rows;
+   const double d = P[0];
+   double l[SIMPLE_RMAX];
+   int ro[SIMPLE_RMAX];
+#pragma unroll
+   for (int a = 0; a < SIMPLE_RMAX; ++a)
+      if (a < r) { ro[a] = rows[a]; l[a] = P[1 + a]; }
+   double* T = arena + bd.T_in;
+   const int* bm = bmap + bd.bmap_off;
+   const int n = bd.n, n_head = bd.n_head;
+#pragma unroll
+   for (int b = 0; b < SIMPLE_RMAX; ++b) {
+      if (b < r) {
+         const int cb = ro[b];
+         const double lbd = l[b] * d;
+#pragma unroll
+         for (int a = b; a < SIMPLE_RMAX; ++a) {
+            if (a < r) {
+               const int ra = ro[a];
+               const double u = l[a] * lbd;
+               if (cb < n) {
+                  const int tr = ra < n ? ra - n_head : bd.m_pad + (ra - n);
+                  atomic_add_f64(T + tr + (long long)(cb - n_head) * bd.ldT, -u);
+               } else if (SC) {
+                  atomic_add_f64(sc_entry(SC, ldSC, bm, sctab, bd.sctab_off, bd.nb, ra - n, cb - n), -u);
+               }
+            }
+         }
+      }
+   }
 }
 
 __device__ __forceinline__ int packed_col(int p, int n) {
@@ -775,6 +819,7 @@
    const int n = bd.n, n_head = bd.n_head, c = blockIdx.y;
    double* S_ = gbuf ? gbuf + gstride * blk_group[blk] : SC;
    const bool tail_chunk = c < nt;
+   const bool ordered = tail_chunk || gbuf;
    if (!tail_chunk && (!S_ || bd.mf_split)) return;
    int lo, hi;
    if (tail_chunk) {
@@ -821,9 +866,79 @@
                if (gbuf) *tgt += u; else atomic_add_f64(tgt, u);
             }
          }
-         __syncthreads();
-      }
-   }
+         if (ordered) __syncthreads();
+      }
+   }
+}
+
+constexpr int FT_PF = 8;
+__global__ __launch_bounds__(64) void k_tail_first_touch(const BlkDesc* __restrict__ blks, const long long* __restrict__ colbase,
+                                                        const int* __restrict__ init_off, const FtInit* __restrict__ init,
+                                                        const int* __restrict__ piece_off, const FtPiece* __restrict__ piece,
+                                                        const int* __restrict__ rowidx, const double* __restrict__ kval,
+                                                        const double* __restrict__ bval, const double* __restrict__ uarena,
+                                                        double* __restrict__ arena) {
+   extern __shared__ __align__(16) double ft_col[];
+   typedef double double2_t __attribute__((ext_vector_type(2)));
+   const BlkDesc bd = blks[blockIdx.y];
+   const int c = blockIdx.x, lane = threadIdx.x;
+   if (c >= bd.m_pad) return;
+   const int r0 = c / TILE * TILE, len = bd.ldT - r0;
+   const long long g = colbase[blockIdx.y] + c;
+   const int i0 = init_off[g], i1 = init_off[g + 1], p0 = piece_off[g], p1 = piece_off[g + 1];
+   const int n = bd.n, n_head = bd.n_head, m_pad = bd.m_pad;
+   FtPiece d[FT_PF];
+   int ra[FT_PF][2];
+   double u[FT_PF][2];
+   auto request = [&](int pb) {
+#pragma unroll
+      for (int k = 0; k < FT_PF; ++k) {
+         d[k] = pb + k < p1 ? piece[pb + k] : FtPiece{0, 0, 0, 0};
+#pragma unroll
+         for (int h = 0; h < 2; ++h) {
+            ra[k][h] = 0; u[k][h] = 0.0;
+            if (lane + 64 * h < d[k].cnt) { ra[k][h] = rowidx[d[k].rows + lane + 64 * h]; u[k][h] = uarena[d[k].u + lane + 64 * h]; }
+         }
+      }
+   };
+   auto slot = [&](int row) { return (row < n ? row - n_head : m_pad + (row - n)) - r0; };
+   FtInit e0 = FtInit{0, 0};
+   if (i0 + lane < i1) e0 = init[i0 + lane];
+   request(p0);
+   double v0 = 0.0;
+   if (i0 + lane < i1) v0 = e0.src >= 0 ? kval[e0.src] : bval[~e0.src];
+   const double2_t z = {0.0, 0.0};
+   for (int i = 2 * lane; i < len; i += 128) *(double2_t*)(ft_col + i) = z;
+   __builtin_amdgcn_fence(__ATOMIC_ACQ_REL, "wavefront");
+   if (i0 + lane < i1) ft_col[e0.row - r0] = v0;
+   for (int q = i0 + 64 + lane; q < i1; q += 64) {
+      const FtInit e = init[q];
+      ft_col[e.row - r0] = e.src >= 0 ? kval[e.src] : bval[~e.src];
+   }
+   if (c >= bd.m && lane == 0) ft_col[c - r0] = 1.0;
+   __builtin_amdgcn_fence(__ATOMIC_ACQ_REL, "wavefront");
+   for (int pb = p0; pb < p1;) {
+#pragma unroll
+      for (int k = 0; k < FT_PF; ++k) {
+         const int cnt = d[k].cnt;
+         if (lane < cnt) ft_col[slot(ra[k][0])] += u[k][0];
+         if (lane + 64 < cnt) ft_col[slot(ra[k][1])] += u[k][1];
+         for (int i = 128 + lane; i < cnt; i += 64)
+            ft_col[slot(rowidx[d[k].rows + i])] += uarena[d[k].u + i];
+         __builtin_amdgcn_fence(__ATOMIC_ACQ_REL, "wavefront");
+      }
+      pb += FT_PF;
+      if (pb < p1) request(pb);
+   }
+   double2_t* dst = (double2_t*)(arena + bd.T_in + (long long)c * bd.ldT + r0);
+   constexpr int STEP = 128;
+   int i = 2 * lane;
+   for (; i + 3 * STEP < len; i += 4 * STEP) {
+      const double2_t a0 = *(const double2_t*)(ft_col + i), a1 = *(const double2_t*)(ft_col + i + STEP);
+      const double2_t a2 = *(const double2_t*)(ft_col + i + 2 * STEP), a3 = *(const double2_t*)(ft_col + i + 3 * STEP);
+      dst[i >> 1] = a0; dst[(i + STEP) >> 1] = a1; dst[(i + 2 * STEP) >> 1] = a2; dst[(i + 3 * STEP) >> 1] = a3;
+   }
+   for (; i < len; i += STEP) dst[i >> 1] = *(const double2_t*)(ft_col + i);
 }
 
 constexpr int BR_IDMAX = 192;
diff --git a/pips-ipmpp_amd/csrc/layout.cpp b/pips-ipmpp_amd/csrc/layout.cpp
--- a/pips-ipmpp_amd/csrc/layout.cpp
+++ b/pips-ipmpp_amd/csrc/layout.cpp
@@ -521,6 +521,74 @@
    return PIPS_OK;
 }
 
+int layout_first_touch(const std::vector<BlockSym>& sym, const Bases& B, const LayoutKnobs& knobs, BatchLayout& o) {
+   const int nblk = (int)sym.size();
+   o.tail_first_touch = false;
+   o.ft_ld_max = 0; o.ft_cols_max = 0;
+   for (const BlkDesc& bd : o.h_blks) { o.ft_ld_max = std::max(o.ft_ld_max, bd.ldT); o.ft_cols_max = std::max(o.ft_cols_max, bd.m_pad); }
+   if (knobs.tail_first_touch == 0 || !o.mf || knobs.deterministic || o.spine_total > 0 || o.ft_cols_max == 0 || o.levels.empty() ||
+       8LL * o.ft_ld_max > std::min(knobs.ft_lds_bytes, FT_LDS_MAX) || o.nnzK_total >= INT_MAX || o.nnzB_total >= INT_MAX)
+      return PIPS_OK;
+   for (const BlkDesc& bd : o.h_blks)
+      if ((bd.ldT & 1) || (bd.T_in & 1)) return PIPS_OK;
+   o.h_ft_colbase.assign(nblk + 1, 0);
+   for (int b = 0; b < nblk; ++b) o.h_ft_colbase[b + 1] = o.h_ft_colbase[b] + o.h_blks[b].m_pad;
+   if (o.h_ft_colbase[nblk] >= INT_MAX) return PIPS_OK;
+   const size_t ncols = (size_t)o.h_ft_colbase[nblk];
+   struct Init { int col, row, src; };
+   struct Piece { int col; FtPiece p; };
+   std::vector<Init> ini;
+   std::vector<Piece> pcs;
+   for (int b = 0; b < nblk; ++b) {
+      const BlockSym& s = sym[b];
+      const BlkDesc& bd = o.h_blks[b];
+      const int cb = (int)o.h_ft_colbase[b];
+      auto take = [&](const std::vector<int64_t>& dst, std::vector<long long>& out, long long base, bool border) -> int {
+         for (size_t p = 0; p < dst.size(); ++p) {
+            if (out[(size_t)base + p] < 0 || dst[p] < s.T_off) continue;
+            const long long rel = dst[p] - s.T_off;
+            const int c = (int)(rel / bd.ldT), row = (int)(rel % bd.ldT);
+            if (c >= bd.m_pad || row < c / TILE * TILE) PIPS_FAIL(PIPS_ERR_STATE, "analyze: internal error, entry %zu of block %d lands above the diagonal tile of tail column %d", p, b, c);
+            ini.push_back(Init{cb + c, row, border ? ~(int)(base + (long long)p) : (int)(base + (long long)p)});
+            out[(size_t)base + p] = -1;
+         }
+         return PIPS_OK;
+      };
+      if (int rc = take(s.a_dst, o.h_kdst, o.kptr[b], false)) return rc;
+      if (o.schur_mode_eff == 1)
+         if (int rc = take(s.b_dst, o.h_bdst, B.bptr[b], true)) return rc;
+      for (int q = o.h_root_off[b]; q < o.h_root_off[b + 1]; ++q) {
+         const SnDesc& sn = o.h_sns[o.h_roots[q]];
+         const int r = bd.mf_split == 2 ? sn.rb : sn.r;
+         const int* rows = o.h_rowidx.data() + sn.rows;
+         for (int a = 0; a < r; ++a) {
+            const int tr = rows[a] < bd.n ? rows[a] - bd.n_head : bd.m_pad + (rows[a] - bd.n);
+            if (rows[a] < bd.n_head || tr >= bd.ldT || (a > 0 && rows[a] <= rows[a - 1]))
+               PIPS_FAIL(PIPS_ERR_STATE, "analyze: internal error, row %d of root front %d of block %d", a, o.h_roots[q], b);
+         }
+         for (int bcol = 0; bcol < std::min(sn.rb, r); ++bcol)
+            pcs.push_back(Piece{cb + rows[bcol] - bd.n_head,
+                                FtPiece{sn.U + (long long)bcol * r - (long long)bcol * (bcol - 1) / 2, sn.rows + bcol, r - bcol, o.h_roots[q]}});
+      }
+   }
+   o.h_ft_init_off.assign(ncols + 1, 0); o.h_ft_piece_off.assign(ncols + 1, 0);
+   for (const Init& e : ini) ++o.h_ft_init_off[(size_t)e.col + 1];
+   for (const Piece& e : pcs) ++o.h_ft_piece_off[(size_t)e.col + 1];
+   for (size_t g = 0; g < ncols; ++g) { o.h_ft_init_off[g + 1] += o.h_ft_init_off[g]; o.h_ft_piece_off[g + 1] += o.h_ft_piece_off[g]; }
+   o.h_ft_init.assign(ini.size(), FtInit{0, 0}); o.h_ft_piece.assign(pcs.size(), FtPiece{0, 0, 0, 0});
+   {
+      std::vector<int> fi(o.h_ft_init_off.begin(), o.h_ft_init_off.end() - 1), fp(o.h_ft_piece_off.begin(), o.h_ft_piece_off.end() - 1);
+      for (const Init& e : ini) o.h_ft_init[(size_t)fi[(size_t)e.col]++] = FtInit{e.row, e.src};
+      for (const Piece& e : pcs) o.h_ft_piece[(size_t)fp[(size_t)e.col]++] = e.p;
+   }
+   const LevelRange& L0 = o.levels[0];
+   for (int i = L0.simple_begin; i < L0.simple_begin + L0.simple_cnt; ++i)
+      if (o.h_sns[i].n_useg == 0 && o.h_sns[i].r > 0) o.h_ft_leaves.push_back(i);
+   o.n_ft_leaves = (int)o.h_ft_leaves.size();
+   o.tail_first_touch = true;
+   return PIPS_OK;
+}
+
 void layout_full_rows(const std::vector<BlockInput>& in, const std::vector<BlockSym>& sym, BatchLayout& o) {
    const int nblk = (int)in.size();
    const std::vector<long long>&kptr = o.kptr, &x_off = o.x_off;
@@ -699,6 +767,7 @@
    layout_spine_lists(sym, sorted_id, lstar, out);
    layout_tail_single(sym, knobs, out);
    if ((rc = layout_index_arrays(in, sym, sorted_id, B, out))) return rc;
+   if ((rc = layout_first_touch(sym, B, knobs, out))) return rc;
    layout_full_rows(in, sym, out);
    layout_border_csr(in, S, B, out);
    layout_leaf_gather(out);
@@ -870,7 +939,8 @@
    drop(h_rowidx, h_sncol, h_bmap, h_perm, h_upd, h_mfint, h_nprimal, h_psign, h_psign_off, h_perm_off, h_kdst, h_bdst, h_kdiag, h_rowbase,
         h_krowptr, h_kcolidx, h_frowptr, h_fcol, h_fsrc, h_flong, h_bt_rowptr, h_bt_colidx, h_bt_xoff, h_bval, h_br_rowptr, h_br_sc, h_br_src,
         h_schur_slot, h_leafdesc, h_lf_rows, h_lf_ptr, h_lf_src, h_lf_pos, h_lb_list, tile_first, h_roots, h_bb_batches, h_bb_meta, h_bb_pos,
-        h_kb_rec, h_kb_list, h_kb_tail, h_kb_off, h_spine, h_spine_off);
+        h_kb_rec, h_kb_list, h_kb_tail, h_kb_off, h_spine, h_spine_off, h_ft_colbase, h_ft_init_off, h_ft_piece_off, h_ft_init, h_ft_piece,
+        h_ft_leaves);
 }
 
 }
diff --git a/pips-ipmpp_amd/csrc/layout.h b/pips-ipmpp_amd/csrc/layout.h
--- a/pips-ipmpp_amd/csrc/layout.h
+++ b/pips-ipmpp_amd/csrc/layout.h
@@ -39,6 +39,9 @@
 size_t bb_lds_bytes(const BbPlanSize& z);
 inline bool bb_fits(const BbPlanSize& z) { return bb_lds_bytes(z) <= 160 * 1024 && z.poscap <= 4 * 512 && z.stage <= 2 * 6 * 512; }
 
+constexpr long long FT_LDS_BUDGET = 80 * 1024;
+constexpr long long FT_LDS_MAX = 160 * 1024;
+
 struct LayoutKnobs {
    bool deterministic = false;
    int schur_mode = 0;
@@ -49,6 +52,8 @@
    int border_backward = -1, aug_sweeps = -1;
    bool sweep_launches = false;
    long long free_device_bytes = 0;
+   int tail_first_touch = -1;
+   long long ft_lds_bytes = FT_LDS_BUDGET;
    bool mf = false;
    int schur_mode_eff = 1;
 };
@@ -103,6 +108,14 @@
    std::vector<int> h_spine, h_spine_off;
    bool tail_single = false;
    long long tail_scratch = 0;
+   bool tail_first_touch = false;
+   int ft_ld_max = 0, ft_cols_max = 0;
+   int n_ft_leaves = 0;
+   std::vector<long long> h_ft_colbase;
+   std::vector<int> h_ft_init_off, h_ft_piece_off;
+   std::vector<FtInit> h_ft_init;
+   std::vector<FtPiece> h_ft_piece;
+   std::vector<int> h_ft_leaves;
    std::vector<int> schur_cols;
    std::vector<int> h_bt_rowsc, h_bt_rownnz, h_bt_rowblk;
    int n_flong = 0;
diff --git a/pips-ipmpp_amd/csrc/records.h b/pips-ipmpp_amd/csrc/records.h
--- a/pips-ipmpp_amd/csrc/records.h
+++ b/pips-ipmpp_amd/csrc/records.h
@@ -79,8 +79,15 @@
 
 struct BgEntry { long long off; unsigned y; unsigned short stride, w; };
 
+struct FtInit { int row, src; };
+struct FtPiece {
+   long long u, rows;
+   int cnt, front;
+};
+
 constexpr int FULL_LONG_ROW = 512;
 
+static_assert(sizeof(FtInit) == 8 && sizeof(FtPiece) == 24, "record layout read by the kernels");
 static_assert(sizeof(SnDesc) == 96 && sizeof(BlkDesc) == 176 && sizeof(TileTask) == 16, "record layout read by the kernels");
 static_assert(sizeof(BbMeta) == 32 && sizeof(BbBatch) == 40 && sizeof(LeafDesc) == 24 && sizeof(BgEntry) == 16, "record layout read by the kernels");
 
diff --git a/pips-ipmpp_amd/python/capi.py b/pips-ipmpp_amd/python/capi.py
--- a/pips-ipmpp_amd/python/capi.py
+++ b/pips-ipmpp_amd/python/capi.py
@@ -46,7 +46,7 @@
     "pips_hip_ldl_solve_dev", "pips_hip_ldl_solve_sparse", "pips_hip_ldl_factor_schur_batch", "pips_hip_ldl_solve_batch", "pips_hip_ldl_solve_batch_dev",
     "pips_hip_ldl_inertia_batch", "pips_hip_ldl_factor_schur_sparse", "pips_hip_ldl_factor_schur_sparse_batch",
     "pips_hip_dense_ldl_create", "pips_hip_dense_ldl_factor", "pips_hip_dense_ldl_factor_dev", "pips_hip_dense_ldl_solve",
-    "pips_hip_dense_ldl_solve_dev", "pips_hip_dense_ldl_inertia", "pips_hip_dense_ldl_info", "pips_hip_dense_ldl_set_pivoting", "pips_hip_dense_ldl_set_distributed", "pips_hip_dense_ldl_destroy", "pips_root_plan_build", "pips_layout_probe", "pips_tail_plan_probe", "pips_ipm_layout_probe", "pips_hip_host_wait_count", "pips_hip_host_wait_sites", "pips_hip_device_allocs_live", "pips_hip_device_bytes_live",
+    "pips_hip_dense_ldl_solve_dev", "pips_hip_dense_ldl_inertia", "pips_hip_dense_ldl_info", "pips_hip_dense_ldl_set_pivoting", "pips_hip_dense_ldl_set_distributed", "pips_hip_dense_ldl_destroy", "pips_root_plan_build", "pips_layout_probe", "pips_tail_plan_probe", "pips_first_touch_probe", "pips_ipm_layout_probe", "pips_hip_host_wait_count", "pips_hip_host_wait_sites", "pips_hip_device_allocs_live", "pips_hip_device_bytes_live",
     "pips_hip_batch_create", "pips_hip_batch_set_block", "pips_hip_batch_set_options", "pips_hip_batch_set_schur_mode", "pips_hip_batch_set_deterministic", "pips_hip_batch_get_schur_mode", "pips_hip_batch_add_regularization", "pips_hip_batch_set_refinement",
     "pips_hip_batch_last_refinement_steps", "pips_hip_batch_set_refinement_backward_error",
     "pips_hip_batch_last_refinement_measure", "pips_hip_batch_analyze",
@@ -619,12 +619,12 @@
         return (out.T if w < 2 else out), (m, m_pad, nb, ldT)
 
     def info(self):
-        what = np.zeros(27, np.int64)
-        _check(lib.pips_hip_batch_info(self._h, _ptr(what), C.c_int(27)), "pips_hip_batch_info")
+        what = np.zeros(28, np.int64)
+        _check(lib.pips_hip_batch_info(self._h, _ptr(what), C.c_int(28)), "pips_hip_batch_info")
         keys = ["nnzL", "n", "n_head", "m", "n_sn", "n_levels", "flops_factor", "flops_border", "arena_bytes", "ntc", "upd_table_bytes", "nb", "nnzK",
                 "ltsolve_from_augmented_factor", "multifrontal_head", "max_front", "update_matrix_bytes", "fronts_in_device_memory", "nnzL_head", "head_row_indices",
                 "nnzL_border", "augmented_sweeps", "augmented_passes", "tail_border_entries", "blocks_with_border_split", "blocks_with_k_only_fronts",
-                "packed_schur_rhs"]
+                "packed_schur_rhs", "tail_first_touch"]
         return {k: int(v) for k, v in zip(keys, what)}
 
     def sync(self):
```

Result: faster. 8.579 64-block work units/s (1 factorize + 4 solveCompressed) (median of 6 runs) (+1.3%).
